# konrad-kaminski/ratelimit

Hardware: AMD Instinct MI355X
Metric: rate-limit decisions/sec (whole node) at 10M/1B keys; p99 batch latency (higher is better)
Workload: dtype u32

## Files before the change

### ratelimit_amd/csrc/rl_engine.h

```cpp
#pragma once

#include <hip/hip_runtime.h>

#include <string>

#include "../../include/ratelimit_hip.h"
#include "rl_device.h"
#include "rl_kernels.h"
#include "rl_match.h"

namespace rl {

#ifndef RL_NBUF
#define RL_NBUF 4
#endif
constexpr uint32_t NBUF = RL_NBUF;
constexpr uint32_t ERRB_RING = 2 * NBUF;
constexpr uint32_t ERRW_B0 = NBUF + 3, ERRW_WORDS = ERRW_B0 + ERRB_RING;
constexpr uint32_t PROF_RING = 8;
constexpr uint32_t PROGRESS_RING = 64;

struct HostSlot {
  uint8_t* stem = nullptr;
  uint32_t *off = nullptr, *req = nullptr, *limit = nullptr, *hits = nullptr, *rule = nullptr;
  int64_t* now = nullptr;
  uint8_t *unit = nullptr, *flags = nullptr;
  uint8_t *code = nullptr, *status = nullptr;
  uint32_t *rem = nullptr, *reset = nullptr;
  unsigned long long* stats = nullptr;
  uint8_t* cbuf = nullptr;
  uint64_t cbuf_cap = 0;
  hipEvent_t in_done = nullptr;
  hipEvent_t out_done = nullptr;
};

struct Engine {
  rl_config cfg;
  hipStream_t stream = nullptr;
  hipStream_t pipe[NBUF] = {};
  hipEvent_t b_done[NBUF] = {};
  hipEvent_t b_table[NBUF] = {};
  hipEvent_t consumed[NBUF] = {};
  hipEvent_t route_ready = nullptr;
  hipEvent_t caller_ready = nullptr;
  bool serial_debug = false;
  uint32_t next = 0, last = NBUF - 1;
  uint32_t errb_seq = NBUF;
  bool b_early = true;
  uint64_t hash_seed = 0;
  HashKey hk{};
  Slot* slots = nullptr;
  uint64_t nslots = 0;
  LogEnt* log = nullptr;
  uint32_t log_cap = 0;
  unsigned long long* log_ctr = nullptr;
  uint32_t horizon = 0;
  uint32_t* tear = nullptr;
  bool copy_time = false;
  bool host_time = false;
  double ht[8] = {};
  uint64_t ht_n = 0;
  hipEvent_t ct_ev[3][64] = {};
  uint32_t ct_n = 0;
  double ct_ms = 0, ct_wait_ms = 0, ct_gap_ms = 0;
  uint64_t ct_count = 0;
  uint8_t* arena = nullptr;
  uint8_t* arena2 = nullptr;
  uint64_t arena_cap16 = 0;
  Scratch s[NBUF]{};
  Scratch rs{};
  bool rs_ready = false;
  unsigned long long* h_base = nullptr;
  uint32_t* errw = nullptr;
  uint8_t* d_stem = nullptr;
  uint32_t *d_off = nullptr, *d_req = nullptr, *d_limit = nullptr, *d_hits = nullptr, *d_rule = nullptr;
  int64_t* d_now = nullptr;
  uint8_t *d_unit = nullptr, *d_flags = nullptr, *d_code = nullptr, *d_status = nullptr;
  uint32_t *d_rem = nullptr, *d_reset = nullptr;
  unsigned long long* d_stats = nullptr;
  uint32_t* h_err = nullptr;
  uint32_t* h_long = nullptr;
  uint32_t long_recent = 0;
  int long_mode = 1;
  uint32_t* h_big = nullptr;
  uint32_t big_recent = 0;
  int big_mode = 1;
  uint32_t* h_late = nullptr;
  uint32_t late_recent = 0;
  int late_mode = 1;
  unsigned long long* h_counters = nullptr;
  std::string last_error;
  uint64_t batches = 0, decisions = 0;
  bool prof = false;
  uint32_t prof_every = 1, prof_skip = 0;
  bool prof_pending[PROF_RING] = {};
  uint32_t prof_next = 0;
  hipEvent_t ev[PROF_RING][RL_NUM_STAGES + 1] = {};
  double stage_ms[RL_NUM_STAGES] = {};
  uint64_t prof_batches = 0;
  unsigned long long* d_kt_acc = nullptr;
  double wclk_khz = 0;
  uint8_t* cfg_blob = nullptr;
  CfgDev cfg_dev{};
  bool cfg_loaded = false;
  uint8_t* mbuf = nullptr;
  size_t mbuf_cap = 0;
  uint32_t* h_match = nullptr;
  HostSlot hs[NBUF]{};
  hipStream_t h2d = nullptr, d2h = nullptr;
  uint32_t hnext = 0;
  bool hs_ready = false;
  uint64_t seq_sub = 0, seq_done = 0;
  hipEvent_t done_ring[PROGRESS_RING] = {};
};

enum StreamRole : uint32_t { SR_ROUTER = 1, SR_HOSTCOPY = 2, SR_PIPE = 4 };
hipError_t rl_stream_create(hipStream_t* st, uint32_t role);
Engine* eng_create(const rl_config* cfg, char* err, size_t errlen);
void eng_destroy(Engine* c);
const char* eng_last_error(const Engine* c);
int eng_do_limit(Engine* c, const rl_batch* in, rl_result* out);
int eng_do_limit_async(Engine* c, const rl_batch* in, rl_result* out, void* stream);
int eng_do_limit_host_async(Engine* c, const rl_batch* in, rl_result* out);
int eng_do_limit_compact_async(Engine* c, const rl_batch_compact* in, rl_result* out);
int eng_compact_check(Engine* c, const rl_batch_compact* in, const rl_result* out);
int eng_do_limit_prefixed_async(Engine* c, const rl_batch_prefixed* in, rl_result* out);
int eng_prefixed_check(Engine* c, const rl_batch_prefixed* in, const rl_result* out, uint32_t* tiles);
int eng_synchronize(Engine* c);
int eng_batch_progress(Engine* c, uint64_t* submitted, uint64_t* completed);
int eng_sweep(Engine* c, int64_t now, uint64_t* n_evicted);
int eng_restore(Engine* c, const rl_restore_batch* in);
int eng_table_info_get(Engine* c, rl_table_info* info);
int eng_debug_keys(Engine* c, const rl_batch* in, uint8_t* out_bytes, uint32_t* out_off, uint32_t out_cap);
int eng_debug_log_tear(Engine* c, const rl_log_tear* arm, rl_log_tear* out);
int eng_debug_decide(Engine* c, uint32_t n, const uint32_t* before, const uint32_t* after, const uint8_t* lc_hit,
                     const uint32_t* hits, const uint32_t* limit, const uint8_t* unit, const uint8_t* flags,
                     const int64_t* now, uint8_t* code, uint32_t* remaining, uint32_t* reset_s, uint64_t* stat_deltas,
                     uint8_t* lc_set);
struct RouteBufs {
  uint8_t* dest;
  uint32_t* hist;
  uint32_t* start;
};
int eng_route_pack(Engine* c, const rl_batch* in, uint32_t n_shards, uint32_t src_rank, void* send_rec,
                   uint8_t* send_stem, uint32_t* perm, uint64_t* counts, void* stream, uint32_t cstride = 2,
                   uint64_t meta0 = 0, uint64_t meta1 = 0, uint32_t own_rank = ROUTE_OWN_NONE,
                   unsigned long long* hash_out = nullptr, unsigned long long* counts_host = nullptr,
                   const RouteBufs* bufs = nullptr);
int eng_route_do_limit(Engine* c, uint32_t n, const void* recv_rec, const uint8_t* recv_stem, uint64_t recv_stem_bytes,
                       const uint64_t* src_stem_base, uint32_t n_shards, uint32_t n_rules, uint32_t rule_stride,
                       uint64_t* ret, uint64_t* stats, int isolate, void* stream);
int eng_route_scatter(Engine* c, uint32_t n, const uint32_t* perm, const uint64_t* ret, rl_result* out, void* stream);
int eng_profile(Engine* c, int enable);
int eng_profile_read(Engine* c, double* ms, uint32_t n, uint64_t* batches);
int eng_config_load(Engine* c, const rl_config_tree* tree);
using RequestsDoLimit = int (*)(void* user, const rl_batch* dev_in, rl_result* dev_out, hipStream_t st);
int eng_do_limit_requests(Engine* c, const rl_request_batch* in, rl_request_result* out, RequestsDoLimit run = nullptr,
                          void* user = nullptr);
int eng_local_cache_info_get(Engine* c, int64_t now, rl_local_cache_info* info);
int eng_snapshot_size(Engine* c, uint64_t* bytes);
int eng_snapshot_save(Engine* c, void* host, uint64_t bytes);
int eng_snapshot_load(Engine* c, const void* host, uint64_t bytes);

int eng_route_owner(Engine* c, uint32_t n, const Wire* recv_rec, const uint8_t* recv_stem, uint64_t recv_stem_bytes,
                    const uint64_t* src_stem_base, uint32_t n_src, uint32_t n_rules, uint32_t rule_stride,
                    unsigned long long* stats, int isolate, hipEvent_t ready, uint32_t* slot,
                    const OwnChunk* own = nullptr, const uint32_t* woff = nullptr,
                    const unsigned long long* wbad = nullptr);

int eng_fail(Engine* c, int code, const std::string& msg);

bool scratch_alloc(Scratch& s, uint32_t n);
void scratch_free(Scratch& s);

}
```

### ratelimit_amd/csrc/rl_engine.hip

```cpp
#include <hip/hip_runtime.h>
#include <hip/hip_ext.h>

#include <algorithm>
#include <chrono>
#include <cstdio>
#include <cstdlib>
#include <random>
#include <cstring>
#include <string>
#include <vector>

#include "../../include/ratelimit_hip.h"
#include "rl_device.h"
#include "rl_kernels.h"
#include "rl_match.h"
#include "rl_engine.h"

using namespace rl;



namespace {

thread_local std::string g_err;

int set_err(Engine* c, int code, const std::string& msg);

void prof_fold(Engine* c, uint32_t k) {
  if (!c->prof_pending[k]) return;
  c->prof_pending[k] = false;
  if (hipEventSynchronize(c->ev[k][RL_NUM_STAGES]) != hipSuccess) return;
  for (int i = 0; i < RL_NUM_STAGES; i++) {
    float ms = 0;
    if (hipEventElapsedTime(&ms, c->ev[k][i], c->ev[k][i + 1]) == hipSuccess) c->stage_ms[i] += ms;
  }
  c->prof_batches++;
}

void prof_fold_all(Engine* c) {
  for (uint32_t k = 0; k < PROF_RING; k++) prof_fold(c, (c->prof_next + k) % PROF_RING);
}

hipEvent_t* prof_events(Engine* c) {
  if (!c->prof) return nullptr;
  if (c->prof_skip) {
    c->prof_skip--;
    return nullptr;
  }
  c->prof_skip = c->prof_every - 1;
  const uint32_t k = c->prof_next;
  c->prof_next = (k + 1) % PROF_RING;
  prof_fold(c, k);
  c->prof_pending[k] = true;
  return c->ev[k];
}

int set_err(Engine* c, int code, const std::string& msg) {
  if (c) c->last_error = msg;
  else g_err = msg;
  return code;
}

#define HIPCHK(c, expr)                                                                        \
  do {                                                                                         \
    hipError_t _e = (expr);                                                                    \
    if (_e != hipSuccess)                                                                      \
      return set_err((c), RL_E_HIP, std::string("gpu: ") + #expr + ": " + hipGetErrorString(_e)); \
  } while (0)

template <typename T>
hipError_t dalloc(T** p, size_t count) {
  return hipMalloc((void**)p, std::max<size_t>(count, 1) * sizeof(T));
}

inline double wall_s() {
  return std::chrono::duration<double>(std::chrono::steady_clock::now().time_since_epoch()).count();
}

int map_err(Engine* c, uint32_t e) {
  if (!e) return RL_OK;
  if (e & ERR_TIME) return set_err(c, RL_E_TIME, "gpu: now outside [0, 2^32-172800] or before the last sweep");
  if (e & ERR_HISTORY)
    return set_err(c, RL_E_TIME,
                   "gpu: a request's window is older than its key's history holds (more than 8 windows and "
                   "div + expiration_jitter_max_seconds behind the key's newest, or the history log overwrote it: "
                   "raise history_entries)");
  if (e & ERR_INVALID) return set_err(c, RL_E_INVALID, "gpu: malformed batch (unit, rule id, request index or stem offsets)");
  if (e & ERR_TABLE_FULL) return set_err(c, RL_E_TABLE_FULL, "gpu: counter table full (raise table_slots or sweep)");
  if (e & ERR_ARENA_FULL) return set_err(c, RL_E_ARENA_FULL, "gpu: long-stem arena full (raise arena_bytes)");
  return set_err(c, RL_E_INTERNAL, "gpu: unknown device error");
}

hipError_t after_batches(Engine* c, hipStream_t st) {
  for (uint32_t k = 0; k < NBUF; k++) {
    const hipError_t e = hipStreamWaitEvent(st, c->b_done[k], 0);
    if (e != hipSuccess) return e;
  }
  return hipSuccess;
}

int collect(Engine* c, hipStream_t st = nullptr) {
  if (!st) st = c->stream;
  HIPCHK(c, hipMemcpyAsync(c->h_err, c->errw, ERRW_WORDS * sizeof(uint32_t), hipMemcpyDeviceToHost, st));
  HIPCHK(c, hipStreamSynchronize(st));
  uint32_t e = c->h_err[NBUF + 2];
  for (uint32_t j = 0; j < NBUF; j++) e |= c->h_err[j];
  for (uint32_t j = 0; j < ERRB_RING; j++) e |= c->h_err[ERRW_B0 + j];
  if (e || c->h_err[NBUF + 1]) {
    HIPCHK(c, hipMemsetAsync(c->errw, 0, ERRW_WORDS * sizeof(uint32_t), st));
    HIPCHK(c, hipStreamSynchronize(st));
  }
  return map_err(c, e);
}

TableDev table_view(Engine* c);
Params params(Engine* c, int isolate = 0);

uint32_t enqueue(Engine* c, const BatchDev& b_in, const OutDev& o, int restore, hipStream_t st, bool pipelined) {
  const uint32_t k = c->next;
  const BatchDev& b = b_in;
  c->next = (k + 1) % NBUF;
  TableDev t = table_view(c);
  t.log_epoch = c->s[k].log_epoch;
  const int isolate = (!restore && o.status) ? 1 : 0;
  const Params P = params(c, isolate);
  const uint32_t* errb_prev = c->s[c->last].errb;
  c->s[k].errb = c->errw + ERRW_B0 + (c->errb_seq++ % ERRB_RING);
  const bool early = c->b_early;
  bool lng = c->long_mode == 2;
  if (c->long_mode == 1) {
    for (uint32_t j = 0; j < NBUF; j++)
      if (__atomic_load_n(&c->h_long[j], __ATOMIC_RELAXED)) {
        __atomic_store_n(&c->h_long[j], 0u, __ATOMIC_RELAXED);
        c->long_recent = 4 * NBUF;
      }
    lng = c->long_recent > 0;
    if (c->long_recent) c->long_recent--;
  }
  uint32_t* hint = c->long_mode ? c->h_long + k : nullptr;
  bool big_full = c->big_mode == 0;
  if (c->big_mode == 1) {
    for (uint32_t j = 0; j < NBUF; j++)
      if (__atomic_load_n(&c->h_big[j], __ATOMIC_RELAXED)) {
        __atomic_store_n(&c->h_big[j], 0u, __ATOMIC_RELAXED);
        c->big_recent = 4 * NBUF;
      }
    big_full = c->big_recent > 0;
    if (c->big_recent) c->big_recent--;
  }
  uint32_t* bhint = c->big_mode == 1 ? c->h_big + k : nullptr;
  bool late_full = c->late_mode == 0;
  if (c->late_mode == 1) {
    for (uint32_t j = 0; j < NBUF; j++)
      if (__atomic_load_n(&c->h_late[j], __ATOMIC_RELAXED)) {
        __atomic_store_n(&c->h_late[j], 0u, __ATOMIC_RELAXED);
        c->late_recent = 4 * NBUF;
      }
    late_full = c->late_recent > 0;
    if (c->late_recent) c->late_recent--;
  }
  uint32_t* lhint = c->late_mode == 1 ? c->h_late + k : nullptr;
  if (pipelined) {
    hipStream_t a = c->pipe[k];
    hipEvent_t* ev = prof_events(c);
    (void)hipStreamWaitEvent(a, c->b_done[k], 0);
    (void)hipStreamWaitEvent(a, c->consumed[k], 0);
    launch_stage_a(b, c->s[k], isolate, P.per_second, a, ev, hint, lng, bhint, big_full);
    if (early) launch_b_begin_early(b, o, c->s[k], restore, a, c->log_ctr);
    (void)hipStreamWaitEvent(a, c->b_table[c->last], 0);
    launch_stage_b(b, o, t, P, c->s[k], restore, a, ev, errb_prev, c->b_table[k], ev ? c->d_kt_acc : nullptr,
                   early, lhint, late_full);
    (void)hipEventRecord(c->b_done[k], a);
  } else {
    if (!st) st = c->stream;
    (void)after_batches(c, st);
    hipEvent_t* ev = prof_events(c);
    launch_stage_a(b, c->s[k], isolate, P.per_second, st, ev, hint, lng, bhint, big_full);
    if (early) launch_b_begin_early(b, o, c->s[k], restore, st, c->log_ctr);
    launch_stage_b(b, o, t, P, c->s[k], restore, st, ev, errb_prev, c->b_table[k], ev ? c->d_kt_acc : nullptr,
                   early, lhint, late_full);
    (void)hipEventRecord(c->b_done[k], st);
  }
  c->last = k;
  return k;
}

hipError_t track(Engine* c, hipStream_t st) {
  if (c->seq_sub - c->seq_done >= PROGRESS_RING) {
    const hipError_t e = hipEventSynchronize(c->done_ring[c->seq_done % PROGRESS_RING]);
    if (e != hipSuccess) return e;
    c->seq_done++;
  }
  const hipError_t e = hipEventRecord(c->done_ring[c->seq_sub % PROGRESS_RING], st);
  c->seq_sub++;
  return e;
}

int check_sizes(Engine* c, const rl_batch* in, uint64_t stem_bytes) {
  if (!in) return set_err(c, RL_E_INVALID, "gpu: null batch");
  if (in->n > c->cfg.max_batch || in->n_requests > c->cfg.max_requests || in->n_rules > c->cfg.max_rules ||
      stem_bytes > c->cfg.max_stem_bytes)
    return set_err(c, RL_E_CAPACITY, "gpu: batch exceeds configured max_batch/max_requests/max_rules/max_stem_bytes");
  if (in->n && in->n_requests == 0) return set_err(c, RL_E_INVALID, "gpu: descriptors without requests");
  return RL_OK;
}

BatchDev dev_view(const Engine* c, const rl_batch* in, uint32_t stem_cap) {
  BatchDev b{};
  b.hk = c->hk;
  b.n = in->n;
  b.n_req = in->n_requests;
  b.n_rules = in->n_rules;
  b.stem_cap = stem_cap;
  b.stem_total = stem_cap;
  b.now_desc = 0;
  b.stem = in->stem_bytes;
  b.off = in->stem_off;
  b.now = in->now;
  b.req = in->req_idx;
  b.unit = in->unit;
  b.flags = in->flags;
  b.limit = in->limit;
  b.hits = in->hits;
  b.rule = in->rule_id;
  return b;
}

hipError_t log_ctr_get(Engine* c, std::vector<unsigned long long>& ctr, unsigned long long* lost,
                       unsigned long long* refused = nullptr) {
  std::vector<unsigned long long> h((size_t)(LOG_PARTS + 1) * LOG_CTR_STRIDE);
  hipError_t e = hipMemcpyAsync(h.data(), c->log_ctr, h.size() * 8, hipMemcpyDeviceToHost, c->stream);
  if (e == hipSuccess) e = hipStreamSynchronize(c->stream);
  if (e != hipSuccess) return e;
  ctr.resize(LOG_PARTS);
  for (uint32_t k = 0; k < LOG_PARTS; k++) ctr[k] = h[(size_t)k * LOG_CTR_STRIDE];
  if (lost) *lost = h[(size_t)LOG_PARTS * LOG_CTR_STRIDE];
  if (refused) *refused = h[(size_t)LOG_PARTS * LOG_CTR_STRIDE + 1];
  return hipSuccess;
}

TableDev table_view(Engine* c) {
  TableDev t;
  t.slots = c->slots;
  t.log = c->log;
  t.log_ctr = c->log_ctr;
  t.log_cap = c->log_cap;
  t.horizon = c->horizon;
  t.hist_lost = c->log_ctr + (size_t)LOG_PARTS * LOG_CTR_STRIDE;
  t.tear = c->tear;
  t.log_epoch = nullptr;
  t.mask = c->nslots - 1;
  t.arena = c->arena;
  t.arena_used16 = c->s[0].counters + 4;
  t.arena_cap16 = c->arena_cap16;
  t.max_probe = (uint32_t)std::min<uint64_t>(c->nslots, 1u << 16);
  t.shift = 64u - (uint32_t)__builtin_ctzll(c->nslots);
  return t;
}

Params params(Engine* c, int isolate) {
  Params P;
  P.ratio = c->cfg.near_limit_ratio;
  P.lc_en = c->cfg.local_cache_enabled != 0;
  P.per_second = c->cfg.per_second_split != 0;
  P.isolate = isolate;
  return P;
}

bool alloc_buffer(Scratch& s, uint32_t n) {
  const size_t items = (size_t)n / (64 * 4 * 8) + 1 + PART_DIGITS;
  bool ok = dalloc(&s.big_meta, PART_DIGITS) == hipSuccess && dalloc(&s.big_n, 1) == hipSuccess &&
            dalloc(&s.big_work, items) == hipSuccess && dalloc(&s.work_n, 1) == hipSuccess &&
            dalloc(&s.sorted_n, 1) == hipSuccess &&
            dalloc(&s.big_cnt, items * (1 + 2 * BIG_HEAVY)) == hipSuccess;
  ok = ok && dalloc(&s.rec, n) == hipSuccess && dalloc(&s.res, n) == hipSuccess;
  for (int i = 0; i < 2; i++) ok = ok && dalloc(&s.keys[i], n) == hipSuccess && dalloc(&s.vals[i], n) == hipSuccess;
  ok = ok && dalloc(&s.grp, n) == hipSuccess && dalloc(&s.lead, n) == hipSuccess && dalloc(&s.gmask, n) == hipSuccess &&
       dalloc(&s.defer, n) == hipSuccess &&
       dalloc(&s.defer_n, 1) == hipSuccess && dalloc(&s.defer2, n) == hipSuccess &&
       dalloc(&s.defer1, n) == hipSuccess && dalloc(&s.defer1_n, 1) == hipSuccess &&
       dalloc(&s.defer2_n, 1) == hipSuccess && dalloc(&s.fast_blk, (size_t)n / (256 * 32) + 1) == hipSuccess &&
       dalloc(&s.log_epoch, LOG_PARTS) == hipSuccess &&
       dalloc(&s.uniq, n) == hipSuccess && dalloc(&s.uniq_n, 1) == hipSuccess &&
       dalloc(&s.long_runs, (size_t)n / 1024 + 2) == hipSuccess &&
       dalloc(&s.kt_blk, 2 * ((size_t)n / 2 + BIG_HEAVY * PART_DIGITS + 2 * (size_t)n + 512) / 256) == hipSuccess;
  ok = ok && dalloc(&s.hits_s, n) == hipSuccess && dalloc(&s.segsum, n) == hipSuccess &&
       dalloc(&s.rid, n) == hipSuccess && dalloc(&s.run_start, (size_t)n + 1) == hipSuccess &&
       dalloc(&s.run_flags, n) == hipSuccess && dalloc(&s.run_state, n) == hipSuccess && dalloc(&s.run_alias, n) == hipSuccess &&
       dalloc(&s.run_f, n) == hipSuccess &&
       dalloc(&s.runs64, 1) == hipSuccess && dalloc(&s.split, 2) == hipSuccess && dalloc(&s.drun, (size_t)n / 2 + BIG_HEAVY * PART_DIGITS) == hipSuccess;
  ok = ok && dalloc(&s.hit_a, n) == hipSuccess && dalloc(&s.tile, n) == hipSuccess &&
       dalloc(&s.hit_t, n) == hipSuccess;
  ok = ok && dalloc(&s.run_end, n) == hipSuccess &&
       dalloc(&s.part_info, (size_t)PART_DIGITS * std::max((n + PART_TILE - 1) / PART_TILE, 1u)) == hipSuccess;
  ok = ok && dalloc(&s.r_base, RL_MAX_SHARDS) == hipSuccess && dalloc(&s.woff, (size_t)n + 1) == hipSuccess &&
       dalloc(&s.wtsum, WIRE_SCAN_WORDS(n)) == hipSuccess;
  return ok;
}

void free_buffer(Scratch& s) {
  void* bufs[] = {s.rec, s.res, s.big_meta, s.big_n, s.big_work, s.work_n, s.sorted_n, s.big_cnt, s.keys[0], s.keys[1],
                  s.vals[0], s.vals[1], s.grp, s.lead, s.gmask, s.defer, s.defer_n, s.defer2, s.defer2_n, s.defer1,
                  s.defer1_n, s.fast_blk, s.hits_s, s.segsum, s.rid, s.run_start, s.run_flags, s.run_state, s.run_alias,
                  s.run_f, s.runs64, s.split, s.drun, s.run_end, s.part_info, s.hit_a, s.tile, s.hit_t, s.r_base,
                  s.uniq, s.uniq_n, s.long_runs, s.kt_blk, s.log_epoch, s.woff, s.wtsum};
  for (void* p : bufs)
    if (p) (void)hipFree(p);
}

int stage(Engine* c, const rl_batch* in, BatchDev* out) {
  const uint32_t n = in->n, nq = in->n_requests;
  const uint64_t nb = n ? in->stem_off[n] : 0;
  int rc = check_sizes(c, in, nb);
  if (rc) return rc;
  hipStream_t st = c->stream;
  HIPCHK(c, after_batches(c, st));
  if (nb) HIPCHK(c, hipMemcpyAsync(c->d_stem, in->stem_bytes, nb, hipMemcpyHostToDevice, st));
  HIPCHK(c, hipMemcpyAsync(c->d_off, in->stem_off, (n + 1) * sizeof(uint32_t), hipMemcpyHostToDevice, st));
  if (nq) HIPCHK(c, hipMemcpyAsync(c->d_now, in->now, nq * sizeof(int64_t), hipMemcpyHostToDevice, st));
  if (n) {
    HIPCHK(c, hipMemcpyAsync(c->d_req, in->req_idx, n * 4, hipMemcpyHostToDevice, st));
    HIPCHK(c, hipMemcpyAsync(c->d_unit, in->unit, n, hipMemcpyHostToDevice, st));
    HIPCHK(c, hipMemcpyAsync(c->d_flags, in->flags, n, hipMemcpyHostToDevice, st));
    HIPCHK(c, hipMemcpyAsync(c->d_limit, in->limit, n * 4, hipMemcpyHostToDevice, st));
    HIPCHK(c, hipMemcpyAsync(c->d_hits, in->hits, n * 4, hipMemcpyHostToDevice, st));
    HIPCHK(c, hipMemcpyAsync(c->d_rule, in->rule_id, n * 4, hipMemcpyHostToDevice, st));
  }
  rl_batch d = *in;
  d.stem_bytes = c->d_stem;
  d.stem_off = c->d_off;
  d.now = c->d_now;
  d.req_idx = c->d_req;
  d.unit = c->d_unit;
  d.flags = c->d_flags;
  d.limit = c->d_limit;
  d.hits = c->d_hits;
  d.rule_id = c->d_rule;
  *out = dev_view(c, &d, c->cfg.max_stem_bytes);
  return RL_OK;
}

}

namespace rl {

const char* eng_last_error(const Engine* c) { return c ? c->last_error.c_str() : g_err.c_str(); }

hipError_t rl_stream_create(hipStream_t* st, uint32_t role) {
  static const uint32_t dedicated =
      getenv("RL_DEDICATED_QUEUES") ? (uint32_t)strtoul(getenv("RL_DEDICATED_QUEUES"), nullptr, 0) : 0u;
  if (!(dedicated & role)) return hipStreamCreateWithFlags(st, hipStreamNonBlocking);
  int dev = 0, cus = 0;
  hipError_t e = hipGetDevice(&dev);
  if (e == hipSuccess) e = hipDeviceGetAttribute(&cus, hipDeviceAttributeMultiprocessorCount, dev);
  if (e != hipSuccess) return e;
  std::vector<uint32_t> mask(((uint32_t)cus + 31) / 32, 0xFFFFFFFFu);
  return hipExtStreamCreateWithCUMask(st, (uint32_t)mask.size(), mask.data());
}

Engine* eng_create(const rl_config* cfg_in, char* err, size_t errlen) {
  auto fail = [&](const std::string& m, Engine* c) -> Engine* {
    if (err && errlen) snprintf(err, errlen, "%s", m.c_str());
    g_err = m;
    if (c) eng_destroy(c);
    return nullptr;
  };
  if (!cfg_in) return fail("gpu: null config", nullptr);
  rl_config cfg = *cfg_in;
  if (!cfg.table_slots) cfg.table_slots = 1ull << 24;
  if (cfg.table_slots & (cfg.table_slots - 1)) return fail("gpu: table_slots must be a power of two", nullptr);
  if (!cfg.arena_bytes) cfg.arena_bytes = 64ull << 20;
  if (!cfg.history_entries) cfg.history_entries = cfg.table_slots;
  if (cfg.history_entries > (uint64_t)LOG_PARTS * LOG_PART_MAX)
    return fail("gpu: history_entries must be at most 2^31", nullptr);
  if (cfg.expiration_jitter_max_seconds < 0) return fail("gpu: expiration_jitter_max_seconds must be >= 0", nullptr);
  if (!cfg.max_batch) cfg.max_batch = 1u << 20;
  if (cfg.max_batch > MAX_PART_TILES * PART_TILE)
    return fail("gpu: max_batch must be at most 8388608 descriptors", nullptr);
  if (!cfg.max_requests) cfg.max_requests = cfg.max_batch;
  if (!cfg.max_rules) cfg.max_rules = 65536;
  if (!cfg.max_stem_bytes) cfg.max_stem_bytes = 128u * cfg.max_batch;
  if (hipSetDevice(cfg.device) != hipSuccess) return fail("gpu: hipSetDevice failed", nullptr);

  Engine* c = new Engine();
  c->cfg = cfg;
  c->hash_seed = cfg.hash_seed;
  while (!c->hash_seed) {
    std::random_device rd;
    c->hash_seed = ((uint64_t)rd() << 32) ^ rd();
  }
  c->cfg.hash_seed = c->hash_seed;
  c->hk = hash_key_of(c->hash_seed, cfg.debug_hash_bits);
  c->nslots = cfg.table_slots;
  {
    const uint64_t want = std::max<uint64_t>(cfg.history_entries / LOG_PARTS, std::max<uint64_t>(cfg.max_batch / 16, 1024));
    uint64_t cap = 1;
    while (cap * 2 <= want && cap * 2 <= LOG_PART_MAX) cap *= 2;
    if (cap < want && cap < LOG_PART_MAX) cap *= 2;
    c->log_cap = (uint32_t)cap;
    c->cfg.history_entries = (uint64_t)LOG_PARTS * cap;
    c->horizon = (uint32_t)std::min<int64_t>(cfg.expiration_jitter_max_seconds, 1ll << 30);
  }
  c->arena_cap16 = cfg.arena_bytes / 16;
  const uint32_t n = cfg.max_batch;
  bool ok = true;
  for (uint32_t k = 0; k < NBUF; k++) ok = ok && rl_stream_create(&c->pipe[k], SR_PIPE) == hipSuccess;
  if (const char* be = getenv("RL_B_BEGIN_EARLY")) c->b_early = atoi(be) != 0;
  c->stream = c->pipe[0];
  for (uint32_t k = 0; k < NBUF; k++)
    ok = ok && hipEventCreateWithFlags(&c->b_done[k], hipEventDisableTiming) == hipSuccess &&
         hipEventCreateWithFlags(&c->b_table[k], hipEventDisableTiming) == hipSuccess;
  for (uint32_t k = 0; k < PROGRESS_RING; k++)
    ok = ok && hipEventCreateWithFlags(&c->done_ring[k], hipEventDisableTiming) == hipSuccess;
  ok = ok && dalloc(&c->slots, c->nslots) == hipSuccess &&
       dalloc(&c->log, (size_t)LOG_PARTS * c->log_cap) == hipSuccess &&
       dalloc(&c->log_ctr, (size_t)(LOG_PARTS + 1) * LOG_CTR_STRIDE) == hipSuccess;
  ok = ok && dalloc(&c->arena, cfg.arena_bytes) == hipSuccess && dalloc(&c->arena2, cfg.arena_bytes) == hipSuccess;
  for (uint32_t k = 0; k < NBUF; k++) ok = ok && alloc_buffer(c->s[k], n);
  Scratch& s0 = c->s[0];
  ok = ok && dalloc(&c->errw, ERRW_WORDS) == hipSuccess;
  for (uint32_t k = 0; k < NBUF; k++)
    ok = ok && hipEventCreateWithFlags(&c->consumed[k], hipEventDisableTiming) == hipSuccess;
  ok = ok && hipEventCreateWithFlags(&c->route_ready, hipEventDisableTiming) == hipSuccess &&
       hipEventCreateWithFlags(&c->caller_ready, hipEventDisableTiming) == hipSuccess;
  c->serial_debug = getenv("RL_DEBUG_SERIAL") != nullptr;
  c->copy_time = getenv("RL_DEBUG_COPYTIME") != nullptr;
  c->host_time = getenv("RL_DEBUG_HOSTTIME") != nullptr;
  for (uint32_t k = 0; c->copy_time && k < 64; k++)
    ok = ok && hipEventCreate(&c->ct_ev[0][k]) == hipSuccess && hipEventCreate(&c->ct_ev[1][k]) == hipSuccess &&
         hipEventCreate(&c->ct_ev[2][k]) == hipSuccess;
  ok = ok && hipHostMalloc((void**)&c->h_base, (size_t)NBUF * RL_MAX_SHARDS * 8) == hipSuccess;
  for (uint32_t k = 0; k < NBUF; k++)
    ok = ok && dalloc(&c->s[k].stripes, (size_t)STAT_STRIPES * STAT_LDS_RULES * RL_NUM_STATS) == hipSuccess;
  ok = ok && dalloc(&s0.time_floor, 1) == hipSuccess;
  ok = ok && dalloc(&s0.counters, 8) == hipSuccess;
  for (uint32_t k = 0; k < NBUF; k++) {
    Scratch& sk = c->s[k];
    sk.err = c->errw ? c->errw + k : nullptr;
    sk.errb = c->errw ? c->errw + ERRW_B0 + k : nullptr;
    sk.errs = c->errw ? c->errw + NBUF + 1 : nullptr;
    sk.time_floor = s0.time_floor;
    sk.counters = s0.counters;
  }
  ok = ok && dalloc(&c->d_stem, (size_t)cfg.max_stem_bytes + 64) == hipSuccess;
  ok = ok && dalloc(&c->d_off, (size_t)n + 1) == hipSuccess;
  ok = ok && dalloc(&c->d_now, cfg.max_requests) == hipSuccess;
  ok = ok && dalloc(&c->d_req, n) == hipSuccess && dalloc(&c->d_unit, n) == hipSuccess &&
       dalloc(&c->d_flags, n) == hipSuccess && dalloc(&c->d_limit, n) == hipSuccess &&
       dalloc(&c->d_hits, n) == hipSuccess && dalloc(&c->d_rule, n) == hipSuccess;
  ok = ok && dalloc(&c->d_code, n) == hipSuccess && dalloc(&c->d_status, n) == hipSuccess &&
       dalloc(&c->d_rem, n) == hipSuccess &&
       dalloc(&c->d_reset, n) == hipSuccess;
  ok = ok && dalloc(&c->d_stats, (size_t)cfg.max_rules * RL_NUM_STATS) == hipSuccess;
  ok = ok && hipHostMalloc((void**)&c->h_err, ERRW_WORDS * sizeof(uint32_t)) == hipSuccess;
  ok = ok && hipHostMalloc((void**)&c->h_counters, 8 * sizeof(unsigned long long)) == hipSuccess;
  ok = ok && hipHostMalloc((void**)&c->h_long, NBUF * sizeof(uint32_t)) == hipSuccess;
  if (ok) memset(c->h_long, 0, NBUF * sizeof(uint32_t));
  if (const char* sl = getenv("RL_SPLIT_LONG")) c->long_mode = atoi(sl);
  ok = ok && hipHostMalloc((void**)&c->h_big, NBUF * sizeof(uint32_t)) == hipSuccess;
  if (ok) memset(c->h_big, 0, NBUF * sizeof(uint32_t));
  if (const char* bc = getenv("RL_BIG_CUE")) c->big_mode = atoi(bc);
  ok = ok && hipHostMalloc((void**)&c->h_late, NBUF * sizeof(uint32_t)) == hipSuccess;
  if (ok) memset(c->h_late, 0, NBUF * sizeof(uint32_t));
  if (const char* lc = getenv("RL_LATE_CUE")) c->late_mode = atoi(lc);
  if (!ok) return fail("gpu: device allocation failed (table_slots/arena/max_batch too large?)", c);
  ok = hipMemsetAsync(c->slots, 0, c->nslots * sizeof(Slot), c->stream) == hipSuccess &&
       hipMemsetAsync(c->log_ctr, 0, (size_t)(LOG_PARTS + 1) * LOG_CTR_STRIDE * 8, c->stream) == hipSuccess &&
       hipMemsetAsync(c->errw, 0, ERRW_WORDS * 4, c->stream) == hipSuccess &&
       hipMemsetAsync(s0.time_floor, 0, 8, c->stream) == hipSuccess &&
       hipMemsetAsync(s0.counters, 0, 64, c->stream) == hipSuccess &&
       hipMemsetAsync(c->s[0].stripes, 0, (size_t)STAT_STRIPES * STAT_LDS_RULES * RL_NUM_STATS * 8, c->stream) ==
           hipSuccess &&
       hipMemsetAsync(c->d_stem, 0, (size_t)cfg.max_stem_bytes + 64, c->stream) == hipSuccess &&
       hipStreamSynchronize(c->stream) == hipSuccess;
  for (uint32_t k = 0; k < NBUF; k++)
    ok = ok && hipEventRecord(c->b_done[k], c->stream) == hipSuccess &&
         hipEventRecord(c->b_table[k], c->stream) == hipSuccess &&
         (k == 0 || hipMemsetAsync(c->s[k].stripes, 0, (size_t)STAT_STRIPES * STAT_LDS_RULES * RL_NUM_STATS * 8,
                                   c->stream) == hipSuccess) &&
         hipEventRecord(c->consumed[k], c->stream) == hipSuccess;
  if (!ok) return fail("gpu: device initialisation failed", c);
  return c;
}

void free_host_slots(Engine* c) {
  for (HostSlot& h : c->hs) {
    void* bufs[] = {h.stem, h.off, h.req, h.limit, h.hits, h.rule, h.now, h.unit, h.flags, h.code, h.status, h.rem,
                    h.reset, h.stats, h.cbuf};
    for (void* p : bufs)
      if (p) (void)hipFree(p);
    if (h.in_done) (void)hipEventDestroy(h.in_done);
    if (h.out_done) (void)hipEventDestroy(h.out_done);
    h = HostSlot{};
  }
  for (hipStream_t st : {c->h2d, c->d2h})
    if (st) (void)hipStreamDestroy(st);
  c->h2d = c->d2h = nullptr;
  c->hs_ready = false;
}

void copy_time_fold(Engine* c, bool all);

void eng_destroy(Engine* c) {
  if (!c) return;
  (void)hipSetDevice(c->cfg.device);
  if (c->host_time && c->ht_n)
    fprintf(stderr, "RL_DEBUG_HOSTTIME: %llu batches, ms each: check %.4f copy %.4f unpack %.4f enqueue %.4f to_host %.4f "
            "track %.4f\n", (unsigned long long)c->ht_n, c->ht[0] / c->ht_n * 1e3, c->ht[1] / c->ht_n * 1e3,
            c->ht[2] / c->ht_n * 1e3, c->ht[3] / c->ht_n * 1e3, c->ht[4] / c->ht_n * 1e3, c->ht[5] / c->ht_n * 1e3);
  if (c->copy_time) {
    (void)hipDeviceSynchronize();
    copy_time_fold(c, true);
    if (c->ct_count)
      fprintf(stderr, "RL_DEBUG_COPYTIME: %llu input copies, %.4f ms each, slot wait %.4f ms, gap after the previous "
              "copy %.4f ms\n", (unsigned long long)c->ct_count, c->ct_ms / c->ct_count, c->ct_wait_ms / c->ct_count,
              c->ct_gap_ms / c->ct_count);
    for (uint32_t k = 0; k < 64; k++)
      for (int j = 0; j < 3; j++)
        if (c->ct_ev[j][k]) (void)hipEventDestroy(c->ct_ev[j][k]);
  }
  if (c->hs_ready) {
    (void)hipDeviceSynchronize();
    free_host_slots(c);
  }
  for (uint32_t k = 0; k < NBUF; k++)
    if (c->pipe[k]) (void)hipStreamSynchronize(c->pipe[k]);
  for (uint32_t k = 0; k < PROF_RING; k++)
    for (int i = 0; i <= RL_NUM_STAGES; i++)
      if (c->ev[k][i]) (void)hipEventDestroy(c->ev[k][i]);
  if (c->d_kt_acc) (void)hipFree(c->d_kt_acc);
  for (uint32_t k = 0; k < NBUF; k++) {
    free_buffer(c->s[k]);
    if (c->b_done[k]) (void)hipEventDestroy(c->b_done[k]);
    if (c->b_table[k]) (void)hipEventDestroy(c->b_table[k]);
    if (c->consumed[k]) (void)hipEventDestroy(c->consumed[k]);
  }
  for (uint32_t k = 0; k < PROGRESS_RING; k++)
    if (c->done_ring[k]) (void)hipEventDestroy(c->done_ring[k]);
  if (c->rs_ready) {
    c->rs.err = nullptr;
    scratch_free(c->rs);
  }
  if (c->route_ready) (void)hipEventDestroy(c->route_ready);
  if (c->caller_ready) (void)hipEventDestroy(c->caller_ready);
  if (c->h_base) (void)hipHostFree(c->h_base);
  const Scratch& s0 = c->s[0];
  void* bufs[] = {c->slots, c->log, c->log_ctr, c->tear, c->arena, c->arena2, c->errw, s0.stripes, s0.time_floor, s0.counters, c->d_stem, c->d_off,
                  c->d_now, c->d_req, c->d_unit, c->d_flags, c->d_limit, c->d_hits, c->d_rule, c->d_code, c->d_status,
                  c->d_rem,
                  c->d_reset, c->d_stats};
  for (void* p : bufs)
    if (p) (void)hipFree(p);
  for (uint32_t k = 1; k < NBUF; k++)
    if (c->s[k].stripes) (void)hipFree(c->s[k].stripes);
  if (c->h_err) (void)hipHostFree(c->h_err);
  if (c->h_counters) (void)hipHostFree(c->h_counters);
  if (c->h_long) (void)hipHostFree(c->h_long);
  if (c->h_big) (void)hipHostFree(c->h_big);
  if (c->h_late) (void)hipHostFree(c->h_late);
  for (void* p : {(void*)c->cfg_blob, (void*)c->mbuf})
    if (p) (void)hipFree(p);
  if (c->h_match) (void)hipHostFree(c->h_match);
  for (uint32_t k = 0; k < NBUF; k++)
    if (c->pipe[k]) (void)hipStreamDestroy(c->pipe[k]);
  delete c;
}

int eng_do_limit_async(Engine* c, const rl_batch* in, rl_result* out, void* stream) {
  if (!c || !in || !out) return set_err(c, RL_E_INVALID, "gpu: null argument");
  int rc = check_sizes(c, in, 0);
  if (rc) return rc;
  if ((uintptr_t)in->stem_bytes & 3u) return set_err(c, RL_E_INVALID, "gpu: stem_bytes must be 4-byte aligned");
  HIPCHK(c, hipSetDevice(c->cfg.device));
  BatchDev b = dev_view(c, in, c->cfg.max_stem_bytes);
  OutDev o{out->code, out->limit_remaining, out->reset_s, (unsigned long long*)out->stats, out->status};
  hipStream_t st = (hipStream_t)stream;
  if (st && c->serial_debug) {
    enqueue(c, b, o, 0, st, false);
    HIPCHK(c, track(c, st));
  } else {
    if (st && hipStreamQuery(st) == hipErrorNotReady) {
      HIPCHK(c, hipEventRecord(c->caller_ready, st));
      HIPCHK(c, hipStreamWaitEvent(c->pipe[c->next], c->caller_ready, 0));
    }
    const uint32_t k = enqueue(c, b, o, 0, nullptr, true);
    HIPCHK(c, track(c, c->pipe[k]));
  }
  HIPCHK(c, hipGetLastError());
  c->batches++;
  c->decisions += in->n;
  return RL_OK;
}

bool scratch_alloc(Scratch& s, uint32_t n) {
  s = Scratch{};
  bool ok = alloc_buffer(s, n);
  ok = ok && dalloc(&s.err, 1) == hipSuccess && dalloc(&s.route_start, 2 * RL_MAX_SHARDS + 1) == hipSuccess &&
       dalloc(&s.route_dest, n) == hipSuccess && dalloc(&s.route_hash, n) == hipSuccess &&
       dalloc(&s.route_hist, 2ull * RL_MAX_SHARDS * ((n + ROUTE_TILE - 1) / ROUTE_TILE)) == hipSuccess;
  ok = ok && hipMemset(s.err, 0, 4) == hipSuccess;
  return ok;
}

void scratch_free(Scratch& s) {
  free_buffer(s);
  for (void* p : {(void*)s.err, (void*)s.route_start, (void*)s.route_dest, (void*)s.route_hash, (void*)s.route_hist})
    if (p) (void)hipFree(p);
  s = Scratch{};
}

int eng_route_pack(Engine* c, const rl_batch* in, uint32_t n_shards, uint32_t src_rank, void* send_rec,
                   uint8_t* send_stem, uint32_t* perm, uint64_t* counts, void* stream, uint32_t cstride,
                   uint64_t meta0, uint64_t meta1, uint32_t own_rank, unsigned long long* hash_out,
                   unsigned long long* counts_host, const RouteBufs* bufs) {
  if (!c || !in || !counts || (in->n && (!send_rec || !send_stem || !perm)))
    return set_err(c, RL_E_INVALID, "gpu: null argument");
  if (n_shards < 1 || n_shards > RL_MAX_SHARDS || src_rank >= n_shards)
    return set_err(c, RL_E_INVALID, "gpu: n_shards must be 1..256 and src_rank < n_shards");
  int rc = check_sizes(c, in, 0);
  if (rc) return rc;
  if ((uintptr_t)in->stem_bytes & 3u) return set_err(c, RL_E_INVALID, "gpu: stem_bytes must be 4-byte aligned");
  HIPCHK(c, hipSetDevice(c->cfg.device));
  if (!c->rs_ready) {
    HIPCHK(c, after_batches(c, c->stream));
    HIPCHK(c, hipStreamSynchronize(c->stream));
    if (!scratch_alloc(c->rs, c->cfg.max_batch)) {
      scratch_free(c->rs);
      return set_err(c, RL_E_HIP, "gpu: routing scratch allocation failed");
    }
    (void)hipFree(c->rs.err);
    c->rs.err = c->errw + NBUF + 2;
    c->rs_ready = true;
  }
  hipStream_t st = stream ? (hipStream_t)stream : c->stream;
  BatchDev b = dev_view(c, in, c->cfg.max_stem_bytes);
  Scratch rs = c->rs;
  if (bufs) {
    rs.route_dest = bufs->dest;
    rs.route_hist = bufs->hist;
    rs.route_start = bufs->start;
  }
  launch_route_pack(b, n_shards, src_rank, (Wire*)send_rec, send_stem, perm, (unsigned long long*)counts, rs, st,
                    cstride, meta0, meta1, own_rank, hash_out, counts_host);
  HIPCHK(c, hipGetLastError());
  return RL_OK;
}

int eng_route_owner(Engine* c, uint32_t n, const Wire* recv_rec, const uint8_t* recv_stem, uint64_t recv_stem_bytes,
                    const uint64_t* src_stem_base, uint32_t n_src, uint32_t n_rules, uint32_t rule_stride,
                    unsigned long long* stats, int isolate, hipEvent_t ready, uint32_t* slot,
                    const OwnChunk* own, const uint32_t* woff, const unsigned long long* wbad) {
  const uint32_t rules_eff = rule_stride ? n_src * rule_stride : n_rules;
  const bool has_own = own && own->n;
  if (!c || !src_stem_base || (n && (!recv_rec || (!recv_stem && recv_stem_bytes))) || (rules_eff && !stats))
    return set_err(c, RL_E_INVALID, "gpu: null argument");
  if (n && !recv_stem && !(has_own && own->n == n)) return set_err(c, RL_E_INVALID, "gpu: null argument");
  if (has_own && ((uint64_t)own->lo + own->n > n || own->rank >= n_src || !own->idx || !own->hash || !own->stem ||
                  ((uintptr_t)own->stem & 3u)))
    return set_err(c, RL_E_INVALID, "gpu: bad own chunk");
  if (n_src < 1 || n_src > RL_MAX_SHARDS) return set_err(c, RL_E_INVALID, "gpu: n_shards must be 1..256");
  if (rule_stride && n_rules > rule_stride) return set_err(c, RL_E_INVALID, "gpu: n_rules exceeds the rule stride");
  if (n > c->cfg.max_batch || rules_eff > c->cfg.max_rules || recv_stem_bytes >= (1ull << 32))
    return set_err(c, RL_E_CAPACITY, "gpu: routed batch exceeds max_batch/max_rules or 4 GiB of stems");
  if ((uintptr_t)recv_stem & 3u) return set_err(c, RL_E_INVALID, "gpu: recv_stem must be 4-byte aligned");
  HIPCHK(c, hipSetDevice(c->cfg.device));
  const uint32_t k = c->next;
  Scratch& sk = c->s[k];
  hipStream_t a = c->pipe[k];
  HIPCHK(c, hipStreamWaitEvent(a, c->b_done[k], 0));
  HIPCHK(c, hipStreamWaitEvent(a, c->consumed[k], 0));
  if (ready) HIPCHK(c, hipStreamWaitEvent(a, ready, 0));
  if (!(has_own && own->n == n)) {
    unsigned long long* hb = c->h_base + (size_t)k * RL_MAX_SHARDS;
    HIPCHK(c, hipEventSynchronize(c->b_done[k]));
    for (uint32_t j = 0; j < n_src; j++) hb[j] = src_stem_base[j];
    HIPCHK(c, hipMemcpyAsync(sk.r_base, hb, (size_t)n_src * 8, hipMemcpyHostToDevice, a));
    if (!woff) {
      launch_wire_offsets(recv_rec, n, has_own ? own->lo : 0u, has_own ? own->lo + own->n : 0u, sk.r_base, n_src,
                          recv_stem_bytes, sk.woff, sk.wtsum, a);
      woff = sk.woff;
      wbad = sk.wtsum + WIRE_SCAN_TILES(n);
    }
  }
  BatchDev b{};
  b.hk = c->hk;
  b.n = n;
  b.n_req = n;
  b.n_rules = rules_eff;
  b.stem_cap = (uint32_t)recv_stem_bytes;
  b.stem_total = (uint32_t)recv_stem_bytes;
  b.now_desc = 1;
  b.stem = recv_stem;
  b.wire = recv_rec;
  b.woff = woff;
  b.wbad = wbad;
  b.wbase = sk.r_base;
  b.n_src = n_src;
  b.rule_stride = rule_stride;
  if (has_own) b.own = *own;
  OutDev o{nullptr, nullptr, nullptr, stats, isolate ? c->d_status : nullptr};
  const uint32_t kk = enqueue(c, b, o, 0, nullptr, true);
  HIPCHK(c, hipGetLastError());
  c->batches++;
  c->decisions += n;
  *slot = kk;
  return RL_OK;
}

int eng_route_do_limit(Engine* c, uint32_t n, const void* recv_rec, const uint8_t* recv_stem, uint64_t recv_stem_bytes,
                       const uint64_t* src_stem_base, uint32_t n_shards, uint32_t n_rules, uint32_t rule_stride,
                       uint64_t* ret, uint64_t* stats, int isolate, void* stream) {
  if (!c || (n && !ret)) return set_err(c, RL_E_INVALID, "gpu: null argument");
// ... 987 lines not shown
```

### ratelimit_amd/csrc/rl_kernels.h

```cpp
#pragma once

#include <hip/hip_runtime.h>
#include <stdint.h>

#include "rl_device.h"

namespace rl {

#ifndef RL_PART_ITEMS
#define RL_PART_ITEMS 16
#endif
constexpr uint32_t PART_ITEMS = RL_PART_ITEMS, PART_TILE = 256 * PART_ITEMS;
constexpr uint32_t PART_BITS = 10, PART_DIGITS = 1u << PART_BITS;
#ifndef RL_BIG_BLOCKS
#define RL_BIG_BLOCKS 64
#endif
constexpr uint32_t BIG_BLOCKS = RL_BIG_BLOCKS;
constexpr uint32_t BIG_ITEM_BLOCKS = 256;
constexpr uint32_t BIG_HEAVY = 4;

struct BigMeta {
  uint32_t d, S, base, nchunks, item0, r, rb_heavy, db_heavy;
  uint32_t heavy[BIG_HEAVY];
};
constexpr uint32_t MAX_PART_TILES = 2048 * 16 / PART_ITEMS;
constexpr uint32_t LONG_RUN = 32;
constexpr uint32_t RUN_SLOW = 1, RUN_FAST = 2, RUN_MULTI = 4;
constexpr uint32_t RUN_NOWVAR = 8;
constexpr uint32_t RUN_ALIAS = 16;
constexpr uint32_t RUN_AHEAD = 32;
constexpr uint32_t RUN_MERGE = 64;
constexpr uint32_t RUN_G_SHIFT = 8, RUN_UMASK_SHIFT = 16;
constexpr uint32_t RUN_UNITS = 128, RUN_STEMS = 1u << 24;
#ifndef RL_KEY_HEAD
#define RL_KEY_HEAD 64
#endif
constexpr uint32_t KEY_HEAD = RL_KEY_HEAD;
constexpr uint32_t KEY_HV = KEY_HEAD / 16;
static_assert(KEY_HEAD % 16 == 0 && KEY_HEAD >= 48 && KEY_HEAD <= 64, "key head: 48 or 64 bytes (>= KEY_IN)");
constexpr uint32_t STAT_STRIPES = 64;
constexpr uint32_t STAT_LDS_RULES = 512;
constexpr uint32_t RUNS_GENERAL_LATE_BLOCKS = 8;

struct Wire;
struct OwnChunk {
  uint32_t lo, n, rank, stem_total;
  uint32_t src_n;
  uint32_t n_rules;
  const uint32_t* idx;
  const unsigned long long* hash;
  const uint8_t* stem;
  const uint32_t* off;
  const int64_t* now;
  const uint32_t* req;
  const uint8_t* unit;
  const uint8_t* flags;
  const uint32_t* limit;
  const uint32_t* hits;
  const uint32_t* rule;
  uint8_t* code;
  uint32_t* rem;
  uint32_t* reset;
  uint8_t* status;
  uint32_t* src_err;
};
struct BatchDev {
  uint32_t n, n_req, n_rules, stem_cap;
  uint32_t stem_total;
  uint32_t now_desc;
  HashKey hk;
  const uint8_t* stem;
  const uint32_t* off;
  const int64_t* now;
  const uint32_t* req;
  const uint8_t* unit;
  const uint8_t* flags;
  const uint32_t* limit;
  const uint32_t* hits;
  const uint32_t* rule;
  const Wire* wire;
  const uint32_t* woff;
  const unsigned long long* wbad;
  const unsigned long long* wbase;
  uint32_t n_src, rule_stride;
  OwnChunk own;
};

struct __attribute__((aligned(16))) Rec {
  uint32_t hlo;
  uint32_t off;
  uint32_t lu;
  uint32_t rule;
  uint32_t req;
  uint32_t now;
  uint32_t hits;
  uint32_t limit;
};
static_assert(sizeof(Rec) == 32, "Rec is two dwordx4");

struct SRec {
  const Rec* rec;
  const uint32_t* sv;
  __device__ inline Rec operator[](uint32_t q) const { return rec[sv[q]]; }
};

__host__ __device__ inline uint32_t rec_len(const Rec& r) { return r.lu & 0xFFFFu; }
__host__ __device__ inline uint32_t rec_unit(const Rec& r) { return (r.lu >> 16) & 0xFFu; }
__host__ __device__ inline uint32_t rec_flags(const Rec& r) { return r.lu >> 24; }

constexpr uint32_t ROUTE_REQ_BITS = 24;
constexpr uint32_t ROUTE_MAX_REQ = 1u << ROUTE_REQ_BITS;
constexpr uint32_t ROUTE_TILE = 512;
struct __attribute__((aligned(8))) Wire {
  uint32_t label;
  uint32_t lu;
  uint32_t limit;
  uint32_t hits;
  uint32_t rule;
  uint32_t now;
  unsigned long long hash;
};
constexpr uint32_t WIRE_NOW_BAD = 0xFFFFFFFFu;
static_assert(sizeof(Wire) == RL_WIRE_BYTES, "wire record size is part of the ABI");

struct OutDev {
  uint8_t* code;
  uint32_t* rem;
  uint32_t* reset;
  unsigned long long* stats;
  uint8_t* status;
};

struct TableDev {
  Slot* slots;
  LogEnt* log;
  unsigned long long* log_ctr;
  uint32_t log_cap;
  uint32_t horizon;
  unsigned long long* hist_lost;
  const unsigned long long* log_epoch;
  uint32_t* tear;
  uint64_t mask;
  uint8_t* arena;
  unsigned long long* arena_used16;
  uint64_t arena_cap16;
  uint32_t max_probe;
  uint32_t shift;
};

struct Params {
  float ratio;
  int lc_en;
  int per_second;
  int isolate;
};

struct Scratch {
  Rec* rec;
  unsigned long long* res;
  uint32_t* keys[2];
  uint32_t* vals[2];
  BigMeta* big_meta;
  uint32_t* big_n;
  uint32_t* big_work;
  uint32_t* work_n;
  uint32_t* sorted_n;
  uint32_t* big_cnt;
  uint32_t* grp;
  uint32_t* lead;
  uint8_t* gmask;
  uint32_t* defer;
  uint32_t* defer_n;
  uint32_t* defer2;
  uint32_t* defer2_n;
  uint32_t* defer1;
  uint32_t* defer1_n;
  uint32_t* fast_blk;
  unsigned long long* log_epoch;
  uint2* uniq;
  uint32_t* uniq_n;
  uint32_t* long_runs;
  unsigned long long* kt_blk;
  unsigned long long* stripes;
  uint32_t* hits_s;
  uint32_t* hit_a;
  uint4* tile;
  uint32_t* hit_t;
  uint32_t* segsum;
  uint32_t* rid;
  uint32_t* run_start;
  uint32_t* run_end;
  uint32_t* part_info;
  uint32_t* run_flags;
  uint4* run_state;
  uint4* run_alias;
  uint32_t* run_f;
  unsigned long long* runs64;
  unsigned long long* split;
  uint32_t* drun;
  uint32_t* err;
  uint32_t* errb;
  uint32_t* errs;
  int64_t* time_floor;
  unsigned long long* counters;
  uint32_t* route_start;
  uint8_t* route_dest;
  unsigned long long* route_hash;
  uint32_t* route_hist;
  unsigned long long* r_base;
  uint32_t* woff;
  unsigned long long* wtsum;
};

void launch_stage_a(const BatchDev& b, const Scratch& s, int isolate, int per_second, hipStream_t st,
                    hipEvent_t* ev = nullptr, uint32_t* long_hint = nullptr, bool long_kernel = false,
                    uint32_t* big_hint = nullptr, bool big_full = true);
void launch_stage_b(const BatchDev& b, const OutDev& o, const TableDev& t, const Params& P, const Scratch& s,
                    int restore, hipStream_t st, hipEvent_t* ev, const uint32_t* errb_prev, hipEvent_t table_done,
                    unsigned long long* kt_acc = nullptr, bool early = false, uint32_t* late_hint = nullptr,
                    bool late_full = true);
void launch_b_begin_early(const BatchDev& b, const OutDev& o, const Scratch& s, int restore, hipStream_t st,
                          const unsigned long long* log_ctr);
void launch_unpack(const rl_batch_compact& cb, const uint8_t* buf, uint32_t* req, uint8_t* unit, uint8_t* flags,
                   uint32_t* limit, uint32_t* hits, uint32_t* rule, int64_t* now, uint32_t* err, hipStream_t st);
void launch_unpack_range(const rl_batch_compact& cb, const uint8_t* buf, uint32_t d0, uint32_t d1, uint32_t q0,
                         uint32_t q1, uint32_t* req, uint8_t* unit, uint8_t* flags, uint32_t* limit, uint32_t* hits,
                         uint32_t* rule, int64_t* now, uint32_t* err, hipStream_t st);
constexpr uint32_t TO_HOST_MAX = 6;
struct ToHost {
  const uint8_t* src[TO_HOST_MAX];
  uint8_t* dst[TO_HOST_MAX];
  uint64_t bytes[TO_HOST_MAX];
  uint32_t n;
};
void launch_to_host(const ToHost& c, hipStream_t st);
hipError_t copy_to_host(ToHost c, hipStream_t st);

void launch_unpack_prefixed(const rl_batch_prefixed& pb, const uint8_t* buf, uint32_t t0, uint32_t t1, uint8_t* stem,
                            uint32_t* off, uint32_t* req, uint8_t* unit, uint8_t* flags, uint32_t* limit,
                            uint32_t* hits, uint32_t* rule, int64_t* now, uint32_t* err, hipStream_t st);
constexpr uint32_t ROUTE_OWN_NONE = 0xFFFFFFFFu;
constexpr uint32_t WIRE_SCAN_TILE = 2048;
inline uint32_t WIRE_SCAN_TILES(uint64_t n) { return (uint32_t)((n + WIRE_SCAN_TILE) / WIRE_SCAN_TILE); }
inline uint32_t WIRE_SCAN_WORDS(uint64_t n) { return WIRE_SCAN_TILES(n) + 1; }
void launch_wire_offsets(const Wire* w, uint32_t n, uint32_t olo, uint32_t ohi, const unsigned long long* wbase,
                         uint32_t n_src, unsigned long long stem_total, uint32_t* woff, unsigned long long* tsum,
                         hipStream_t st);
void launch_route_pack(const BatchDev& b, uint32_t n_shards, uint32_t src_rank, Wire* out, uint8_t* out_stem,
                       uint32_t* perm, unsigned long long* counts, const Scratch& s, hipStream_t st,
                       uint32_t cstride = 2, unsigned long long meta0 = 0, unsigned long long meta1 = 0,
                       uint32_t own_rank = ROUTE_OWN_NONE, unsigned long long* hash_out = nullptr,
                       unsigned long long* counts_host = nullptr);
void launch_cnt_fill(unsigned long long* cnt, uint32_t n_peers, uint32_t cstride, unsigned long long meta0,
                     unsigned long long meta1, hipStream_t st, unsigned long long* cnt_host = nullptr);
void launch_route_fail(unsigned long long* ret, uint32_t n, uint32_t status, hipStream_t st);
void launch_route_scatter(const uint32_t* perm, const unsigned long long* ret, uint32_t n, const OutDev& o,
                          hipStream_t st, uint32_t* src_err = nullptr, const uint32_t* errb = nullptr,
                          uint32_t own_lo = 0, uint32_t own_hi = 0);
void launch_route_ret(const unsigned long long* res, uint32_t n, const uint32_t* errb, unsigned long long* ret,
                      hipStream_t st);
void launch_stats_sum(const unsigned long long* stage, uint32_t n_blocks, uint32_t m, unsigned long long* out,
                      hipStream_t st, uint32_t stride = 0);
void launch_sweep(const TableDev& t, uint64_t nslots, uint32_t now, unsigned long long* evicted, hipStream_t st);
void launch_arena_compact(Slot* slots, uint64_t nslots, const uint8_t* from, uint8_t* to, unsigned long long* used16,
                          hipStream_t st);
void launch_lc_count(const TableDev& t, uint64_t nslots, uint32_t now, unsigned long long* out, hipStream_t st);
void launch_table_info(const Slot* slots, uint64_t nslots, unsigned long long* out, hipStream_t st);
bool log_tear_hook();
void launch_debug_keys(const BatchDev& b, uint8_t* out, uint32_t* klen, hipStream_t st);
void launch_debug_decide(uint32_t n, const uint32_t* before, const uint32_t* after, const uint8_t* lc_hit,
                         const uint32_t* hits, const uint32_t* limit, const uint8_t* unit, const uint8_t* flags,
                         const int64_t* now, float ratio, int lc_en, uint8_t* code, uint32_t* rem, uint32_t* reset,
                         unsigned long long* deltas, uint8_t* lc_set, hipStream_t st);

}
```

### ratelimit_amd/csrc/rl_kernels.hip

```cpp
#include <hip/hip_runtime.h>
#include <stdint.h>
#include <cstdlib>

#include "rl_device.h"
#include "rl_kernels.h"

#ifndef RL_ABL
#define RL_ABL 0
#endif

namespace rl {

constexpr uint32_t HASH_LDS_BYTES = 16384;

__global__ __launch_bounds__(256) void k_prepare(BatchDev b, Rec* __restrict__ rec, uint32_t* __restrict__ keys,
                                                 uint32_t* err, uint32_t* errs, int isolate,
                                                 const int64_t* time_floor, uint32_t* defer_n,
                                                 uint32_t* big_n, uint32_t* work_n, uint32_t* __restrict__ run_flags,
                                                 unsigned long long* num_runs, uint32_t* __restrict__ hit_a,
                                                 unsigned long long* __restrict__ res, uint32_t* sorted_n,
                                                 uint32_t* uniq_n) {
  __shared__ uint32_t lds[HASH_LDS_BYTES / 4 + 4];
  const uint32_t tid = threadIdx.x;
  const uint32_t i = blockIdx.x * 256 + tid;
// ... 1195 lines not shown
        c = Win{x.w, 0, 0, lcw};
      } else if (G.old[ui].ws != x.w) {
        gen_set_old(t, G, ui, Win{x.w, 0, 0, lcw}, true);
      }
    }
    for (uint32_t k = 0; k < 4; k++) {
      if (!(G.present >> k & 1) || ps_class(P, k) != ps_e) continue;
      Win* R = gen_rec(t, G, k, x.w, x.now, nullptr);
      if (R) {
        R->count = nv;
        R->expire = ex;
        gen_touch(G, k, R);
      }
    }
    after = nv;
  }
  if (restore) {
    if (x.flags) {
      for (uint32_t k = 0; k < 4; k++) {
        if (!(G.present >> k & 1)) continue;
        Win* R = gen_rec(t, G, k, x.w, x.now, nullptr);
        if (R) {
          R->lc = x.now + x.d;
          gen_touch(G, k, R);
        }
      }
    }
    return;
  }
  const Decision r = decide(after - x.h, after, lc_hit && !x.shadow, x.h, x.thr, P.ratio, x.shadow, P.lc_en);
  if (r.set_lc) {
    uint32_t j = 0;
    while (j < G.npend && G.pend_w[j] != x.w) j++;
    if (j == G.npend) G.npend++;
    G.pend_w[j] = x.w;
    G.pend_e[j] = x.now + x.d;
  }
  emit(res, L, acc, x, r, lc_hit);
}

__device__ __attribute__((always_inline)) inline void replay_simple(SRec rec_s, const uint32_t* svals,
                                                                    unsigned long long* res, const TableDev& t,
                                                                    const Params& P, const uint32_t* grp,
                                                                    uint32_t p, uint32_t end, uint32_t k, int64_t s0,
                                                                    Win cur0, uint32_t ring0, uint32_t tag0,
                                                                    const Rec& x0, uint32_t e0, LaneStats& L,
                                                                    StatAcc& acc, uint32_t* err, bool restore) {
  Slot* s = &t.slots[s0];
  SimpleState S;
  S.cur = cur0;
  S.old = Win{WS_INVALID, 0, 0, 0};
  S.si = (uint32_t)s0;
  S.tag = tag0;
  S.chain = ring0;
  S.cur_dirty = S.old_dirty = S.chain_dirty = false;
  S.cur_req = 0xFFFFFFFFu;
  S.pend = false;
  simple_step(t, P, res, L, acc, S, load_elem(x0, e0, restore), restore, err);
  for (uint32_t q = p + 1; q < end; q++) {
    if (grp && grp[q] != k) continue;
    simple_step(t, P, res, L, acc, S, load_elem(rec_s[q], svals[q], restore), restore, err);
  }
  S.apply_pending();
  if (S.old_dirty) simple_put(t, S);
  if (S.cur_dirty) s->cur = S.cur;
  if (S.chain_dirty) s->ring = S.chain;
}

__device__ __attribute__((always_inline)) inline uint32_t wave_incl_add(uint32_t x);
struct SegPair {
  uint32_t f, s;
};
__device__ inline SegPair seg_op(SegPair a, SegPair b) { return SegPair{a.f | b.f, b.f ? b.s : a.s + b.s}; }

struct SegChunk {
  uint64_t heads;
  uint32_t h;
};

__device__ inline SegPair seg_chunk_scan(const SegChunk& c, uint32_t lane) {
  const uint32_t P = wave_incl_add(c.h);
  const uint64_t le = c.heads & (lane == 63 ? ~0ull : ((2ull << lane) - 1));
  const uint32_t lh = le ? 63u - (uint32_t)__clzll((long long)le) : 0u;
  const uint32_t Plh = __shfl(P, lh, 64), hlh = __shfl(c.h, lh, 64);
  return le ? SegPair{1u, P - (Plh - hlh)} : SegPair{0u, P};
}

constexpr uint32_t BK_HEAVY = BIG_HEAVY;
constexpr uint32_t BK_HEAVY_MIN = 3;

template <uint32_t W, uint32_t IT>
struct BkShape {
  static constexpr uint32_t WAVES = W, ITEMS = IT, THREADS = 64 * W, CAP = 64 * W * IT, STRIP = 64 * IT;
};
using BkSmall = BkShape<4, 8>;
using BkBig = BkShape<8, 8>;

#ifdef RL_BK_PROF
__device__ unsigned long long g_bk_prof[PART_DIGITS * 16];
__device__ uint32_t g_bk_peel[PART_DIGITS * 16];
#define BK_STAMP(d, k) \
  if (threadIdx.x == 0) g_bk_prof[(d) * 16 + (k)] = wall_clock64()
#else
#define BK_STAMP(d, k)
#endif

template <uint32_t IT, uint32_t BITS>
__device__ inline void wave_multisplit(const uint32_t (&kk)[IT], uint32_t nvalid_base, uint32_t limit, uint32_t shift,
                                       uint32_t* row, uint32_t (&pos)[IT]) {
  const uint32_t lane = threadIdx.x & 63;
  const uint64_t lt_mask = (1ull << lane) - 1;
  uint32_t leader[IT];
#pragma unroll
  for (uint32_t i = 0; i < IT; i++) {
    leader[i] = lane;
    pos[i] = 0;
    if (nvalid_base + i * 64 >= limit) continue;
    const bool valid = nvalid_base + i * 64 + lane < limit;
    const uint32_t d = (kk[i] >> shift) & ((1u << BITS) - 1u);
    uint64_t peers = __ballot(valid);
#pragma unroll
    for (uint32_t bit = 0; bit < BITS; bit++) {
      const bool sb = (d >> bit) & 1u;
      const uint64_t bal = __ballot(sb);
      peers &= sb ? bal : ~bal;
    }
    const uint32_t rank = __popcll(peers & lt_mask);
    leader[i] = valid ? (uint32_t)(__ffsll((unsigned long long)peers) - 1) : lane;
    pos[i] = (valid && rank == 0) ? atomicAdd(&row[d], (uint32_t)__popcll(peers)) : 0u;
    pos[i] |= rank << 16;
  }
#pragma unroll
  for (uint32_t i = 0; i < IT; i++) pos[i] = __shfl(pos[i] & 0xFFFFu, leader[i]) + (pos[i] >> 16);
}

__device__ inline uint32_t scan256(uint32_t v, uint32_t* wsum4, uint32_t* total) {
  const uint32_t lane = threadIdx.x & 63, wave = threadIdx.x >> 6;
  uint32_t inc = v;
#pragma unroll
  for (uint32_t off = 1; off < 64; off <<= 1) {
    const uint32_t y = __shfl_up(inc, off, 64);
    if (lane >= off) inc += y;
  }
  if (wave < 4 && lane == 63) wsum4[wave] = inc;
  __syncthreads();
  uint32_t pre = 0;
#pragma unroll
  for (uint32_t w = 0; w < 4; w++) pre += w < wave ? wsum4[w] : 0u;
  if (total) *total = wsum4[0] + wsum4[1] + wsum4[2] + wsum4[3];
  __syncthreads();
  return pre + inc - v;
}

__global__ __launch_bounds__(256) void k_part(const uint32_t* __restrict__ kin, const uint32_t* __restrict__ hin,
                                              uint4* __restrict__ out, uint32_t n, uint32_t ntiles,
                                              uint32_t* __restrict__ info, const uint32_t* err) {
  constexpr uint32_t DPT = PART_DIGITS / 256;
  __shared__ uint32_t wcnt[4][PART_DIGITS];
  __shared__ uint32_t wsum[4];
  __shared__ uint32_t sk[PART_TILE], sv[PART_TILE], sh[PART_TILE];
  if (*err) return;
  const uint32_t tid = threadIdx.x, lane = tid & 63, wave = tid >> 6, tile = blockIdx.x;
  for (uint32_t j = tid; j < 4 * PART_DIGITS; j += 256) (&wcnt[0][0])[j] = 0;
  __syncthreads();
  const uint32_t wbase = tile * PART_TILE + wave * 64 * PART_ITEMS;
  uint32_t kk[PART_ITEMS], vv[PART_ITEMS], hh[PART_ITEMS], pos[PART_ITEMS];
#pragma unroll
  for (uint32_t i = 0; i < PART_ITEMS; i++) {
    const uint32_t j = min(wbase + i * 64 + lane, n - 1);
    kk[i] = kin[j];
    vv[i] = j;
    hh[i] = hin[j];
  }
  wave_multisplit<PART_ITEMS, PART_BITS>(kk, wbase, n, 32 - PART_BITS, wcnt[wave], pos);
  __syncthreads();
  uint32_t c[DPT], tsum = 0;
#pragma unroll
  for (uint32_t j = 0; j < DPT; j++) {
    const uint32_t d = tid * DPT + j;
    uint32_t acc = 0;
#pragma unroll
    for (uint32_t w = 0; w < 4; w++) {
      const uint32_t t = wcnt[w][d];
      wcnt[w][d] = acc;
      acc += t;
    }
    c[j] = acc;
    tsum += acc;
  }
  uint32_t excl = scan256(tsum, wsum, nullptr);
#pragma unroll
  for (uint32_t j = 0; j < DPT; j++) {
    const uint32_t d = tid * DPT + j;
    info[(size_t)d * ntiles + tile] = (excl << 16) | c[j];
#pragma unroll
    for (uint32_t w = 0; w < 4; w++) wcnt[w][d] += excl;
    excl += c[j];
  }
  __syncthreads();
#pragma unroll
  for (uint32_t i = 0; i < PART_ITEMS; i++) {
    if (wbase + i * 64 + lane < n) {
      const uint32_t d = kk[i] >> (32 - PART_BITS);
      const uint32_t q = wcnt[wave][d] + pos[i];
      sk[q] = kk[i];
      sv[q] = vv[i];
      sh[q] = hh[i];
    }
  }
  __syncthreads();
  const uint32_t cnt = min(PART_TILE, n - tile * PART_TILE);
  uint4* o = out + (size_t)tile * PART_TILE;
#pragma unroll
  for (uint32_t i = 0; i < PART_ITEMS; i++) {
    const uint32_t q = i * 256 + tid;
    if (q < cnt) o[q] = make_uint4(sk[q], sv[q], sh[q], 0u);
  }
}

template <typename B>
struct BucketLds {
  uint32_t k[B::CAP], v[B::CAP], h[B::CAP];
  uint32_t wcnt[B::WAVES][256];
  uint32_t gsum[B::WAVES / 4][256];
  uint32_t base[256];
  uint32_t roff[3][256];
  uint32_t dtot[256];
  uint32_t wsum[B::WAVES];
  SegPair sp[B::WAVES];
  uint32_t sh[B::WAVES];
  SegPair carry;
  uint32_t hcarry, rb, nruns, S, base_pos, db, dcnt;
  uint32_t heavy[BK_HEAVY];
  uint32_t hcnt[BK_HEAVY];
  uint32_t hstart[BK_HEAVY];
  uint32_t hrun[BK_HEAVY];
  uint32_t hw[B::WAVES][BK_HEAVY];
  uint32_t hsw[B::WAVES][BK_HEAVY];
  uint32_t acc[1 + 2 * BK_HEAVY];
  uint32_t lw[B::WAVES];
  uint32_t nheavy, nlight;
  uint32_t ub;
};

extern __shared__ uint32_t bk_seg[];

template <uint32_t IT>
__device__ inline void bucket_src(uint32_t ntiles, const uint32_t (&p)[IT], uint32_t (&j)[IT]) {
  const uint32_t* seg = bk_seg;
  const uint32_t* src = bk_seg + ntiles + 1;
  uint32_t lo[IT];
#pragma unroll
  for (uint32_t i = 0; i < IT; i++) lo[i] = 0;
#pragma unroll
  for (uint32_t step = MAX_PART_TILES / 2; step; step >>= 1) {
    if (step >= ntiles) continue;
#pragma unroll
    for (uint32_t i = 0; i < IT; i++) {
      const uint32_t m = lo[i] + step;
      if (m < ntiles && seg[m] <= p[i]) lo[i] = m;
    }
  }
#pragma unroll
  for (uint32_t i = 0; i < IT; i++) j[i] = src[lo[i]] + p[i];
}

template <typename B>
__device__ inline uint32_t block_sum(BucketLds<B>& L, uint32_t v) {
  const uint32_t lane = threadIdx.x & 63, wave = threadIdx.x >> 6;
#pragma unroll
  for (uint32_t off = 32; off; off >>= 1) v += __shfl_xor(v, off, 64);
  if (lane == 0) L.wsum[wave] = v;
  __syncthreads();
  uint32_t s = 0;
#pragma unroll
  for (uint32_t w = 0; w < B::WAVES; w++) s += L.wsum[w];
  __syncthreads();
  return s;
}

template <typename B>
__device__ inline void bucket_setup(BucketLds<B>& L, const uint32_t* __restrict__ info, uint32_t ntiles, uint32_t d) {
  const uint32_t tid = threadIdx.x, lane = tid & 63, wave = tid >> 6;
  uint32_t* seg = bk_seg;
  uint32_t* src = bk_seg + ntiles + 1;
  uint32_t carry = 0, offs = 0;
  for (uint32_t t0 = 0; t0 < ntiles; t0 += B::THREADS) {
    const uint32_t t = t0 + tid;
    const uint32_t e = t < ntiles ? info[(size_t)d * ntiles + t] : 0u;
    const uint32_t cnt = e & 0xFFFFu;
    offs += e >> 16;
    uint32_t inc = cnt;
#pragma unroll
    for (uint32_t off = 1; off < 64; off <<= 1) {
      const uint32_t y = __shfl_up(inc, off, 64);
      if (lane >= off) inc += y;
    }
    if (lane == 63) L.wsum[wave] = inc;
    __syncthreads();
    uint32_t pre = carry, all = carry;
    for (uint32_t w = 0; w < B::WAVES; w++) {
      pre += w < wave ? L.wsum[w] : 0u;
      all += L.wsum[w];
    }
    if (t < ntiles) {
      const uint32_t st = pre + inc - cnt;
      seg[t] = st;
      src[t] = t * PART_TILE + (e >> 16) - st;
    }
    carry = all;
    __syncthreads();
  }
  const uint32_t bp = block_sum(L, offs);
  if (tid == 0) {
    seg[ntiles] = carry;
    L.S = carry;
    L.base_pos = bp;
  }
  __syncthreads();
}

template <typename B, uint32_t BITS>
__device__ inline void bucket_rank(BucketLds<B>& L, const uint32_t (&kk)[B::ITEMS], uint32_t strip0, uint32_t limit,
                                   uint32_t shift, bool chunk_scan, uint32_t (&pos)[B::ITEMS]) {
  const uint32_t tid = threadIdx.x, wave = tid >> 6;
  for (uint32_t j = tid; j < B::WAVES * 256; j += B::THREADS) (&L.wcnt[0][0])[j] = 0;
  __syncthreads();
  uint32_t local[B::ITEMS];
  wave_multisplit<B::ITEMS, BITS>(kk, strip0, limit, shift, L.wcnt[wave], local);
  __syncthreads();
  constexpr uint32_t NG = B::WAVES / 4;
  const uint32_t dg = tid & 255u, g = tid >> 8;
  uint32_t r[4], c = 0;
#pragma unroll
  for (uint32_t w = 0; w < 4; w++) r[w] = L.wcnt[g * 4 + w][dg];
#pragma unroll
  for (uint32_t w = 0; w < 4; w++) {
    const uint32_t t = r[w];
    r[w] = c;
    c += t;
  }
  L.gsum[g][dg] = c;
  __syncthreads();
  uint32_t pre = 0, all = 0;
#pragma unroll
  for (uint32_t q = 0; q < NG; q++) {
    const uint32_t t = L.gsum[q][dg];
    pre += q < g ? t : 0u;
    all += t;
  }
#pragma unroll
  for (uint32_t w = 0; w < 4; w++) L.wcnt[g * 4 + w][dg] = r[w] + pre;
  if (tid < 256) L.dtot[tid] = all;
  const uint32_t excl = scan256(tid < 256 ? all : 0u, L.wsum, nullptr);
  if (chunk_scan && tid < 256) L.base[tid] = excl;
  __syncthreads();
#pragma unroll
  for (uint32_t i = 0; i < B::ITEMS; i++) {
    const uint32_t d = (kk[i] >> shift) & ((1u << BITS) - 1u);
    pos[i] = L.base[d] + L.wcnt[wave][d] + local[i];
  }
  __syncthreads();
}

template <typename B>
__device__ inline void lds_sort3(BucketLds<B>& L, uint32_t (&kk)[B::ITEMS], uint32_t (&vv)[B::ITEMS],
                                 uint32_t (&hh)[B::ITEMS], uint32_t n) {
  static_assert(32 - PART_BITS == 22, "passes of 8 + 8 + 6 bits");
  const uint32_t lane = threadIdx.x & 63, strip0 = (threadIdx.x >> 6) * B::STRIP;
  uint32_t pos[B::ITEMS];
#pragma unroll 1
  for (uint32_t pass = 0; pass < 3; pass++) {
    if (pass < 2) bucket_rank<B, 8>(L, kk, strip0, n, 8 * pass, true, pos);
    else bucket_rank<B, 6>(L, kk, strip0, n, 16, true, pos);
#pragma unroll
    for (uint32_t i = 0; i < B::ITEMS; i++) {
      if (strip0 + i * 64 + lane < n) {
        L.k[pos[i]] = kk[i];
        L.v[pos[i]] = vv[i];
        L.h[pos[i]] = hh[i];
      }
    }
    __syncthreads();
#pragma unroll
    for (uint32_t i = 0; i < B::ITEMS; i++) {
      const uint32_t p = strip0 + i * 64 + lane;
      if (p < n) {
        kk[i] = L.k[p];
        vv[i] = L.v[p];
        hh[i] = L.h[p];
      }
    }
  }
}

template <typename B, bool FROM_LDS>
__device__ inline void bucket_segment(BucketLds<B>& L, uint32_t d, uint32_t S, uint32_t base,
                                      const uint32_t* __restrict__ sk, const uint32_t* __restrict__ sh,
                                      uint32_t* __restrict__ segsum, uint32_t* __restrict__ rid,
                                      uint32_t* __restrict__ run_start, uint32_t* __restrict__ run_end,
                                      unsigned long long* num_runs, uint32_t* __restrict__ drun) {
  constexpr uint32_t IT = B::ITEMS;
  const uint32_t tid = threadIdx.x, lane = tid & 63, wave = tid >> 6;
  auto key = [&](uint32_t p) -> uint32_t { return FROM_LDS ? L.k[p] : sk[base + p]; };
  auto hit = [&](uint32_t p) -> uint32_t { return FROM_LDS ? L.h[p] : sh[base + p]; };
  uint32_t nh = 0, nd = 0;
  for (uint32_t c0 = 0; c0 < S; c0 += B::CAP) {
    uint32_t a[IT], b[IT], c[IT];
#pragma unroll
    for (uint32_t i = 0; i < IT; i++) {
      const uint32_t p = min(c0 + i * B::THREADS + tid, S - 1);
      a[i] = key(p ? p - 1 : 0);
      b[i] = key(p);
      c[i] = key(p > 1 ? p - 2 : 0);
    }
#pragma unroll
    for (uint32_t i = 0; i < IT; i++) {
      const uint32_t p = c0 + i * B::THREADS + tid;
      nh += (p < S && (p == 0 || a[i] != b[i])) ? 1u : 0u;
      nd += (p < S && p >= 1 && a[i] == b[i] && (p == 1 || c[i] != a[i])) ? 1u : 0u;
    }
  }
  nh = block_sum(L, nh);
  nd = block_sum(L, nd);
  BK_STAMP(d, 4);
  if (tid == 0) {
    const unsigned long long old = atomicAdd(num_runs, ((unsigned long long)nd << 32) | nh);
    L.rb = (uint32_t)old;
    L.db = (uint32_t)(old >> 32);
    L.dcnt = 0;
    L.nruns = nh;
    L.carry = SegPair{0, 0};
    L.hcarry = 0;
  }
  __syncthreads();
  const uint32_t rb = L.rb;
  for (uint32_t c0 = 0; c0 < S; c0 += B::CAP) {
    const uint32_t s0 = c0 + wave * B::STRIP;
    const uint32_t ni = s0 >= S ? 0u : min(IT, (S - s0 + 63) / 64);
    SegChunk ch[IT];
    SegPair agg{0, 0};
    uint32_t hc = 0;
    uint32_t kp[IT], kq[IT], hq[IT], kpp[IT];
#pragma unroll
    for (uint32_t j = 0; j < IT; j++) {
      const uint32_t q = min(s0 + 64 * j + lane, S - 1);
      kp[j] = key(q ? q - 1 : 0);
      kq[j] = key(q);
      hq[j] = hit(q);
      kpp[j] = key(q > 1 ? q - 2 : 0);
    }
    uint32_t hd = 0, sd = 0;
#pragma unroll
    for (uint32_t j = 0; j < IT; j++) {
      const uint32_t q = s0 + 64 * j + lane;
      hd |= (q < S && (q == 0 || kp[j] != kq[j])) ? 1u << j : 0u;
      sd |= (q < S && q >= 1 && kp[j] == kq[j] && (q == 1 || kpp[j] != kp[j])) ? 1u << j : 0u;
    }
#pragma unroll
    for (uint32_t j = 0; j < IT; j++) {
      ch[j] = SegChunk{0, 0};
      if (j >= ni) continue;
      const uint32_t hv = s0 + 64 * j + lane < S ? (hq[j] > 1 ? hq[j] : 1u) : 0u;
      ch[j] = SegChunk{(uint64_t)__ballot((hd >> j) & 1u), hv};
      uint32_t t = hv;
      const uint32_t lh = ch[j].heads ? 63u - (uint32_t)__clzll((long long)ch[j].heads) : 0u;
      if (ch[j].heads && lane < lh) t = 0;
#pragma unroll
      for (uint32_t off = 32; off; off >>= 1) t += __shfl_xor(t, off, 64);
      agg = seg_op(agg, SegPair{ch[j].heads ? 1u : 0u, t});
      hc += (uint32_t)__popcll(ch[j].heads);
    }
    if (lane == 0) {
      L.sp[wave] = agg;
      L.sh[wave] = hc;
    }
    __syncthreads();
    SegPair run = L.carry;
    uint32_t hrun = L.hcarry;
    SegPair tot = run;
    uint32_t htot = hrun;
    for (uint32_t w = 0; w < B::WAVES; w++) {
      if (w == wave) {
        run = tot;
        hrun = htot;
      }
      tot = seg_op(tot, L.sp[w]);
      htot += L.sh[w];
    }
    __syncthreads();
    if (tid == 0) {
      L.carry = tot;
      L.hcarry = htot;
    }
#pragma unroll
    for (uint32_t j = 0; j < IT; j++) {
      if (j >= ni) continue;
      const uint32_t q = s0 + 64 * j + lane;
      const SegPair v = seg_chunk_scan(ch[j], lane);
      const SegPair in = seg_op(run, v);
      const uint64_t heads = ch[j].heads;
      const uint32_t r = hrun + (uint32_t)__popcll(heads & (lane == 63 ? ~0ull : ((2ull << lane) - 1))) - 1;
      if (q < S) {
        segsum[base + q] = in.s;
        rid[base + q] = rb + r;
        if ((heads >> lane) & 1) {
          run_start[rb + r] = base + q;
          if (r) run_end[rb + r - 1] = base + q;
        }
        if ((sd >> j) & 1) drun[L.db + atomicAdd(&L.dcnt, 1u)] = rb + r;
      }
      run = seg_op(run, SegPair{__shfl(v.f, 63, 64), __shfl(v.s, 63, 64)});
      hrun += (uint32_t)__popcll(heads);
    }
    __syncthreads();
  }
  if (tid == 0 && S) run_end[rb + L.nruns - 1] = base + S;
}

constexpr uint32_t BIG_CHUNK = BkSmall::CAP;
constexpr uint32_t BIG_LIGHT_CAP = BkBig::CAP;
constexpr uint32_t BIG_CNT = 1 + 2 * BK_HEAVY;

constexpr uint32_t BK_SAMPLES_PER_LANE = 4;
template <typename B>
__device__ inline void sample_heavy(BucketLds<B>& L, uint32_t S, uint32_t ntiles, const uint4* __restrict__ pt) {
  constexpr uint32_t R = BK_SAMPLES_PER_LANE, NS = 64 * R;
  const uint32_t lane = threadIdx.x & 63;
  if ((threadIdx.x >> 6) == 0) {
    uint32_t p[R], j[R], ks[R], cnt[R];
    bool first[R];
#pragma unroll
    for (uint32_t i = 0; i < R; i++) p[i] = (uint32_t)(((uint64_t)(2 * (lane * R + i) + 1) * S) / (2 * NS));
    bucket_src(ntiles, p, j);
#pragma unroll
    for (uint32_t i = 0; i < R; i++) {
      ks[i] = pt[j[i]].x;
      cnt[i] = 0;
      first[i] = true;
    }
    for (uint32_t q = 0; q < 64; q++) {
#pragma unroll
      for (uint32_t r = 0; r < R; r++) {
        const uint32_t kq = __shfl(ks[r], q, 64), g = q * R + r;
#pragma unroll
        for (uint32_t i = 0; i < R; i++) {
          cnt[i] += kq == ks[i] ? 1u : 0u;
          if (g < lane * R + i && kq == ks[i]) first[i] = false;
        }
      }
    }
    uint32_t nc = 0;
#pragma unroll
    for (uint32_t i = 0; i < R; i++) nc += (first[i] && cnt[i] >= BK_HEAVY_MIN) ? 1u : 0u;
    uint32_t incl = nc;
#pragma unroll
    for (uint32_t o = 1; o < 64; o <<= 1) {
      const uint32_t y = __shfl_up(incl, o, 64);
      if (lane >= o) incl += y;
    }
    uint32_t rank = incl - nc;
#pragma unroll
    for (uint32_t i = 0; i < R; i++)
      if (first[i] && cnt[i] >= BK_HEAVY_MIN) {
        if (rank < BK_HEAVY) L.heavy[rank] = ks[i];
        rank++;
      }
    if (lane == 63) L.nheavy = min(incl, BK_HEAVY);
  }
  __syncthreads();
}

__global__ __launch_bounds__(BkSmall::THREADS, 4) void k_bucket(
    const uint4* __restrict__ pt,
    const uint32_t* __restrict__ info, uint32_t ntiles, uint32_t* __restrict__ sk, uint32_t* __restrict__ sv,
    uint32_t* __restrict__ sh, uint32_t* __restrict__ segsum, uint32_t* __restrict__ rid,
    uint32_t* __restrict__ run_start, uint32_t* __restrict__ run_end, unsigned long long* num_runs,
    uint32_t* __restrict__ drun, BigMeta* __restrict__ meta, uint32_t* big_n, uint32_t* __restrict__ work,
    uint32_t* work_n, uint32_t* sorted_n, uint2* __restrict__ uniq, uint32_t* uniq_n, const uint32_t* err,
    uint32_t* big_hint) {
  using B = BkSmall;
  __shared__ BucketLds<B> L;
  if (*err) return;
  const uint32_t tid = threadIdx.x, lane = tid & 63, wave = tid >> 6, d = blockIdx.x;
  BK_STAMP(d, 0);
  bucket_setup(L, info, ntiles, d);
  const uint32_t S = L.S;
  if (!S) return;
  if (S > B::CAP) {
    sample_heavy(L, S, ntiles, pt);
    if (tid == 0) {
      BigMeta M;
      M.d = d;
      M.S = S;
      M.base = atomicAdd(sorted_n, S);
      M.r = L.nheavy;
      M.nchunks = M.r ? (S + BIG_CHUNK - 1) / BIG_CHUNK : 0u;
      M.item0 = M.nchunks ? atomicAdd(work_n, M.nchunks) : 0u;
      const unsigned long long old =
          M.r ? atomicAdd(num_runs, ((unsigned long long)M.r << 32) | M.r) : 0ull;
      M.rb_heavy = (uint32_t)old;
      M.db_heavy = (uint32_t)(old >> 32);
      for (uint32_t c = 0; c < BK_HEAVY; c++) M.heavy[c] = c < M.r ? L.heavy[c] : 0u;
      const uint32_t b = atomicAdd(big_n, 1u);
      meta[b] = M;
      if (big_hint) *big_hint = 1u;
      L.rb = b;
      L.nruns = M.item0;
      L.hcarry = M.nchunks;
    }
    __syncthreads();
    for (uint32_t t = tid; t < L.hcarry; t += B::THREADS) work[L.nruns + t] = (L.rb << 16) | t;
    return;
  }
  BK_STAMP(d, 1);
  uint32_t kk[B::ITEMS], vv[B::ITEMS], hh[B::ITEMS];
  const uint32_t strip0 = wave * B::STRIP;
  uint32_t pp[B::ITEMS], jj[B::ITEMS];
#pragma unroll
  for (uint32_t i = 0; i < B::ITEMS; i++) pp[i] = min(strip0 + i * 64 + lane, S - 1);
  bucket_src(ntiles, pp, jj);
#pragma unroll
  for (uint32_t i = 0; i < B::ITEMS; i++) {
    const uint4 e = pt[jj[i]];
    kk[i] = e.x;
    vv[i] = e.y;
    hh[i] = e.z;
  }
  BK_STAMP(d, 2);
  uint32_t* ht = L.v;
  uint8_t* df = reinterpret_cast<uint8_t*>(&L.wcnt[0][0]);
  static_assert(sizeof(L.wcnt) >= B::CAP, "dup flags fit the multisplit rows");
  constexpr uint32_t HT = 2 * B::CAP, HT_SHIFT = 32 - 12;
  static_assert(HT == 1u << 12, "hash index bits");
#pragma unroll
  for (uint32_t i = 0; i < B::ITEMS; i++) {
    const uint32_t p = strip0 + i * 64 + lane;
    if (p < S) L.k[p] = kk[i];
  }
  for (uint32_t j = tid; j < HT; j += B::THREADS) ht[j] = 0xFFFFFFFFu;
  for (uint32_t j = tid; j < B::CAP / 4; j += B::THREADS) reinterpret_cast<uint32_t*>(df)[j] = 0u;
  __syncthreads();
#pragma unroll
  for (uint32_t i = 0; i < B::ITEMS; i++) {
    const uint32_t p = strip0 + i * 64 + lane;
    if (p >= S) continue;
    uint32_t h = (kk[i] * 0x9E3779B1u) >> HT_SHIFT;
    for (;;) {
      const uint32_t o = atomicCAS(&ht[h], 0xFFFFFFFFu, p);
      if (o == 0xFFFFFFFFu) break;
      if (L.k[o] == kk[i]) {
        df[p] = 1;
        df[o] = 1;
        break;
      }
      h = (h + 1) & (HT - 1);
    }
  }
  __syncthreads();
  const uint64_t lt = (1ull << lane) - 1;
  uint32_t cidx[B::ITEMS], sidx[B::ITEMS], wc = 0, ws = 0, dmask = 0, smask = 0;
#pragma unroll
  for (uint32_t i = 0; i < B::ITEMS; i++) {
    const uint32_t p = strip0 + i * 64 + lane;
    const bool dup = p < S && df[p], one = p < S && !df[p];
    const uint64_t bl = __ballot(dup), bs = __ballot(one);
    cidx[i] = wc + (uint32_t)__popcll(bl & lt);
    sidx[i] = ws + (uint32_t)__popcll(bs & lt);
    wc += (uint32_t)__popcll(bl);
    ws += (uint32_t)__popcll(bs);
    dmask |= dup ? 1u << i : 0u;
    smask |= one ? 1u << i : 0u;
  }
  if (lane == 0) {
    L.wsum[wave] = wc;
    L.lw[wave] = ws;
  }
  __syncthreads();
  uint32_t wpre = 0, M = 0, spre = 0;
#pragma unroll
  for (uint32_t w = 0; w < B::WAVES; w++) {
    wpre += w < wave ? L.wsum[w] : 0u;
    spre += w < wave ? L.lw[w] : 0u;
    M += L.wsum[w];
  }
#pragma unroll
  for (uint32_t i = 0; i < B::ITEMS; i++) {
    if (!((dmask >> i) & 1u)) continue;
    const uint32_t c = wpre + cidx[i];
    L.k[c] = kk[i];
    L.v[c] = vv[i];
    L.h[c] = hh[i];
  }
  if (tid == 0) {
    if (M) L.base_pos = atomicAdd(sorted_n, M);
    L.ub = M < S ? atomicAdd(uniq_n, S - M) : 0u;
  }
  __syncthreads();
  const uint32_t ub = L.ub + spre;
#pragma unroll
  for (uint32_t i = 0; i < B::ITEMS; i++)
    if ((smask >> i) & 1u) uniq[ub + sidx[i]] = make_uint2(vv[i], kk[i]);
  if (!M) return;
  const uint32_t base = L.base_pos;
  if (M <= 64) {
    if (wave == 0) {
      const bool v = lane < M;
      const uint32_t k = v ? L.k[lane] : 0xFFFFFFFFu, x = v ? L.v[lane] : 0u, y = v ? L.h[lane] : 0u;
      uint32_t r = 0;
      for (uint32_t j = 0; j < M; j++) {
        const uint32_t kj = __shfl(k, j, 64);
        r += (kj < k || (kj == k && j < lane)) ? 1u : 0u;
      }
      if (v) {
        L.k[r] = k;
        L.v[r] = x;
        L.h[r] = y;
      }
    }
    __syncthreads();
  } else {
#pragma unroll
    for (uint32_t i = 0; i < B::ITEMS; i++) {
      const uint32_t p = strip0 + i * 64 + lane;
      kk[i] = p < M ? L.k[p] : 0xFFFFFFFFu;
      vv[i] = p < M ? L.v[p] : 0u;
      hh[i] = p < M ? L.h[p] : 0u;
    }
    __syncthreads();
    lds_sort3(L, kk, vv, hh, M);
  }
  for (uint32_t p = tid; p < M; p += B::THREADS) {
    sk[base + p] = L.k[p];
    sv[base + p] = L.v[p];
  }
  BK_STAMP(d, 3);
  bucket_segment<B, true>(L, d, M, base, sk, sh, segsum, rid, run_start, run_end, num_runs, drun);
  BK_STAMP(d, 5);
}

template <typename B>
__device__ inline bool bucket_peel(BucketLds<B>& L, uint32_t d, uint32_t S, uint32_t base, uint32_t ntiles,
                                   const uint4* __restrict__ pt,
                                   uint32_t* __restrict__ sk,
                                   uint32_t* __restrict__ sv, uint32_t* __restrict__ sh) {
  constexpr uint32_t IT = B::ITEMS;
  const uint32_t tid = threadIdx.x, lane = tid & 63, wave = tid >> 6;
  const uint64_t lt_mask = (1ull << lane) - 1;
  if (wave == 0) {
    uint32_t p[1] = {(uint32_t)(((uint64_t)(2 * lane + 1) * S) >> 7)}, j[1];
    bucket_src(ntiles, p, j);
    const uint32_t ks = pt[j[0]].x;
    uint32_t cnt = 0;
    bool first = true;
    for (uint32_t q = 0; q < 64; q++) {
      const uint32_t kq = __shfl(ks, q, 64);
      cnt += kq == ks ? 1u : 0u;
      if (q < lane && kq == ks) first = false;
    }
    const bool cand = first && cnt >= BK_HEAVY_MIN;
    const uint64_t b = __ballot(cand);
    const uint32_t rank = __popcll(b & lt_mask);
    if (cand && rank < BK_HEAVY) L.heavy[rank] = ks;
    if (lane < BK_HEAVY) {
      L.hcnt[lane] = 0;
      L.hrun[lane] = 0;
    }
    if (lane == 0) {
      L.nheavy = min((uint32_t)__popcll(b), BK_HEAVY);
      L.nlight = 0;
    }
  }
  __syncthreads();
  const uint32_t r = L.nheavy;
  if (!r) return false;
  uint32_t hk[BK_HEAVY];
#pragma unroll
  for (uint32_t c = 0; c < BK_HEAVY; c++) hk[c] = __builtin_amdgcn_readfirstlane(c < r ? L.heavy[c] : 0u);
  uint32_t kk[IT], vv[IT], hh[IT], cls[IT];
  for (uint32_t c0 = 0; c0 < S; c0 += B::CAP) {
    const uint32_t strip0 = c0 + wave * B::STRIP;
    uint32_t pp[IT], jj[IT];
#pragma unroll
    for (uint32_t i = 0; i < IT; i++) pp[i] = min(strip0 + i * 64 + lane, S - 1);
    bucket_src(ntiles, pp, jj);
#pragma unroll
    for (uint32_t i = 0; i < IT; i++) {
      const uint4 e = pt[jj[i]];
      kk[i] = e.x;
      vv[i] = e.y;
      hh[i] = e.z;
    }
    uint32_t wl = 0, lr[IT];
    uint32_t wc[BK_HEAVY];
#pragma unroll
    for (uint32_t c = 0; c < BK_HEAVY; c++) wc[c] = 0;
#pragma unroll
    for (uint32_t i = 0; i < IT; i++) {
      const bool in = strip0 + i * 64 + lane < S;
      cls[i] = in ? r : 0xFFu;
#pragma unroll
      for (uint32_t c = 0; c < BK_HEAVY; c++)
        if (in && c < r && kk[i] == hk[c]) cls[i] = c;
      const uint64_t bl = __ballot(cls[i] == r);
      lr[i] = wl + __popcll(bl & lt_mask);
      wl += __popcll(bl);
#pragma unroll
      for (uint32_t c = 0; c < BK_HEAVY; c++) wc[c] += c < r ? __popcll(__ballot(cls[i] == c)) : 0u;
    }
    if (lane == 0) {
      L.lw[wave] = wl;
#pragma unroll
      for (uint32_t c = 0; c < BK_HEAVY; c++) L.hw[wave][c] = wc[c];
    }
    __syncthreads();
    uint32_t pre = L.nlight, tl = 0;
    for (uint32_t w = 0; w < B::WAVES; w++) {
      pre += w < wave ? L.lw[w] : 0u;
      tl += L.lw[w];
    }
#pragma unroll
    for (uint32_t i = 0; i < IT; i++) {
      const uint32_t at = pre + lr[i];
      if (cls[i] == r && at < B::CAP) {
        L.k[at] = kk[i];
        L.v[at] = vv[i];
        L.h[at] = hh[i];
      }
    }
    __syncthreads();
    if (tid < BK_HEAVY) {
      uint32_t t = 0;
      for (uint32_t w = 0; w < B::WAVES; w++) t += L.hw[w][tid];
      L.hcnt[tid] += t;
    }
    if (tid == 0) L.nlight += tl;
    __syncthreads();
  }
  const uint32_t nl = L.nlight;
  if (nl > B::CAP) return false;
  BK_STAMP(d, 13);
  const uint32_t strip0 = wave * B::STRIP;
#pragma unroll
  for (uint32_t i = 0; i < IT; i++) {
    const uint32_t p = strip0 + i * 64 + lane;
    kk[i] = p < nl ? L.k[p] : 0xFFFFFFFFu;
    vv[i] = p < nl ? L.v[p] : 0u;
    hh[i] = p < nl ? L.h[p] : 0u;
  }
  if (nl) lds_sort3(L, kk, vv, hh, nl);
  if (tid < r) {
    const uint32_t K = hk[tid];
    uint32_t lo = 0, hi = nl;
    while (lo < hi) {
      const uint32_t mid = (lo + hi) >> 1;
      if (L.k[mid] < K) lo = mid + 1;
      else hi = mid;
    }
    uint32_t st = lo;
    for (uint32_t c = 0; c < r; c++) st += hk[c] < K ? L.hcnt[c] : 0u;
    L.hstart[tid] = st;
  }
#ifdef RL_BK_PROF
  __syncthreads();
  if (tid == 0) {
    uint32_t* g = g_bk_peel + d * 16;
    g[0] = r;
    g[1] = nl;
    for (uint32_t c = 0; c < BK_HEAVY; c++) {
      g[2 + c] = hk[c];
      g[6 + c] = L.hcnt[c];
      g[10 + c] = L.hstart[c];
    }
    g[14] = S;
  }
#endif
#pragma unroll
  for (uint32_t i = 0; i < IT; i++) {
    const uint32_t p = strip0 + i * 64 + lane;
    if (p < nl) {
      uint32_t at = p;
#pragma unroll
      for (uint32_t c = 0; c < BK_HEAVY; c++) at += (c < r && hk[c] < kk[i]) ? L.hcnt[c] : 0u;
      sk[base + at] = kk[i];
      sv[base + at] = vv[i];
      sh[base + at] = hh[i];
    }
  }
  __syncthreads();
  BK_STAMP(d, 14);
  for (uint32_t c0 = 0; c0 < S; c0 += B::CAP) {
    const uint32_t s0 = c0 + wave * B::STRIP;
    uint32_t pp[IT], jj[IT];
#pragma unroll
    for (uint32_t i = 0; i < IT; i++) pp[i] = min(s0 + i * 64 + lane, S - 1);
    bucket_src(ntiles, pp, jj);
#pragma unroll
    for (uint32_t i = 0; i < IT; i++) {
      const uint4 e = pt[jj[i]];
      kk[i] = e.x;
      vv[i] = e.y;
      hh[i] = e.z;
    }
    uint32_t hr[IT], wc[BK_HEAVY];
#pragma unroll
    for (uint32_t c = 0; c < BK_HEAVY; c++) wc[c] = 0;
#pragma unroll
    for (uint32_t i = 0; i < IT; i++) {
      const bool in = s0 + i * 64 + lane < S;
      cls[i] = BK_HEAVY;
#pragma unroll
      for (uint32_t c = 0; c < BK_HEAVY; c++)
        if (in && c < r && kk[i] == hk[c]) cls[i] = c;
      hr[i] = 0;
#pragma unroll
      for (uint32_t c = 0; c < BK_HEAVY; c++) {
        if (c >= r) continue;
        const uint64_t b = __ballot(cls[i] == c);
        if (cls[i] == c) hr[i] = wc[c] + __popcll(b & lt_mask);
        wc[c] += __popcll(b);
      }
    }
    if (lane == 0) {
#pragma unroll
      for (uint32_t c = 0; c < BK_HEAVY; c++) L.hw[wave][c] = wc[c];
    }
    __syncthreads();
#pragma unroll
    for (uint32_t i = 0; i < IT; i++) {
      const uint32_t c = cls[i];
      if (c < BK_HEAVY) {
        uint32_t at = L.hstart[c] + L.hrun[c] + hr[i];
        for (uint32_t w = 0; w < wave; w++) at += L.hw[w][c];
        sk[base + at] = kk[i];
        sv[base + at] = vv[i];
        sh[base + at] = hh[i];
      }
    }
    __syncthreads();
    if (tid < r) {
      uint32_t t = 0;
      for (uint32_t w = 0; w < B::WAVES; w++) t += L.hw[w][tid];
      L.hrun[tid] += t;
    }
    __syncthreads();
  }
  __threadfence_block();
  __syncthreads();
  BK_STAMP(d, 15);
  return true;
}

template <typename B>
__device__ inline void bucket_lsd(BucketLds<B>& L, uint32_t S, uint32_t base, uint32_t ntiles,
                                  const uint4* __restrict__ pt,
                                  uint32_t* __restrict__ sk,
                                  uint32_t* __restrict__ sv, uint32_t* __restrict__ sh, uint32_t* __restrict__ ht,
                                  uint32_t* __restrict__ segsum, uint32_t* __restrict__ rid) {
  constexpr uint32_t IT = B::ITEMS;
  const uint32_t tid = threadIdx.x, lane = tid & 63, wave = tid >> 6;
  uint32_t kk[IT], vv[IT], hh[IT], pos[IT];
  for (uint32_t j = tid; j < 3 * 256; j += B::THREADS) (&L.roff[0][0])[j] = 0;
  __syncthreads();
  for (uint32_t c0 = 0; c0 < S; c0 += B::CAP) {
    uint32_t pp[IT], jj[IT];
#pragma unroll
    for (uint32_t i = 0; i < IT; i++) pp[i] = min(c0 + i * B::THREADS + tid, S - 1);
    bucket_src(ntiles, pp, jj);
#pragma unroll
    for (uint32_t i = 0; i < IT; i++) kk[i] = pt[jj[i]].x;
#pragma unroll
    for (uint32_t i = 0; i < IT; i++) {
      if (c0 + i * B::THREADS + tid < S) {
        atomicAdd(&L.roff[0][kk[i] & 255u], 1u);
        atomicAdd(&L.roff[1][(kk[i] >> 8) & 255u], 1u);
        atomicAdd(&L.roff[2][(kk[i] >> 16) & 63u], 1u);
      }
    }
  }
  __syncthreads();
  for (uint32_t pass = 0; pass < 3; pass++) {
    const uint32_t v = tid < 256 ? L.roff[pass][tid] : 0u;
    const uint32_t excl = scan256(v, L.wsum, nullptr);
    if (tid < 256) L.roff[pass][tid] = excl;
  }
  __syncthreads();
  for (uint32_t pass = 0; pass < 3; pass++) {
    const uint32_t* ik = pass == 1 ? sk + base : rid + base;
    const uint32_t* iv = pass == 1 ? sv + base : segsum + base;
    const uint32_t* ih = pass == 1 ? sh + base : ht + base;
    uint32_t* ok = pass == 1 ? rid + base : sk + base;
    uint32_t* ov = pass == 1 ? segsum + base : sv + base;
    uint32_t* oh = pass == 1 ? ht + base : sh + base;
    for (uint32_t c0 = 0; c0 < S; c0 += B::CAP) {
      const uint32_t strip0 = c0 + wave * B::STRIP;
      uint32_t pp[IT], jj[IT];
#pragma unroll
      for (uint32_t i = 0; i < IT; i++) pp[i] = min(strip0 + i * 64 + lane, S - 1);
      if (pass == 0) {
        bucket_src(ntiles, pp, jj);
      } else {
#pragma unroll
        for (uint32_t i = 0; i < IT; i++) jj[i] = pp[i];
      }
      if (pass == 0) {
#pragma unroll
        for (uint32_t i = 0; i < IT; i++) {
          const uint4 e = pt[jj[i]];
          kk[i] = e.x;
          vv[i] = e.y;
          hh[i] = e.z;
        }
      } else {
#pragma unroll
        for (uint32_t i = 0; i < IT; i++) {
          kk[i] = ik[jj[i]];
          vv[i] = iv[jj[i]];
          hh[i] = ih[jj[i]];
        }
      }
#pragma unroll
      for (uint32_t i = 0; i < IT; i++)
        if (strip0 + i * 64 + lane >= S) kk[i] = 0xFFFFFFFFu;
      if (tid < 256) L.base[tid] = L.roff[pass][tid];
      if (pass < 2) bucket_rank<B, 8>(L, kk, strip0, S, 8 * pass, false, pos);
      else bucket_rank<B, 6>(L, kk, strip0, S, 16, false, pos);
      if (tid < 256) L.roff[pass][tid] += L.dtot[tid];
#pragma unroll
      for (uint32_t i = 0; i < IT; i++) {
        if (strip0 + i * 64 + lane < S) {
          ok[pos[i]] = kk[i];
          ov[pos[i]] = vv[i];
          oh[pos[i]] = hh[i];
        }
      }
    }
    __threadfence_block();
    __syncthreads();
  }
}

__device__ inline uint32_t wave_sum32(uint32_t x) {
#pragma unroll
  for (uint32_t m = 32; m >= 1; m >>= 1) x += __shfl_xor(x, m, 64);
  return x;
}

#ifndef RL_DPP_SCAN
#define RL_DPP_SCAN 1
#endif
__device__ __attribute__((always_inline)) inline uint32_t wave_incl_add(uint32_t x) {
#if RL_DPP_SCAN
  x += (uint32_t)__builtin_amdgcn_update_dpp(0, (int)x, 0x111, 0xf, 0xf, false);
  x += (uint32_t)__builtin_amdgcn_update_dpp(0, (int)x, 0x112, 0xf, 0xf, false);
  x += (uint32_t)__builtin_amdgcn_update_dpp(0, (int)x, 0x114, 0xf, 0xf, false);
  x += (uint32_t)__builtin_amdgcn_update_dpp(0, (int)x, 0x118, 0xf, 0xf, false);
  x += (uint32_t)__builtin_amdgcn_update_dpp(0, (int)x, 0x142, 0xa, 0xf, false);
  x += (uint32_t)__builtin_amdgcn_update_dpp(0, (int)x, 0x143, 0xc, 0xf, false);
#else
  const uint32_t lane = __lane_id();
#pragma unroll
  for (uint32_t off = 1; off < 64; off <<= 1) {
    const uint32_t y = __shfl_up(x, off, 64);
    if (lane >= off) x += y;
  }
#endif
  return x;
}

__device__ inline void big_chunk_load(const BigMeta& M, uint32_t j, uint32_t ntiles, const uint4* __restrict__ pt,
                                      uint32_t (&kk)[BkSmall::ITEMS], uint32_t (&vv)[BkSmall::ITEMS],
                                      uint32_t (&hh)[BkSmall::ITEMS], uint32_t (&cls)[BkSmall::ITEMS], bool values) {
  using B = BkSmall;
  const uint32_t lane = threadIdx.x & 63, s0 = j * BIG_CHUNK + (threadIdx.x >> 6) * B::STRIP;
  uint32_t pp[B::ITEMS], jj[B::ITEMS];
#pragma unroll
  for (uint32_t i = 0; i < B::ITEMS; i++) pp[i] = min(s0 + i * 64 + lane, M.S - 1);
  bucket_src(ntiles, pp, jj);
#pragma unroll
  for (uint32_t i = 0; i < B::ITEMS; i++) {
    const uint4 e = pt[jj[i]];
    kk[i] = e.x;
    hh[i] = e.z;
    vv[i] = values ? e.y : 0u;
  }
#pragma unroll
  for (uint32_t i = 0; i < B::ITEMS; i++) {
    cls[i] = s0 + i * 64 + lane < M.S ? M.r : 0xFFu;
#pragma unroll
    for (uint32_t c = 0; c < BK_HEAVY; c++)
      if (cls[i] != 0xFFu && c < M.r && kk[i] == M.heavy[c]) cls[i] = c;
  }
}

__global__ __launch_bounds__(BkSmall::THREADS) void k_big_count(const uint4* __restrict__ pt,
                                                                const uint32_t* __restrict__ info, uint32_t ntiles,
                                                                const BigMeta* __restrict__ meta,
                                                                const uint32_t* __restrict__ work,
                                                                const uint32_t* work_n, uint32_t* __restrict__ cnt,
                                                                const uint32_t* err) {
  using B = BkSmall;
  __shared__ BucketLds<B> L;
  if (*err) return;
  const uint32_t tid = threadIdx.x, lane = tid & 63, wave = tid >> 6, nw = *work_n;
  for (uint32_t it = blockIdx.x; it < nw; it += gridDim.x) {
    const uint32_t w = work[it];
    const BigMeta M = meta[w >> 16];
    bucket_setup(L, info, ntiles, M.d);
    uint32_t kk[B::ITEMS], vv[B::ITEMS], hh[B::ITEMS], cls[B::ITEMS];
    big_chunk_load(M, w & 0xFFFFu, ntiles, pt, kk, vv, hh, cls, false);
    uint32_t nl = 0, nc[BK_HEAVY], hs[BK_HEAVY];
#pragma unroll
    for (uint32_t c = 0; c < BK_HEAVY; c++) nc[c] = hs[c] = 0;
#pragma unroll
    for (uint32_t i = 0; i < B::ITEMS; i++) {
      const uint32_t hv = hh[i] > 1 ? hh[i] : 1u;
      nl += cls[i] == M.r ? 1u : 0u;
#pragma unroll
      for (uint32_t c = 0; c < BK_HEAVY; c++) {
        nc[c] += cls[i] == c ? 1u : 0u;
        hs[c] += cls[i] == c ? hv : 0u;
      }
    }
    nl = wave_sum32(nl);
#pragma unroll
    for (uint32_t c = 0; c < BK_HEAVY; c++) {
      nc[c] = wave_sum32(nc[c]);
      hs[c] = wave_sum32(hs[c]);
    }
    if (lane == 0) {
      L.lw[wave] = nl;
#pragma unroll
      for (uint32_t c = 0; c < BK_HEAVY; c++) {
        L.hw[wave][c] = nc[c];
        L.hsw[wave][c] = hs[c];
      }
    }
    __syncthreads();
    if (tid < BIG_CNT) {
      uint32_t t = 0;
      for (uint32_t v = 0; v < B::WAVES; v++)
        t += tid == 0 ? L.lw[v] : tid <= BK_HEAVY ? L.hw[v][tid - 1] : L.hsw[v][tid - 1 - BK_HEAVY];
      cnt[(size_t)it * BIG_CNT + tid] = t;
    }
    __syncthreads();
  }
}

__global__ __launch_bounds__(BkSmall::THREADS) void k_big_place(
    const uint4* __restrict__ pt,
    const uint32_t* __restrict__ info, uint32_t ntiles, const BigMeta* __restrict__ meta,
    const uint32_t* __restrict__ work, const uint32_t* work_n, const uint32_t* __restrict__ cnt,
    uint32_t* __restrict__ sk, uint32_t* __restrict__ sv, uint32_t* __restrict__ sh, uint32_t* __restrict__ segsum,
    uint32_t* __restrict__ rid, uint32_t* __restrict__ run_start, uint32_t* __restrict__ run_end,
    uint32_t* __restrict__ drun, const uint32_t* err) {
  using B = BkSmall;
  __shared__ BucketLds<B> L;
  if (*err) return;
  const uint32_t tid = threadIdx.x, lane = tid & 63, wave = tid >> 6, nw = *work_n;
  const uint64_t lt_mask = (1ull << lane) - 1;
  for (uint32_t it = blockIdx.x; it < nw; it += gridDim.x) {
    const uint32_t w = work[it], j = w & 0xFFFFu;
    const BigMeta M = meta[w >> 16];
    if (tid < BIG_CNT) L.acc[tid] = 0;
    uint32_t tot[BIG_CNT];
#pragma unroll
    for (uint32_t k = 0; k < BIG_CNT; k++) tot[k] = 0;
    __syncthreads();
    for (uint32_t t = tid; t < M.nchunks; t += B::THREADS) {
      const uint32_t* ct = cnt + (size_t)(M.item0 + t) * BIG_CNT;
#pragma unroll
      for (uint32_t k = 0; k < BIG_CNT; k++) {
        const uint32_t v = ct[k];
        tot[k] += v;
        if (t < j) atomicAdd(&L.acc[k], v);
      }
    }
#pragma unroll
    for (uint32_t k = 0; k < 1 + BK_HEAVY; k++) tot[k] = block_sum(L, tot[k]);
    bucket_setup(L, info, ntiles, M.d);
    const uint32_t NL = tot[0];
    if (NL > BIG_LIGHT_CAP) continue;
    uint32_t hstart[BK_HEAVY];
    uint32_t st = NL;
#pragma unroll
    for (uint32_t c = 0; c < BK_HEAVY; c++) {
      hstart[c] = st;
      st += c < M.r ? tot[1 + c] : 0u;
    }
    if (j == 0 && tid < M.r) {
      run_start[M.rb_heavy + tid] = M.base + hstart[tid];
      run_end[M.rb_heavy + tid] = M.base + hstart[tid] + tot[1 + tid];
      drun[M.db_heavy + tid] = M.rb_heavy + tid;
    }
    uint32_t kk[B::ITEMS], vv[B::ITEMS], hh[B::ITEMS], cls[B::ITEMS];
    big_chunk_load(M, j, ntiles, pt, kk, vv, hh, cls, true);
    uint32_t rk[B::ITEMS], hp[B::ITEMS], wl = 0, wc[BK_HEAVY], wh[BK_HEAVY];
#pragma unroll
    for (uint32_t c = 0; c < BK_HEAVY; c++) wc[c] = wh[c] = 0;
#pragma unroll
    for (uint32_t i = 0; i < B::ITEMS; i++) {
      const uint64_t bl = __ballot(cls[i] == M.r);
      rk[i] = wl + __popcll(bl & lt_mask);
      wl += __popcll(bl);
      hp[i] = 0;
      const uint32_t hv = hh[i] > 1 ? hh[i] : 1u;
#pragma unroll
      for (uint32_t c = 0; c < BK_HEAVY; c++) {
        if (c >= M.r) continue;
        const bool mine = cls[i] == c;
        const uint64_t b = __ballot(mine);
        const uint32_t x = wave_incl_add(mine ? hv : 0u);
        if (mine) {
          rk[i] = wc[c] + __popcll(b & lt_mask);
          hp[i] = wh[c] + x;
        }
        wc[c] += __popcll(b);
        wh[c] += (uint32_t)__builtin_amdgcn_readlane((int)x, 63);
      }
    }
    if (lane == 0) {
      L.lw[wave] = wl;
#pragma unroll
      for (uint32_t c = 0; c < BK_HEAVY; c++) {
        L.hw[wave][c] = wc[c];
        L.hsw[wave][c] = wh[c];
      }
    }
    __syncthreads();
    uint32_t lpre = L.acc[0], cpre[BK_HEAVY], hpre[BK_HEAVY];
#pragma unroll
    for (uint32_t c = 0; c < BK_HEAVY; c++) {
      cpre[c] = L.acc[1 + c];
      hpre[c] = L.acc[1 + BK_HEAVY + c];
    }
    for (uint32_t v = 0; v < wave; v++) {
      lpre += L.lw[v];
#pragma unroll
      for (uint32_t c = 0; c < BK_HEAVY; c++) {
        cpre[c] += L.hw[v][c];
        hpre[c] += L.hsw[v][c];
      }
    }
#pragma unroll
    for (uint32_t i = 0; i < B::ITEMS; i++) {
      const uint32_t c = cls[i];
      if (c == M.r) {
        const uint32_t at = M.base + lpre + rk[i];
        sk[at] = kk[i];
        sv[at] = vv[i];
        sh[at] = hh[i];
      } else if (c < BK_HEAVY) {
        uint32_t cp = 0, hq = 0, hs0 = 0;
#pragma unroll
        for (uint32_t q = 0; q < BK_HEAVY; q++)
          if (q == c) {
            cp = cpre[q];
            hq = hpre[q];
            hs0 = hstart[q];
          }
        const uint32_t at = M.base + hs0 + cp + rk[i];
        sk[at] = kk[i];
        sv[at] = vv[i];
        segsum[at] = hq + hp[i];
        rid[at] = M.rb_heavy + c;
      }
    }
    __syncthreads();
  }
}

__global__ __launch_bounds__(BkBig::THREADS) void k_bucket_big(
    const uint4* __restrict__ pt,
    const uint32_t* __restrict__ info, uint32_t ntiles, uint32_t* __restrict__ sk, uint32_t* __restrict__ sv,
    uint32_t* __restrict__ sh, uint32_t* __restrict__ ht, uint32_t* __restrict__ segsum, uint32_t* __restrict__ rid,
    uint32_t* __restrict__ run_start, uint32_t* __restrict__ run_end, unsigned long long* num_runs,
    uint32_t* __restrict__ drun, const BigMeta* __restrict__ meta, const uint32_t* big_n,
    const uint32_t* __restrict__ cnt, const uint32_t* err) {
  using B = BkBig;
  __shared__ BucketLds<B> L;
  if (*err) return;
  const uint32_t tid = threadIdx.x, lane = tid & 63, wave = tid >> 6, nb = *big_n;
  for (uint32_t bi = blockIdx.x; bi < nb; bi += gridDim.x) {
    const BigMeta M = meta[bi];
    const uint32_t d = M.d, S = M.S, base = M.base;
    BK_STAMP(d, 0);
    uint32_t nl = 0;
    for (uint32_t t = tid; t < M.nchunks; t += B::THREADS) nl += cnt[(size_t)(M.item0 + t) * BIG_CNT];
    nl = block_sum(L, nl);
    if (M.r && nl <= BIG_LIGHT_CAP) {
      uint32_t kk[B::ITEMS], vv[B::ITEMS], hh[B::ITEMS];
      const uint32_t strip0 = wave * B::STRIP;
#pragma unroll
      for (uint32_t i = 0; i < B::ITEMS; i++) {
        const uint32_t p = min(strip0 + i * 64 + lane, nl ? nl - 1 : 0u);
        kk[i] = sk[base + p];
        vv[i] = sv[base + p];
        hh[i] = sh[base + p];
      }
#pragma unroll
      for (uint32_t i = 0; i < B::ITEMS; i++)
        if (strip0 + i * 64 + lane >= nl) kk[i] = 0xFFFFFFFFu;
      if (nl) {
        lds_sort3(L, kk, vv, hh, nl);
#pragma unroll
        for (uint32_t i = 0; i < B::ITEMS; i++) {
          const uint32_t p = strip0 + i * 64 + lane;
          if (p < nl) {
            sk[base + p] = kk[i];
            sv[base + p] = vv[i];
          }
        }
        __syncthreads();
        bucket_segment<B, true>(L, d, nl, base, sk, sh, segsum, rid, run_start, run_end, num_runs, drun);
      }
    } else {
      if (tid < M.r) run_start[M.rb_heavy + tid] = run_end[M.rb_heavy + tid] = 0;
      bucket_setup(L, info, ntiles, d);
      BK_STAMP(d, 1);
      if (!bucket_peel(L, d, S, base, ntiles, pt, sk, sv, sh))
        bucket_lsd(L, S, base, ntiles, pt, sk, sv, sh, ht, segsum, rid);
      bucket_segment<B, false>(L, d, S, base, sk, sh, segsum, rid, run_start, run_end, num_runs, drun);
    }
    BK_STAMP(d, 7);
    __syncthreads();
  }
}

#ifndef RL_RC_CHUNK
#define RL_RC_CHUNK 256
#endif
constexpr uint32_t RC_CHUNK = RL_RC_CHUNK;

template <typename Pred>
__device__ __attribute__((always_inline)) inline uint32_t block_compact(uint32_t lo, uint32_t hi, uint32_t* list,
                                                                        uint32_t* count, Pred pred) {
  const uint32_t lane = threadIdx.x & 63;
  if (threadIdx.x == 0) *count = 0;
  __syncthreads();
  for (uint32_t i0 = lo; i0 < hi; i0 += blockDim.x) {
    const uint32_t i = i0 + threadIdx.x;
    const bool take = i < hi && pred(i);
    const uint64_t m = __ballot(take);
    uint32_t base = 0;
    if (lane == 0 && m) base = atomicAdd(count, (uint32_t)__popcll(m));
    base = __shfl(base, 0);
    if (take) list[base + __popcll(m & ((1ull << lane) - 1))] = i;
  }
  __syncthreads();
  return *count;
}

constexpr uint32_t SPLIT_POS_OTHER = 0xFFu, SPLIT_POS_SKIP = 0xFEu, SPLIT_POS_NOWVAR = 1u << 16;
constexpr uint32_t SPLIT_ULIST = 1024;

__global__ __launch_bounds__(256) void k_run_check(BatchDev b, SRec rec_s,
                                                   const uint32_t* __restrict__ skeys,
                                                   const uint32_t* __restrict__ rid,
                                                   const uint32_t* __restrict__ run_start,
                                                   uint32_t* __restrict__ run_end,
                                                   uint32_t* __restrict__ run_flags, uint32_t* __restrict__ defer,
                                                   uint32_t* defer_n, const uint32_t* err,
                                                   const unsigned long long* num_runs, unsigned long long* split,
                                                   const uint32_t* sorted_n, uint32_t* __restrict__ pos_unit,
                                                   uint32_t* __restrict__ pos_hits, uint2* __restrict__ uniq,
                                                   uint32_t* uniq_n, uint32_t* long_runs, uint32_t* __restrict__ keys0) {
  __shared__ uint32_t s_list[RC_CHUNK], s_cnt;
  if (blockIdx.x == 0 && threadIdx.x == 0) {
    split[0] = 0;
    split[1] = *num_runs;
    long_runs[0] = 0;
  }
  if (*err) return;
  const uint32_t sn = *sorted_n;
  for (uint32_t q0 = blockIdx.x * RC_CHUNK; q0 < min(blockIdx.x * RC_CHUNK + RC_CHUNK, sn); q0 += blockDim.x) {
    const uint32_t q = q0 + threadIdx.x;
    const uint32_t k = q < sn ? skeys[q] : 0u;
    const bool one = q < sn && (q == 0 || skeys[q - 1] != k) && (q + 1 >= sn || skeys[q + 1] != k);
    const uint64_t m = __ballot(one);
    if (!m) continue;
    const uint32_t lane = threadIdx.x & 63, leader = (uint32_t)__ffsll((unsigned long long)m) - 1;
    uint32_t at = 0;
    if (lane == leader) at = atomicAdd(uniq_n, (uint32_t)__popcll(m));
    at = __shfl(at, leader, 64) + (uint32_t)__popcll(m & ((1ull << lane) - 1));
    if (one) uniq[at] = make_uint2(rec_s.sv[q], k);
  }
  const uint32_t lo = max(blockIdx.x * RC_CHUNK, 1u), hi = min(blockIdx.x * RC_CHUNK + RC_CHUNK, sn);
  if (lo >= hi) return;
  const uint32_t cnt = block_compact(lo, hi, s_list, &s_cnt, [&](uint32_t q) { return skeys[q - 1] == skeys[q]; });
  refine_totals(b);
  Rec* rec = const_cast<Rec*>(rec_s.rec);
#pragma unroll 1
  for (uint32_t j = threadIdx.x; j < cnt; j += blockDim.x) {
    const uint32_t q = s_list[j];
    const uint32_t r = rid[q];
    const uint32_t p = run_start[r];
    const uint32_t eq = rec_s.sv[q], ep = rec_s.sv[p];
    const Rec x = rec[eq], y = rec[ep];
    const bool skip = (rec_flags(x) | rec_flags(y)) & FLAG_SKIP;
    const bool same_stem = !skip && x.hlo == y.hlo && (x.lu & 0xFFFFu) == (y.lu & 0xFFFFu) &&
                           key_equal(key_of(b, x), key_of(b, y));
    if (!same_stem && !skip && q == p + 1 && run_end[r] == q + 1) {
      run_end[r] = p;
      const uint32_t at = atomicAdd(uniq_n, 2u);
      uniq[at] = make_uint2(ep, skeys[q]);
      uniq[at + 1] = make_uint2(eq, skeys[q]);
      continue;
    }
    keys0[eq] = KEY_DUP;
    if (q == p + 1) keys0[ep] = KEY_DUP;
    const bool same = same_stem && rec_unit(x) == rec_unit(y);
    pos_unit[q] = (rec_unit(x) << 8) | (skip ? SPLIT_POS_SKIP : !same_stem ? SPLIT_POS_OTHER : 0u) |
                  (x.now != y.now ? SPLIT_POS_NOWVAR : 0u);
    pos_hits[q] = x.hits > 1 ? x.hits : 1u;
    uint32_t f = 0;
    if (!same)
      f = RUN_MULTI | (same_stem ? RUN_UNITS | ((1u << (rec_unit(x) - 1)) << RUN_UMASK_SHIFT) : RUN_STEMS);
    if (x.now != y.now) {
      const uint32_t d = div_of(rec_unit(x));
      f |= (same && x.now / d != y.now / d) ? RUN_SLOW | RUN_NOWVAR : RUN_NOWVAR;
    }
    uint64_t pend = __ballot(f != 0);
    while (pend) {
      const uint32_t leader = (uint32_t)(__ffsll((unsigned long long)pend) - 1);
      const uint32_t rr = __shfl(r, leader, 64);
      const bool mine = f != 0 && r == rr;
      const uint64_t mm = __ballot(mine);
      constexpr uint32_t kBits[] = {RUN_MULTI, RUN_UNITS, RUN_STEMS, RUN_SLOW, RUN_NOWVAR,
                                    1u << RUN_UMASK_SHIFT, 2u << RUN_UMASK_SHIFT, 4u << RUN_UMASK_SHIFT,
                                    8u << RUN_UMASK_SHIFT};
      uint32_t fo = 0;
#pragma unroll
      for (uint32_t bi = 0; bi < sizeof(kBits) / sizeof(kBits[0]); bi++)
        if (__ballot(mine && (f & kBits[bi]))) fo |= kBits[bi];
      if ((threadIdx.x & 63u) == leader &&
          (__hip_atomic_load(&run_flags[rr], __ATOMIC_RELAXED, __HIP_MEMORY_SCOPE_AGENT) & fo) != fo) {
        const uint32_t old = atomicOr(&run_flags[rr], fo);
        if ((fo & RUN_MULTI) && !(old & RUN_MULTI)) defer[atomicAdd(defer_n, 1u)] = rr;
      }
      pend &= ~mm;
    }
  }
}

#ifndef RL_SPLIT_BLOCKS
#define RL_SPLIT_BLOCKS 128
#endif
constexpr uint32_t SPLIT_CAP = 1024, SPLIT_MAXG = 8, SPLIT_BLOCKS = RL_SPLIT_BLOCKS;
constexpr uint32_t DEFER_DONE = 0xFFFFFFFFu;
constexpr uint32_t SPLIT_BAD = 0xFFu;

struct SplitPlan {
  uint8_t ug[SPLIT_MAXG][4];
  uint8_t head[SPLIT_MAXG];
  uint8_t ng[SPLIT_MAXG];
  uint8_t fam[SPLIT_MAXG];
  uint8_t alias[SPLIT_MAXG];
  uint8_t gmask[SPLIT_MAXG];
  uint32_t G, any_alias;
};

__device__ inline uint32_t split_plan(SplitPlan& S, uint32_t NF, const uint32_t* fmask, const uint32_t* fnow,
                                      const uint32_t* fnv, int per_second) {
  uint32_t G = 0;
  S.any_alias = 0;
  for (uint32_t f = 0; f < NF; f++) {
    const uint32_t m = fmask[f];
    S.head[f] = (uint8_t)G;
    if (__popc(m) == 1) {
      if (G >= SPLIT_MAXG) return SPLIT_BAD;
      for (uint32_t u = 0; u < 4; u++) S.ug[f][u] = (uint8_t)G;
      S.fam[G] = (uint8_t)f;
      S.alias[G] = 0;
      S.gmask[G] = (uint8_t)m;
      S.ng[f] = 1;
      G++;
      continue;
    }
    if (fnv[f]) return SPLIT_BAD;
    const uint32_t now = fnow[f], first = G;
    uint32_t w[4];
    for (uint32_t u = 0; u < 4; u++) {
      S.ug[f][u] = SPLIT_BAD;
      if (!((m >> u) & 1)) continue;
      w[u] = now - now % div_of(u + 1);
      const bool cls = per_second && u == 0;
      uint32_t g = SPLIT_BAD;
      for (uint32_t v = 0; v < u; v++) {
        if (!((m >> v) & 1) || w[v] != w[u]) continue;
        if ((per_second && v == 0) != cls) return SPLIT_BAD;
        g = S.ug[f][v];
      }
      if (g == SPLIT_BAD) {
        if (G >= SPLIT_MAXG) return SPLIT_BAD;
        g = G++;
        S.fam[g] = (uint8_t)f;
        S.alias[g] = 1;
        S.gmask[g] = 0;
      }
      S.ug[f][u] = (uint8_t)g;
      S.gmask[g] |= (uint8_t)(1u << u);
    }
    S.ng[f] = (uint8_t)(G - first);
    S.any_alias = 1;
  }
  S.G = G;
  return G;
}

__device__ inline uint32_t split_group_flags(const SplitPlan& S, uint32_t g, uint32_t fl) {
  if (!S.alias[g]) return fl;
  const uint32_t f = S.fam[g];
  uint32_t x = RUN_ALIAS | ((uint32_t)S.gmask[g] << RUN_UMASK_SHIFT);
  if (S.head[f] == g) x |= RUN_AHEAD | ((uint32_t)S.ng[f] << RUN_G_SHIFT);
  return x;
}

constexpr uint32_t SPLIT_UNROLL = 8;
#ifndef RL_SPLIT_ST
#define RL_SPLIT_ST 16
#endif
constexpr uint32_t SPLIT_ST = RL_SPLIT_ST;
#ifndef RL_SPLIT_LONG_THREADS
#define RL_SPLIT_LONG_THREADS 1024
#endif
#ifndef RL_SPLIT_LONG_ST
#define RL_SPLIT_LONG_ST 8
#endif
#ifndef RL_SPLIT_LONG_OCC
#define RL_SPLIT_LONG_OCC 4
#endif
#ifndef RL_SPLIT_LONG_BLOCKS
#define RL_SPLIT_LONG_BLOCKS 8
#endif
#ifndef RL_SPLIT_THREADS
#define RL_SPLIT_THREADS 256
#endif
constexpr uint32_t SPLIT_THREADS = RL_SPLIT_THREADS;

struct UniqList {
  uint2* list;
  uint32_t* n;
  const uint32_t* skeys;
  uint32_t* keys0;
  __device__ inline void single(uint32_t e, uint32_t p) const {
    const uint32_t k = skeys[p];
    keys0[e] = k;
    list[atomicAdd(n, 1u)] = make_uint2(e, k);
  }
};

template <uint32_t NT, uint32_t ST>
__device__ __attribute__((always_inline)) inline void split_long_body(uint32_t j, uint32_t r, uint32_t p, uint32_t L, BatchDev b,
                                                          SRec rec_s, uint32_t* svals, uint32_t* segsum,
                                                          uint32_t* __restrict__ rid, uint32_t* __restrict__ run_start,
                                                          uint32_t* __restrict__ run_end,
                                                          uint32_t* __restrict__ run_flags, uint32_t* __restrict__ defer,
                                                          unsigned long long* num_runs, unsigned long long* split,
                                                          uint32_t* __restrict__ drun, uint32_t drun_cap, uint32_t* grp,
                                                          uint32_t* rank, uint32_t* __restrict__ pos_hits,
                                                          uint32_t* __restrict__ hnew, int per_second, uint32_t rfl,
                                                          const UniqList& uq) {
  constexpr uint32_t NW = NT / 64;
  __shared__ uint32_t s_wc[NW][SPLIT_MAXG], s_wh[NW][SPLIT_MAXG], s_wp[NW][SPLIT_MAXG], s_ws[NW];
  __shared__ uint32_t s_cnt[SPLIT_MAXG], s_base[SPLIT_MAXG], s_id[SPLIT_MAXG], s_fl[SPLIT_MAXG], s_off[SPLIT_MAXG];
  __shared__ uint32_t s_lnow[SPLIT_MAXG], s_lunit[SPLIT_MAXG], s_fmask[SPLIT_MAXG], s_fnv[SPLIT_MAXG];
  __shared__ uint32_t s_bad, s_lead, s_nu, s_ul[SPLIT_ULIST];
  __shared__ SplitPlan s_plan;
  const uint32_t tid = threadIdx.x, lane = tid & 63, wv = tid >> 6;
  const uint64_t lt = lane ? (~0ull >> (64 - lane)) : 0ull;
  Rec* rec = const_cast<Rec*>(rec_s.rec);
  const uint32_t* sv = rec_s.sv;
  {
#ifdef RL_SPLIT_PROF
    uint64_t ts[8];
    ts[0] = wall_clock64();
#define SPLIT_STAMP(i) ts[i] = wall_clock64()
#else
#define SPLIT_STAMP(i)
#endif
    __syncthreads();
    if (tid == 0) {
      s_bad = 0;
      s_nu = 0;
    }
    if (tid < SPLIT_MAXG) {
      s_fmask[tid] = 0;
      s_fnv[tid] = 0;
    }
    __syncthreads();
    uint32_t NF = 0;
    if (tid == 0) {
      const Rec y = rec[sv[p]];
      pos_hits[p] = y.hits > 1 ? y.hits : 1u;
      if ((rfl & (RUN_UNITS | RUN_STEMS)) == RUN_UNITS) {
        grp[p] = rec_unit(y) << 8;
        s_lnow[0] = y.now;
        s_lunit[0] = rec_unit(y);
        s_fnv[0] = (rfl & RUN_NOWVAR) ? 1u : 0u;
        s_fmask[0] = ((rfl >> RUN_UMASK_SHIFT) & 0xFu) | (1u << (rec_unit(y) - 1));
      }
    }
    if ((rfl & (RUN_UNITS | RUN_STEMS)) == RUN_UNITS) {
      NF = 1;
    } else {
      uint32_t fm0 = 0, nv0 = 0;
      for (uint32_t k = tid + 1; k < L; k += NT) {
        const uint32_t v = grp[p + k], lo = v & 0xFFu;
        if (lo == SPLIT_POS_SKIP) {
          s_bad = 1;
        } else if (lo == 0) {
          fm0 |= 1u << (((v >> 8) & 0xFFu) - 1);
          nv0 |= (v & SPLIT_POS_NOWVAR) ? 1u : 0u;
        } else {
          const uint32_t j = atomicAdd(&s_nu, 1u);
          if (j < SPLIT_ULIST) s_ul[j] = k;
        }
      }
      if (tid == 0) {
        const Rec y = rec[sv[p]];
        if ((y.lu >> 24) & FLAG_SKIP) s_bad = 1;
        grp[p] = rec_unit(y) << 8;
        s_lnow[0] = y.now;
        s_lunit[0] = rec_unit(y);
        fm0 |= 1u << (rec_unit(y) - 1);
      }
      if (fm0) atomicOr(&s_fmask[0], fm0);
      if (nv0) s_fnv[0] = 1;
      NF = 1;
      __syncthreads();
      const uint32_t nu = s_nu;
      for (; nu <= SPLIT_ULIST;) {
        if (tid == 0) s_lead = 0xFFFFFFFFu;
        __syncthreads();
        for (uint32_t j = tid; j < nu; j += NT)
          if ((grp[p + s_ul[j]] & 0xFFu) == 0xFFu) atomicMin(&s_lead, s_ul[j]);
        __syncthreads();
        const uint32_t ld = s_lead;
        if (ld == 0xFFFFFFFFu || s_bad || NF == SPLIT_MAXG) break;
        const Rec y = rec[sv[p + ld]];
        const Key ky = key_of(b, y);
        if (tid == 0) {
          s_lnow[NF] = y.now;
          s_lunit[NF] = rec_unit(y);
        }
        uint32_t fm = 0, nv = 0;
        for (uint32_t j = tid; j < nu; j += NT) {
          const uint32_t k = s_ul[j];
          if ((grp[p + k] & 0xFFu) != 0xFFu) continue;
          const Rec x = rec[sv[p + k]];
          if (x.hlo != y.hlo || (x.lu & 0xFFFFu) != (y.lu & 0xFFFFu)) continue;
          if (!key_equal(key_of(b, x), ky)) {
            s_bad = 1;
          } else {
            grp[p + k] = NF | (rec_unit(x) << 8);
            fm |= 1u << (rec_unit(x) - 1);
            nv |= x.now != y.now;
          }
        }
        if (fm) atomicOr(&s_fmask[NF], fm);
        if (nv) s_fnv[NF] = 1;
        NF++;
        __syncthreads();
      }
      for (; nu > SPLIT_ULIST;) {
        if (tid == 0) s_lead = 0xFFFFFFFFu;
        __syncthreads();
        for (uint32_t k = tid; k < L; k += NT)
          if ((grp[p + k] & 0xFFu) == 0xFFu) {
            atomicMin(&s_lead, k);
            break;
          }
        __syncthreads();
        const uint32_t ld = s_lead;
        if (ld == 0xFFFFFFFFu || s_bad || NF == SPLIT_MAXG) break;
        const Rec y = rec[sv[p + ld]];
        const Key ky = key_of(b, y);
        if (tid == 0) {
          s_lnow[NF] = y.now;
          s_lunit[NF] = rec_unit(y);
        }
        uint32_t fm = 0, nv = 0;
        for (uint32_t k0 = tid; k0 < L; k0 += NT * SPLIT_UNROLL) {
          Rec x[SPLIT_UNROLL];
          bool act[SPLIT_UNROLL];
#pragma unroll
          for (uint32_t u = 0; u < SPLIT_UNROLL; u++) {
            const uint32_t k = k0 + u * NT;
            act[u] = k < L && (grp[p + k] & 0xFFu) == 0xFFu;
            if (act[u]) x[u] = rec[sv[p + k]];
          }
#pragma unroll
          for (uint32_t u = 0; u < SPLIT_UNROLL; u++) {
            if (!act[u] || x[u].hlo != y.hlo || (x[u].lu & 0xFFFFu) != (y.lu & 0xFFFFu)) continue;
            if (!key_equal(key_of(b, x[u]), ky)) {
              s_bad = 1;
            } else {
              grp[p + k0 + u * NT] = NF | (rec_unit(x[u]) << 8);
              fm |= 1u << (rec_unit(x[u]) - 1);
              nv |= x[u].now != y.now;
            }
// ... 310 lines not shown
      s_fnv[tid] = 0;
    }
    for (uint32_t k = tid; k < L; k += SPLIT_THREADS) {
      const uint32_t e = rec_s.sv[p + k];
      const Rec x = rec[e];
      s_e[k] = e;
      s_hlo[k] = x.hlo;
      s_lu[k] = x.lu;
      s_now[k] = x.now;
      s_h[k] = x.hits > 1 ? x.hits : 1u;
      s_g[k] = 0xFF;
    }
    __syncthreads();
    for (uint32_t k = tid; k < L; k += SPLIT_THREADS)
      if ((s_lu[k] >> 24) & FLAG_SKIP) s_bad = 1;
    uint32_t NF = 0;
    for (;;) {
      if (tid == 0) s_lead = 0xFFFFFFFFu;
      __syncthreads();
      for (uint32_t k = tid; k < L; k += SPLIT_THREADS)
        if (s_g[k] == 0xFF) atomicMin(&s_lead, k);
      __syncthreads();
      const uint32_t ld = s_lead;
      if (ld == 0xFFFFFFFFu || s_bad || NF == SPLIT_MAXG) break;
      const Rec y = rec[s_e[ld]];
      const Key ky = key_of(b, y);
      if (tid == 0) {
        s_lnow[NF] = y.now;
        s_lunit[NF] = rec_unit(y);
      }
      for (uint32_t k = tid; k < L; k += SPLIT_THREADS) {
        if (s_g[k] != 0xFF || s_hlo[k] != y.hlo || (s_lu[k] & 0xFFFFu) != (y.lu & 0xFFFFu)) continue;
        if (!key_equal(key_of(b, rec[s_e[k]]), ky)) {
          s_bad = 1;
        } else {
          atomicOr(&s_fmask[NF], 1u << (((s_lu[k] >> 16) & 0xFFu) - 1));
          if (s_now[k] != y.now) s_fnv[NF] = 1;
          s_g[k] = (uint8_t)NF;
        }
      }
      NF++;
      __syncthreads();
    }
    if (s_lead != 0xFFFFFFFFu) s_bad = 1;
    __syncthreads();
    if (s_bad) continue;
    if (tid == 0 && split_plan(s_plan, NF, s_fmask, s_lnow, s_fnv, per_second) == SPLIT_BAD) s_bad = 1;
    __syncthreads();
    const uint32_t G = s_plan.G;
    if (s_bad || (G < 2 && !s_plan.any_alias)) continue;
    for (uint32_t k = tid; k < L; k += SPLIT_THREADS) s_g[k] = s_plan.ug[s_g[k]][((s_lu[k] >> 16) & 0xFFu) - 1];
    __syncthreads();
    if (tid < 64) {
      uint32_t cnt[SPLIT_MAXG];
#pragma unroll
      for (uint32_t g = 0; g < SPLIT_MAXG; g++) cnt[g] = 0;
      const uint64_t lt = lane ? (~0ull >> (64 - lane)) : 0ull;
      for (uint32_t c0 = 0; c0 < L; c0 += 64) {
        const uint32_t k = c0 + lane;
        const uint32_t gk = k < L ? s_g[k] : 0xFFu;
#pragma unroll
        for (uint32_t g = 0; g < SPLIT_MAXG; g++) {
          const uint64_t m = __ballot(gk == g);
          if (gk == g) s_pos[k] = (uint16_t)(cnt[g] + __popcll(m & lt));
          cnt[g] += __popcll(m);
        }
      }
      if (lane == 0) {
        uint32_t acc = 0;
#pragma unroll
        for (uint32_t g = 0; g < SPLIT_MAXG; g++) {
          s_cnt[g] = cnt[g];
          s_base[g] = acc;
          s_fl[g] = 0;
          acc += cnt[g];
        }
        uint32_t nd2 = 0;
        for (uint32_t g = 1; g < G; g++) nd2 += (cnt[g] >= 2 || s_plan.alias[g]) ? 1u : 0u;
        const unsigned long long add = ((unsigned long long)nd2 << 32) | (unsigned long long)(G - 1);
        const unsigned long long rs = atomicAdd(&split[0], add), base = split[1];
        const bool room = (uint32_t)(base >> 32) + (uint32_t)(rs >> 32) + nd2 <= drun_cap &&
                          (uint32_t)base + (uint32_t)rs + (G - 1) <= b.n;
        unsigned long long old = 0;
        if (!room) s_bad = 1;
        else old = atomicAdd(num_runs, add);
        if (!s_bad) {
          s_id[0] = r;
          uint32_t di = (uint32_t)(old >> 32);
          for (uint32_t g = 1; g < G; g++) {
            s_id[g] = (uint32_t)old + g - 1;
            if (cnt[g] >= 2 || s_plan.alias[g]) drun[di++] = s_id[g];
          }
        }
      }
    }
    __syncthreads();
    if (s_bad) continue;
    for (uint32_t k = tid; k < L; k += SPLIT_THREADS) {
      const uint32_t g = s_g[k], np = s_base[g] + s_pos[k];
      svals[p + np] = s_e[k];
      rid[p + np] = s_id[g];
      s_nh[np] = s_h[k];
      s_ng[np] = (uint8_t)g;
      if (!s_plan.alias[g]) {
        const uint32_t f = s_plan.fam[g], d = div_of(s_lunit[f]);
        if (s_now[k] != s_lnow[f])
          atomicOr(&s_fl[g], s_now[k] / d != s_lnow[f] / d ? RUN_SLOW | RUN_NOWVAR : RUN_NOWVAR);
        if (s_cnt[g] == 1) {
          uq.single(s_e[k], p);
        }
      }
    }
    __syncthreads();
    if (tid < 64) {
      uint32_t carry = 0;
      for (uint32_t c0 = 0; c0 < L; c0 += 64) {
        const uint32_t k = c0 + lane;
        const bool in = k < L;
        uint32_t v = in ? s_nh[k] : 0u;
        bool f = in && (k == 0 || s_ng[k - 1] != s_ng[k]);
#pragma unroll
        for (uint32_t off = 1; off < 64; off <<= 1) {
          const uint32_t y = __shfl_up(v, off, 64);
          const bool yf = __shfl_up(f ? 1 : 0, off, 64) != 0;
          if (lane >= off) {
            if (!f) v += y;
            f = f || yf;
          }
        }
        if (!f) v += carry;
        if (in) segsum[p + k] = v;
        carry = __shfl(v, 63, 64);
      }
    }
    if (tid < G) {
      const uint32_t id = s_id[tid];
      run_start[id] = p + s_base[tid];
      run_end[id] = p + s_base[tid] + s_cnt[tid];
      run_flags[id] = split_group_flags(s_plan, tid, s_fl[tid]);
    }
    if (tid == 0) defer[j] = DEFER_DONE;
  }
}

#ifndef RL_UNIQ_DENSE
#define RL_UNIQ_DENSE 3
#endif
__device__ __attribute__((always_inline)) inline void unique_body(uint32_t blk, BatchDev b, TableDev t, Params P, const Rec* __restrict__ rec,
                                                const uint32_t* __restrict__ keys0,
                                                const uint2* __restrict__ uniq, const uint32_t* uniq_n,
                                                unsigned long long* __restrict__ res,
                                                uint32_t* __restrict__ defer1, uint32_t* defer1_n,
                                                unsigned long long* stats, unsigned long long* stripes, uint32_t* err,
                                                uint32_t* errs, int restore, const uint32_t* errb_prev) {
  __shared__ uint32_t s_err, s_nu, s_cnt, s_list[256];
  if (threadIdx.x == 0) {
    s_err = __hip_atomic_load(err, __ATOMIC_RELAXED, __HIP_MEMORY_SCOPE_AGENT) | (errb_prev ? *errb_prev : 0u);
    s_nu = *uniq_n;
  }
  __syncthreads();
  const uint32_t nu = s_nu;
  const bool by_list = (uint64_t)nu * 4 < (uint64_t)b.n * RL_UNIQ_DENSE;
  const uint32_t lo = blk * 256, hi = min(lo + 256, by_list ? nu : b.n);
  if (s_err || lo >= hi) return;
  refine_totals(b);
  uint32_t* ferr = P.isolate ? errs : err;
  const bool use_lds = !restore && b.n_rules <= LDS_RULES;
  stats_block_begin(use_lds, b.n_rules);
  StatAcc acc{use_lds, stats};
  LaneStats L;
  L.reset();
  auto single = [&](uint32_t i) { return keys0[i] != KEY_DUP && !((rec[i].lu >> 24) & FLAG_SKIP); };
  bool act;
  uint32_t i, key = 0;
  if (by_list) {
    const uint32_t pos = lo + threadIdx.x;
    const uint2 ent = pos < hi ? uniq[pos] : make_uint2(0u, 0u);
    i = ent.x;
    key = ent.y;
    act = pos < hi && single(i);
  } else {
    const uint32_t i0 = lo + threadIdx.x;
    const bool own = i0 < hi && single(i0);
    if (__syncthreads_count(own) >= 192) {
      act = own;
      i = i0;
    } else {
      const uint32_t cnt = block_compact(lo, hi, s_list, &s_cnt, single);
      act = threadIdx.x < cnt;
      i = act ? s_list[threadIdx.x] : 0u;
    }
    if (act) key = keys0[i];
  }
  if (act) {
    const Rec x = rec[i];
    {
      const uint64_t h0 = ((uint64_t)key << 32) | x.hlo;
      const uint32_t u0 = rec_unit(x);
      SlotImg im;
      load_img_lo(&t.slots[h0 >> t.shift], im);
      const Key k0 = key_of(b, x);
      bool ins = false, ok = true;
      const uint32_t tg0 = slot_tag(h0, u0);
      const int64_t s0 = find_slot_img(t, h0, tg0, k0, u0, &ins, im, ferr);
      if (s0 < 0) {
        ok = false;
      } else if (im.flags() & SLOT_EXACT) {
        ok = false;
      } else if (ins) {
        for (uint32_t u = 1; u <= 4; u++) {
          bool dummy;
          const int64_t so = u == u0 ? -1 : find_slot(t, h0, slot_tag(h0, u), k0, u, false, &dummy, ferr);
          if (so >= 0) {
            t.slots[so].flags |= SLOT_EXACT;
            ok = false;
          }
        }
        if (!ok) t.slots[s0].flags |= SLOT_EXACT;
      }
      if (ok) {
        replay_simple(SRec{rec, nullptr}, nullptr, res, t, P, nullptr, 0, 1, 0, s0, im.cur(), im.ring(), tg0, x, i,
                      L, acc, ferr,
                      restore);
      } else if (s0 == SLOT_TABLE_FULL || s0 == SLOT_ARENA_FULL) {
        if (P.isolate) res[i] = pack_fail(slot_fail_status(s0));
      } else {
        defer1[atomicAdd(defer1_n, 1u)] = i;
      }
    }
  }
  if (!restore) wave_flush(L, acc);
  stats_block_end(use_lds, b.n_rules, stripes);
}

__device__ inline void fail_range(unsigned long long* res, const uint32_t* svals, uint32_t p, uint32_t end,
                                  uint32_t st) {
  for (uint32_t q = p; q < end; q++) res[svals[q]] = pack_fail(st);
}

struct AliasGroup {
  uint32_t id, p, end, mask, w;
};

#ifndef RL_ALIAS_ONE_WALK
#define RL_ALIAS_ONE_WALK 1
#endif
constexpr uint32_t UNIT_WALK_ENDED = 0x10u;
__device__ inline uint32_t find_unit_slots(const TableDev& t, uint64_t hs, const Key& stem, int64_t sidx[4], Win c[4],
                                           uint32_t chain[4]) {
  uint64_t i = hs >> t.shift;
  uint32_t found = 0;
  SlotImg im;
  for (uint32_t p = 0; p < t.max_probe && found != 0xFu; p++, i = (i + 1) & t.mask) {
    load_img_lo(&t.slots[i], im);
    const uint32_t st = im.tag();
    if (st == TAG_EMPTY) return found | UNIT_WALK_ENDED;
    const uint32_t u = im.unit();
    if (u < 1 || u > 4 || ((found >> (u - 1)) & 1) || st != slot_tag(hs, u) || !img_key_equal(im, stem, t.arena))
      continue;
    sidx[u - 1] = (int64_t)i;
    c[u - 1] = im.cur();
    chain[u - 1] = im.ring();
    found |= 1u << (u - 1);
  }
  return found;
}

#ifndef RL_ALIAS_NOINLINE
#define RL_ALIAS_NOINLINE 0
#endif
#if RL_ALIAS_NOINLINE
#define RL_ALIAS_ATTR __attribute__((noinline))
#else
#define RL_ALIAS_ATTR inline
#endif
__device__ RL_ALIAS_ATTR bool alias_setup(const TableDev& t, const Params& P, SRec rec_s, const uint32_t* __restrict__ rid,
                                   const uint32_t* __restrict__ run_start, const uint32_t* __restrict__ run_end,
                                   uint32_t* __restrict__ run_flags, uint4* __restrict__ run_state,
                                   uint4* __restrict__ run_alias, uint32_t* __restrict__ run_f,
                                   uint32_t* __restrict__ fast_blk, unsigned long long* __restrict__ res,
                                   const uint32_t* __restrict__ svals, uint32_t* ferr, uint32_t r, uint32_t fl,
                                   uint32_t u0, uint64_t hs, const Key& stem, uint32_t now) {
#ifdef RL_NO_ALIAS
  return true;
#endif
#ifdef RL_ALIAS_PROF
  uint64_t ta[4];
  ta[0] = wall_clock64();
#define ALIAS_STAMP(i) ta[i] = wall_clock64()
#else
#define ALIAS_STAMP(i)
#endif
  AliasGroup A[4];
  uint32_t G = 1, M;
  A[0].id = r;
  A[0].p = run_start[r];
  A[0].end = run_end[r];
  if (fl & RUN_AHEAD) {
    G = (fl >> RUN_G_SHIFT) & 0xFFu;
    A[0].mask = (fl >> RUN_UMASK_SHIFT) & 0xFu;
    for (uint32_t g = 1; g < G && g < 4; g++) {
      const uint32_t id = rid[A[g - 1].end];
      A[g].id = id;
      A[g].p = run_start[id];
      A[g].end = run_end[id];
      A[g].mask = (run_flags[id] >> RUN_UMASK_SHIFT) & 0xFu;
    }
    if (G > 4) return true;
  } else {
    A[0].mask = 1u << (u0 - 1);
  }
  M = 0;
  for (uint32_t g = 0; g < G; g++) {
    const uint32_t d = div_of(__ffs(A[g].mask));
    A[g].w = now - now % d;
// ... 480 lines not shown
      ce[0] = end;
      for (uint32_t g = 1; g < G; g++) {
        const uint32_t id = rid[ce[g - 1]];
        cq[g] = run_start[id];
        ce[g] = run_end[id];
        um |= (run_flags[id] >> RUN_UMASK_SHIFT) & 0xFu;
      }
      const Rec y = rec_s[p];
      stem_exact(t, P, res, L, acc, ferr, restore, ((uint64_t)key << 32) | y.hlo, key_at(b, rec_s, p), um,
                 [&](auto&& f) {
                   for (;;) {
                     uint32_t bg = MG, be = 0xFFFFFFFFu;
                     for (uint32_t g = 0; g < G; g++)
                       if (cq[g] < ce[g] && svals[cq[g]] < be) {
                         be = svals[cq[g]];
                         bg = g;
                       }
                     if (bg == MG) break;
                     f(load_elem(rec_s[cq[bg]], be, restore));
                     cq[bg]++;
                   }
                 });
      continue;
    }
    uint32_t ng = 0;
    for (uint32_t q = p; q < end; q++) {
      const Rec x = rec_s[q];
      if (rec_flags(x) & FLAG_SKIP) {
        grp[q] = GRP_NONE;
        continue;
      }
      const Key kx = key_of(b, x);
      uint32_t g = 0;
      for (; g < ng; g++) {
        const Rec y = rec_s[lead[p + g]];
        if (y.hlo == x.hlo && rec_len(y) == rec_len(x) && key_equal(key_of(b, y), kx)) break;
      }
      if (g == ng) {
        lead[p + ng] = q;
        gmask[p + ng] = 0;
        ng++;
      }
      grp[q] = g;
      gmask[p + g] |= (uint8_t)(1u << (rec_unit(x) - 1));
    }
    for (uint32_t g = 0; g < ng; g++) {
      const uint32_t q0 = lead[p + g], um = gmask[p + g];
      const Rec y = rec_s[q0];
      const Key stem = key_at(b, rec_s, q0);
      const uint64_t hs = ((uint64_t)key << 32) | y.hlo;
      bool simple = false;
      int64_t s0 = -1;
      if (__popc(um) == 1) {
        const uint32_t u0 = __ffs(um);
        bool ins;
        s0 = find_slot(t, hs, slot_tag(hs, u0), stem, u0, true, &ins, ferr);
        if (s0 < 0) {
          if (P.isolate) fail_group(res, svals, grp, q0, end, g, slot_fail_status(s0));
          continue;
        }
        if (!(t.slots[s0].flags & SLOT_EXACT)) {
          simple = true;
          if (ins) {
            for (uint32_t u = 1; u <= 4 && simple; u++) {
              bool dummy;
              if (u != u0 && find_slot(t, hs, slot_tag(hs, u), stem, u, false, &dummy, ferr) >= 0) simple = false;
            }
          }
        }
      }
      if (simple) {
        replay_simple(rec_s, svals, res, t, P, grp, q0, end, g, s0, t.slots[s0].cur, t.slots[s0].ring, slot_tag(hs, __ffs(um)), y,
                      svals[q0], L, acc, ferr,
                      restore);
        continue;
      }
      stem_exact(t, P, res, L, acc, ferr, restore, hs, stem, um, [&](auto&& f) {
        for (uint32_t q = q0; q < end; q++)
          if (grp[q] == g) f(load_elem(rec_s[q], svals[q], restore));
      });
    }
  }
  for (uint32_t di = blk * 256 + threadIdx.x; di < s_n1; di += nblk * 256) {
    const uint32_t e = defer1[di];
    const Rec x = rec_s.rec[e];
    const uint64_t hs = ((uint64_t)keys0[e] << 32) | x.hlo;
    stem_exact(t, P, res, L, acc, ferr, restore, hs, key_of(b, x), 1u << (rec_unit(x) - 1),
               [&](auto&& f) { f(load_elem(x, e, restore)); });
  }
  if (!restore) wave_flush(L, acc);
  stats_block_end(use_lds, b.n_rules, stripes);
}

__device__ __attribute__((always_inline)) inline void late_scan(uint32_t k, uint32_t F, BatchDev b, TableDev t, Params P,
                                                   SRec rec_s, const uint32_t* __restrict__ svals,
                                                   unsigned long long* __restrict__ res,
                                                   const uint32_t* __restrict__ segsum, const uint32_t* __restrict__ rid,
                                                   const uint32_t* __restrict__ run_start,
                                                   const uint32_t* __restrict__ run_end,
                                                   const uint32_t* __restrict__ run_flags,
                                                   const uint4* __restrict__ run_state,
                                                   const uint4* __restrict__ run_alias, const uint32_t* __restrict__ run_f,
                                                   unsigned long long* stats, unsigned long long* stripes,
                                                   const uint32_t* err, const uint32_t* __restrict__ fast_blk,
                                                   const uint32_t* sorted_n, uint32_t* hint) {
  __shared__ uint32_t s_w[256], s_word[256], s_cnt;
  const uint32_t nw = (b.n + 256u * 32u - 1) / (256u * 32u);
  for (uint32_t w0 = k * 256; w0 < nw; w0 += F * 256) {
    __syncthreads();
    if (threadIdx.x == 0) s_cnt = 0;
    __syncthreads();
    const uint32_t w = w0 + threadIdx.x;
    const uint32_t word = w < nw ? fast_blk[w] : 0u;
    if (word) {
      const uint32_t at = atomicAdd(&s_cnt, 1u);
      s_w[at] = w;
      s_word[at] = word;
    }
    __syncthreads();
    const uint32_t cnt = s_cnt;
    for (uint32_t j = 0; j < cnt; j++) {
      uint32_t bits = s_word[j];
      while (bits) {
        const uint32_t blk = s_w[j] * 32 + (uint32_t)(__ffs(bits) - 1);
        bits &= bits - 1;
        fast_emit_body(blk, sorted_n, b.n_rules, t, P, rec_s, svals, res, segsum, rid, run_start, run_end, run_flags,
                       run_state, run_alias, run_f, stats, stripes, err, fast_blk, hint);
      }
    }
  }
}

#ifndef RL_KT_UNIQ_FIRST
#define RL_KT_UNIQ_FIRST 0
#endif
#ifndef RL_KTABLE_WAVES
#define RL_KTABLE_WAVES 5
#endif
__global__ __launch_bounds__(256, RL_KTABLE_WAVES) void k_table(uint32_t g_runs, BatchDev b, TableDev t, Params P, SRec rec_s,
                                               const uint32_t* __restrict__ skeys,
                                               const uint32_t* __restrict__ svals,
                                               unsigned long long* __restrict__ res,
                                               const uint32_t* __restrict__ run_start,
                                               const uint32_t* __restrict__ run_end, uint32_t* __restrict__ run_flags,
                                               uint4* __restrict__ run_state, uint4* __restrict__ run_alias,
                                               const uint32_t* __restrict__ rid, uint32_t* __restrict__ run_f,
                                               const unsigned long long* num_runs, const uint32_t* __restrict__ drun,
                                               uint32_t* __restrict__ defer2, uint32_t* defer2_n,
                                               const uint32_t* __restrict__ keys0, uint32_t* __restrict__ defer1,
                                               uint32_t* defer1_n, unsigned long long* stats,
                                               unsigned long long* stripes, uint32_t* err, uint32_t* errs, int restore,
                                               uint32_t* __restrict__ fast_blk, const uint2* __restrict__ uniq,
                                               const uint32_t* uniq_n, unsigned long long* __restrict__ kt,
                                               const uint32_t* errb_prev) {

  if (kt && threadIdx.x == 0) kt[2 * blockIdx.x] = wall_clock64();
  if (errb_prev && blockIdx.x == 0 && threadIdx.x == 0) {
    const uint32_t p = *errb_prev;
    if (p) atomicOr(err, p);
  }
#if RL_KT_UNIQ_FIRST
  const uint32_t g_uniq = gridDim.x - g_runs;
  if (blockIdx.x >= g_uniq)
    runs_body(blockIdx.x - g_uniq, b, t, P, rec_s, skeys, svals, res, run_start, run_end, run_flags, run_state,
              run_alias, rid, run_f, num_runs, drun, defer2, defer2_n, stats, stripes, err, errs, restore, fast_blk,
              errb_prev);
  else
    unique_body(blockIdx.x, b, t, P, rec_s.rec, keys0, uniq, uniq_n, res, defer1, defer1_n, stats, stripes, err, errs,
                restore, errb_prev);
#else
  if (blockIdx.x < g_runs)
    runs_body(blockIdx.x, b, t, P, rec_s, skeys, svals, res, run_start, run_end, run_flags, run_state, run_alias, rid,
              run_f, num_runs, drun, defer2, defer2_n, stats, stripes, err, errs, restore, fast_blk, errb_prev);
  else
    unique_body(blockIdx.x - g_runs, b, t, P, rec_s.rec, keys0, uniq, uniq_n, res, defer1, defer1_n, stats, stripes,
                err, errs, restore, errb_prev);
#endif
  if (kt && threadIdx.x == 0) kt[2 * blockIdx.x + 1] = wall_clock64();
}

#ifndef RL_LATE_OCC
#define RL_LATE_OCC 8
#endif
__global__ __launch_bounds__(256, RL_LATE_OCC) void k_late(BatchDev b, TableDev t, Params P, SRec rec_s,
                                                 const uint32_t* __restrict__ skeys, const uint32_t* __restrict__ svals,
                                                 unsigned long long* __restrict__ res,
                                                 const uint32_t* __restrict__ run_start,
                                                 const uint32_t* __restrict__ run_end,
                                                 const uint32_t* __restrict__ defer, const uint32_t* defer_n,
                                                 const uint32_t* __restrict__ defer2, const uint32_t* defer2_n,
                                                 uint32_t* __restrict__ grp, uint32_t* __restrict__ lead,
                                                 uint8_t* __restrict__ gmask, const uint32_t* __restrict__ keys0,
                                                 const uint32_t* __restrict__ defer1, const uint32_t* defer1_n,
                                                 const uint32_t* __restrict__ segsum, const uint32_t* __restrict__ rid,
                                                 const uint32_t* __restrict__ run_flags,
                                                 const uint4* __restrict__ run_state,
                                                 const uint4* __restrict__ run_alias, const uint32_t* __restrict__ run_f,
                                                 unsigned long long* stats, unsigned long long* stripes, uint32_t* err,
                                                 uint32_t* errs, int restore, const uint32_t* __restrict__ fast_blk,
                                                 const uint32_t* sorted_n, uint32_t* hint, int scan) {
  if (blockIdx.x < RUNS_GENERAL_LATE_BLOCKS) {
    general_body(blockIdx.x, RUNS_GENERAL_LATE_BLOCKS, b, t, P, rec_s, skeys, svals, res, run_start, run_end, defer,
                 defer_n, defer2, defer2_n, grp, lead, gmask, keys0, defer1, defer1_n, run_flags, rid, stats, stripes,
                 err, errs, restore);
  } else if (restore) {
  } else if (!scan) {
    for (uint32_t blk = blockIdx.x - RUNS_GENERAL_LATE_BLOCKS; blk * 256 < b.n;
         blk += gridDim.x - RUNS_GENERAL_LATE_BLOCKS)
      fast_emit_body(blk, sorted_n, b.n_rules, t, P, rec_s, svals, res, segsum, rid, run_start, run_end, run_flags,
                     run_state, run_alias, run_f, stats, stripes, err, fast_blk, hint);
  } else {
    late_scan(blockIdx.x - RUNS_GENERAL_LATE_BLOCKS, gridDim.x - RUNS_GENERAL_LATE_BLOCKS, b, t, P, rec_s, svals, res,
              segsum, rid, run_start, run_end, run_flags, run_state, run_alias, run_f, stats, stripes, err, fast_blk,
              sorted_n, hint);
  }
}

__global__ __launch_bounds__(256) void k_b_begin(const uint32_t* __restrict__ erra, uint32_t* errb,
                                                 const uint32_t* errb_prev,
                                                 uint32_t* __restrict__ defer_n, uint32_t* __restrict__ defer1_n,
                                                 unsigned long long* __restrict__ stats, uint32_t m,
                                                 uint32_t* __restrict__ fast_blk, uint32_t nw,
                                                 const unsigned long long* log_ctr,
                                                 unsigned long long* __restrict__ log_epoch) {
  const uint32_t i = blockIdx.x * 256 + threadIdx.x;
  if (log_ctr && i < LOG_PARTS)
    log_epoch[i] = __hip_atomic_load(log_ctr + (size_t)i * LOG_CTR_STRIDE, __ATOMIC_RELAXED, __HIP_MEMORY_SCOPE_AGENT);
  if (i == 0) {
    *errb = (errb_prev ? *errb_prev : 0u) | *erra;
    *defer_n = 0;
    *defer1_n = 0;
  }
  for (uint32_t j = i; j < m; j += gridDim.x * 256) stats[j] = 0;
  for (uint32_t j = i; j < nw; j += gridDim.x * 256) fast_blk[j] = 0;
}

__global__ __launch_bounds__(256) void k_finish(const unsigned long long* __restrict__ res, uint32_t n, OutDev o,
                                                unsigned long long* __restrict__ stripes, uint32_t n_fold,
                                                const uint32_t* err, unsigned long long* lc_ctr,
                                                const unsigned long long* __restrict__ kt, uint32_t kt_n,
                                                unsigned long long* kt_acc, const OwnChunk own) {
  const uint32_t i = blockIdx.x * 256 + threadIdx.x;
  if (kt && blockIdx.x == 0) {
    __shared__ unsigned long long s_lo[256], s_hi[256];
    unsigned long long lo = ~0ull, hi = 0;
    for (uint32_t j = threadIdx.x; j < kt_n; j += 256) {
      lo = min(lo, kt[2 * j]);
      hi = max(hi, kt[2 * j + 1]);
    }
    s_lo[threadIdx.x] = lo;
    s_hi[threadIdx.x] = hi;
    __syncthreads();
    for (uint32_t w = 128; w; w >>= 1) {
      if (threadIdx.x < w) {
        s_lo[threadIdx.x] = min(s_lo[threadIdx.x], s_lo[threadIdx.x + w]);
        s_hi[threadIdx.x] = max(s_hi[threadIdx.x], s_hi[threadIdx.x + w]);
      }
      __syncthreads();
    }
    if (threadIdx.x == 0 && s_hi[0] > s_lo[0]) {
      atomicAdd(&kt_acc[0], s_hi[0] - s_lo[0]);
      atomicAdd(&kt_acc[1], 1ull);
    }
  }
  const bool ok = *err == 0;
  const uint32_t m = n_fold * RL_NUM_STATS;
  if (i < m) {
    unsigned long long s = 0;
    for (uint32_t k = 0; k < STAT_STRIPES; k++) {
      s += stripes[(size_t)k * m + i];
      stripes[(size_t)k * m + i] = 0;
    }
    if (ok) o.stats[i] += s;
  }
  bool hit = false;
  if (ok && i < n) {
    const unsigned long long v = res[i];
    if (o.code) {
      o.code[i] = (uint8_t)res_code(v);
      o.rem[i] = res_rem(v);
      o.reset[i] = res_reset(v);
      if (o.status) o.status[i] = (uint8_t)res_status(v);
    }
    hit = res_lc_hit(v);
  }
  if (own.code && i < n && i - own.lo < own.n) {
    const unsigned long long v = ok ? res[i] : pack_fail(err_status(*err));
    const uint32_t e = own.idx[i - own.lo];
    own.code[e] = (uint8_t)res_code(v);
    own.rem[e] = res_rem(v);
    if (own.reset) own.reset[e] = res_reset(v);
    if (own.status) own.status[e] = (uint8_t)res_status(v);
    else if (own.src_err && res_status(v)) atomicOr(own.src_err, status_err(res_status(v)));
  }
  if (lc_ctr && ok) {
    const unsigned long long w = __ballot(hit);
    if ((threadIdx.x & 63u) == 0 && w) atomicAdd(&lc_ctr[1], (unsigned long long)__popcll(w));
    if (i == 0) atomicAdd(&lc_ctr[0], (unsigned long long)n);
  }
}

template <typename F>
__device__ inline void chain_walk(const TableDev& t, uint32_t si, const Slot& s, F f) {
  uint32_t ptr = s.ring, tprev = s.cur.ws, saved = LOG_NONE, power = 1, lam = 0;
  for (uint32_t hops = 0; ptr != LOG_NONE && hops < LOG_MAX_HOPS && ptr != saved; hops++) {
    const uint32_t pos = ptr & LOG_POS_MASK;
    if (pos >= t.log_cap) return;
    if (++lam == power) {
      saved = ptr;
      power <<= 1;
      lam = 0;
    }
    const LogEnt& e = t.log[(size_t)(ptr >> LOG_POS_BITS) * t.log_cap + pos];
    if (e.slot != si || e.tag != s.tag || e.t_app > tprev) return;
    if (!f(e.w, hops)) return;
    tprev = e.t_app;
    ptr = e.prev;
  }
}

__global__ __launch_bounds__(256) void k_lc_count(const TableDev t, uint64_t nslots, uint32_t now,
                                                  unsigned long long* out) {
  uint32_t live = 0;
  for (uint64_t i = blockIdx.x * 256ull + threadIdx.x; i < nslots; i += (uint64_t)gridDim.x * 256) {
    const Slot& s = t.slots[i];
    if (s.tag < 2) continue;
    live += s.cur.ws != WS_INVALID && now < s.cur.lc;
    chain_walk(t, (uint32_t)i, s, [&](const Win& w, uint32_t at) {
      if (w.ws == WS_INVALID || !(now < w.lc)) return true;
      bool newest = true;
      chain_walk(t, (uint32_t)i, s, [&](const Win& v, uint32_t at2) {
        if (at2 >= at) return false;
        if (v.ws == w.ws) newest = false;
        return newest;
      });
      live += newest;
      return true;
    });
  }
  if (live) atomicAdd(out, (unsigned long long)live);
}

__device__ inline bool win_alive(const Win& w, uint32_t now) {
  return w.ws != WS_INVALID && (now <= w.expire || now < w.lc);
}

__global__ __launch_bounds__(256) void k_sweep(TableDev t, uint64_t nslots, uint32_t now, unsigned long long* evicted) {
  uint32_t local = 0;
  for (uint64_t i = blockIdx.x * 256ull + threadIdx.x; i < nslots; i += (uint64_t)gridDim.x * 256) {
    Slot* s = &t.slots[i];
    if (s->tag < 2) continue;
    bool alive = win_alive(s->cur, now);
    if (!alive)
      chain_walk(t, (uint32_t)i, *s, [&](const Win& w, uint32_t) {
        alive = win_alive(w, now);
        return !alive;
      });
    if (alive) continue;
    s->tag = TAG_TOMB;
    s->ring = LOG_NONE;
    local++;
  }
  if (local) atomicAdd(evicted, (unsigned long long)local);
}

__global__ __launch_bounds__(256) void k_arena_compact(Slot* slots, uint64_t nslots, const uint8_t* __restrict__ from,
                                                       uint8_t* __restrict__ to, unsigned long long* used16) {
  for (uint64_t i = blockIdx.x * 256ull + threadIdx.x; i < nslots; i += (uint64_t)gridDim.x * 256) {
    Slot* s = &slots[i];
    if (s->tag < 2 || s->key_len <= KEY_IN) continue;
    uint32_t* sd = reinterpret_cast<uint32_t*>(s);
    const uint32_t n16 = (s->key_len - KEY_SPLIT + 15) / 16;
    const unsigned long long off = atomicAdd(used16, (unsigned long long)n16);
    const uint4* src = reinterpret_cast<const uint4*>(from + (size_t)sd[SLOT_EXT_DW] * 16);
    uint4* dst = reinterpret_cast<uint4*>(to + off * 16);
    for (uint32_t k = 0; k < n16; k++) dst[k] = src[k];
    sd[SLOT_EXT_DW] = (uint32_t)off;
  }
}

__global__ __launch_bounds__(256) void k_table_info(const Slot* slots, uint64_t nslots, unsigned long long* out) {
  uint32_t live = 0, tomb = 0, exact = 0, hist = 0;
  for (uint64_t i = blockIdx.x * 256ull + threadIdx.x; i < nslots; i += (uint64_t)gridDim.x * 256) {
    const uint32_t tg = slots[i].tag;
    if (tg == TAG_TOMB) tomb++;
    else if (tg >= 2) {
      live++;
      exact += (slots[i].flags & SLOT_EXACT) != 0;
      hist += slots[i].ring != LOG_NONE;
    }
  }
  if (live) atomicAdd(&out[0], (unsigned long long)live);
  if (tomb) atomicAdd(&out[1], (unsigned long long)tomb);
  if (exact) atomicAdd(&out[2], (unsigned long long)exact);
  if (hist) atomicAdd(&out[3], (unsigned long long)hist);
}

__global__ __launch_bounds__(256) void k_debug_keys(BatchDev b, uint8_t* out, uint32_t* klen) {
  const uint32_t i = blockIdx.x * 256 + threadIdx.x;
  if (i >= b.n) return;
  const uint32_t s0 = b.off[i], len = b.off[i + 1] - s0;
  uint8_t* dst = out + s0 + 24ull * i;
  for (uint32_t j = 0; j < len; j++) dst[j] = b.stem[s0 + j];
  const uint32_t now = (uint32_t)b.now[b.req[i]];
  const uint32_t d = div_of(b.unit[i]);
  uint32_t ws = now / d * d;
  uint8_t tmp[12];
  uint32_t nd = 0;
  do { tmp[nd++] = (uint8_t)('0' + ws % 10); ws /= 10; } while (ws);
  for (uint32_t j = 0; j < nd; j++) dst[len + j] = tmp[nd - 1 - j];
  klen[i] = len + nd;
}

__global__ __launch_bounds__(256) void k_debug_decide(uint32_t n, const uint32_t* before, const uint32_t* after,
                                                      const uint8_t* lc_hit, const uint32_t* hits,
                                                      const uint32_t* limit, const uint8_t* unit,
                                                      const uint8_t* flags, const int64_t* now, float ratio,
                                                      int lc_en, uint8_t* code, uint32_t* rem, uint32_t* reset,
                                                      unsigned long long* deltas, uint8_t* lc_set) {
  const uint32_t i = blockIdx.x * 256 + threadIdx.x;
  if (i >= n) return;
  const bool shadow = flags[i] & RL_FLAG_SHADOW;
  const Decision r = decide(before[i], after[i], lc_hit[i] != 0, hits[i], limit[i], ratio, shadow, lc_en != 0);
  code[i] = r.code;
  rem[i] = r.remaining;
  const uint32_t d = div_of(unit[i]);
  reset[i] = d - (uint32_t)(now[i] % d);
  unsigned long long* s = deltas + (size_t)i * RL_NUM_STATS;
  s[RL_STAT_TOTAL_HITS] = 0;
  s[RL_STAT_OVER_LIMIT] = r.d_over;
  s[RL_STAT_NEAR_LIMIT] = r.d_near;
  s[RL_STAT_OVER_LIMIT_WITH_LOCAL_CACHE] = r.d_lc;
  s[RL_STAT_WITHIN_LIMIT] = r.d_within;
  s[RL_STAT_SHADOW_MODE] = r.d_shadow;
  lc_set[i] = r.set_lc;
}

static inline uint32_t cdiv(uint64_t a, uint64_t b) { return (uint32_t)((a + b - 1) / b); }

void launch_stage_a(const BatchDev& b, const Scratch& s, int isolate, int per_second, hipStream_t st,
                    hipEvent_t* ev, uint32_t* long_hint, bool long_kernel, uint32_t* big_hint, bool big_full) {
  const uint32_t g0 = cdiv(b.n > b.n_req ? b.n : b.n_req, 256);
  if (ev) (void)hipEventRecord(ev[0], st);
  if (g0)
    k_prepare<<<g0, 256, 0, st>>>(b, s.rec, s.keys[0], s.err, s.errs, isolate, s.time_floor, s.defer_n, s.big_n,
                                  s.work_n, s.run_flags, s.runs64, s.hit_a, s.res, s.sorted_n, s.uniq_n);
  if (ev) (void)hipEventRecord(ev[1], st);
  const uint32_t ptiles = cdiv(b.n, PART_TILE);
  if (b.n)
    k_part<<<ptiles, 256, 0, st>>>(s.keys[0], b.wire ? s.hit_a : b.hits, s.tile, b.n, ptiles, s.part_info, s.err);
  if (ev) (void)hipEventRecord(ev[2], st);
  if (b.n) {
    const size_t seg_lds = (2ull * ptiles + 1) * 4;
    k_bucket<<<PART_DIGITS, BkSmall::THREADS, seg_lds, st>>>(s.tile, s.part_info, ptiles,
                                                             s.keys[1], s.vals[0], s.hits_s, s.segsum, s.rid,
                                                             s.run_start, s.run_end, s.runs64, s.drun, s.big_meta, s.big_n,
                                                             s.big_work, s.work_n, s.sorted_n, s.uniq, s.uniq_n,
                                                             s.err, big_hint);
#ifndef RL_EXP_NO_BIG
    const uint32_t gi = big_full ? BIG_ITEM_BLOCKS : 1u, gb = big_full ? BIG_BLOCKS : 1u;
    k_big_count<<<gi, BkSmall::THREADS, seg_lds, st>>>(s.tile, s.part_info, ptiles,
                                                                    s.big_meta, s.big_work, s.work_n, s.big_cnt,
                                                                    s.err);
    k_big_place<<<gi, BkSmall::THREADS, seg_lds, st>>>(
        s.tile, s.part_info, ptiles, s.big_meta, s.big_work, s.work_n, s.big_cnt, s.keys[1],
        s.vals[0], s.hits_s, s.segsum, s.rid, s.run_start, s.run_end, s.drun, s.err);
    k_bucket_big<<<gb, BkBig::THREADS, seg_lds, st>>>(s.tile, s.part_info, ptiles,
                                                              s.keys[1], s.vals[0], s.hits_s, s.hit_t, s.segsum,
                                                              s.rid, s.run_start, s.run_end, s.runs64, s.drun, s.big_meta,
                                                              s.big_n, s.big_cnt, s.err);
#endif
    k_run_check<<<cdiv(b.n, RC_CHUNK), 256, 0, st>>>(b, SRec{s.rec, s.vals[0]}, s.keys[1], s.rid, s.run_start,
                                                s.run_end, s.run_flags, s.defer, s.defer_n, s.err, s.runs64, s.split,
                                                s.sorted_n, s.grp, s.hit_t, s.uniq, s.uniq_n, s.long_runs, s.keys[0]);
#ifndef RL_EXP_NO_SPLIT
    k_split<<<SPLIT_BLOCKS, SPLIT_THREADS, 0, st>>>(b, SRec{s.rec, s.vals[0]}, s.vals[0], s.segsum, s.rid, s.run_start,
                                          s.run_end, s.run_flags, s.defer, s.defer_n, s.runs64, s.split, s.drun,
                                          b.n / 2 + BIG_HEAVY * PART_DIGITS, s.grp, s.lead, s.hit_t, s.vals[1], s.err,
                                          per_second, UniqList{s.uniq, s.uniq_n, s.keys[1], s.keys[0]}, s.long_runs, long_hint,
                                          long_kernel ? 1 : 0);
#endif
#if RL_SPLIT_LONG_THREADS
    if (long_kernel)
      k_split_long<<<RL_SPLIT_LONG_BLOCKS, RL_SPLIT_LONG_THREADS, 0, st>>>(
          b, SRec{s.rec, s.vals[0]}, s.vals[0], s.segsum, s.rid, s.run_start, s.run_end, s.run_flags, s.defer,
          s.runs64, s.split, s.drun, b.n / 2 + BIG_HEAVY * PART_DIGITS, s.grp, s.lead, s.hit_t, s.vals[1], s.err,
          per_second, UniqList{s.uniq, s.uniq_n, s.keys[1], s.keys[0]}, s.long_runs);
#endif
  }
}

#ifndef RL_LATE_FAST_BLOCKS
#define RL_LATE_FAST_BLOCKS 0
#endif
constexpr uint32_t LATE_SCAN_BLOCKS = 4;
void launch_b_begin_early(const BatchDev& b, const OutDev& o, const Scratch& s, int restore, hipStream_t st,
                          const unsigned long long* log_ctr) {
  const uint32_t m = restore ? 0u : b.n_rules * RL_NUM_STATS;
  const uint32_t gb = m ? (cdiv(m, 256) < 64 ? cdiv(m, 256) : 64) : 1;
  k_b_begin<<<gb, 256, 0, st>>>(s.err, s.errb, nullptr, s.defer2_n, s.defer1_n, o.stats, m, s.fast_blk,
                                cdiv(b.n, 256 * 32), log_ctr, s.log_epoch);
}

void launch_stage_b(const BatchDev& b, const OutDev& o, const TableDev& t, const Params& P, const Scratch& s,
                    int restore, hipStream_t st, hipEvent_t* ev, const uint32_t* errb_prev, hipEvent_t table_done,
                    unsigned long long* kt_acc, bool early, uint32_t* late_hint, bool late_full) {
  const uint32_t m = restore ? 0u : b.n_rules * RL_NUM_STATS;
  const uint32_t gb = m ? (cdiv(m, 256) < 64 ? cdiv(m, 256) : 64) : 1;
  if (!early)
    k_b_begin<<<gb, 256, 0, st>>>(s.err, s.errb, errb_prev, s.defer2_n, s.defer1_n, o.stats, m, s.fast_blk,
                                  cdiv(b.n, 256 * 32), t.log_ctr, s.log_epoch);
  else if (!b.n)
    k_b_begin<<<1, 256, 0, st>>>(s.errb, s.errb, errb_prev, s.defer2_n, s.defer1_n, o.stats, 0, s.fast_blk, 0,
                                 nullptr, nullptr);
  if (b.n) {
    const uint32_t g = cdiv(b.n, 256);
    const size_t lds = (!restore && b.n_rules <= LDS_RULES) ? (size_t)b.n_rules * RL_NUM_STATS * 8 : 0;
    const SRec rs{s.rec, s.vals[0]};
    if (ev) (void)hipEventRecord(ev[3], st);
    const uint32_t g_runs = cdiv(b.n / 2 + BIG_HEAVY * PART_DIGITS, 256);
    k_table<<<g_runs + g, 256, lds, st>>>(g_runs, b, t, P, rs, s.keys[1], s.vals[0], s.res, s.run_start, s.run_end,
                                         s.run_flags, s.run_state, s.run_alias, s.rid, s.run_f, s.runs64, s.drun,
                                         s.defer2, s.defer2_n,
                                         s.keys[0], s.defer1, s.defer1_n, o.stats, s.stripes, s.errb, s.errs, restore,
                                         s.fast_blk, s.uniq, s.uniq_n, kt_acc ? s.kt_blk : nullptr,
                                         early ? errb_prev : nullptr);
    if (ev) (void)hipEventRecord(ev[4], st);
    if (!restore && P.lc_en)
      k_fast_over<<<g, 256, 0, st>>>(s.sorted_n, rs, s.segsum, s.rid, s.run_flags, s.run_state, s.run_f, s.errb);
#ifndef RL_EXP_NO_LATE
    const uint32_t gl = restore ? 0u : !late_full ? LATE_SCAN_BLOCKS
                                     : (RL_LATE_FAST_BLOCKS && g > RL_LATE_FAST_BLOCKS ? RL_LATE_FAST_BLOCKS : g);
    k_late<<<RUNS_GENERAL_LATE_BLOCKS + gl, 256, lds, st>>>(
        b, t, P, rs, s.keys[1], s.vals[0], s.res, s.run_start, s.run_end, s.defer, s.defer_n, s.defer2, s.defer2_n,
        s.grp, s.lead, s.gmask,
        s.keys[0], s.defer1, s.defer1_n, s.segsum, s.rid, s.run_flags, s.run_state, s.run_alias, s.run_f, o.stats,
        s.stripes, s.errb,
        s.errs, restore, s.fast_blk, s.sorted_n, late_hint, late_full ? 0 : 1);
#endif
    if (table_done) (void)hipEventRecord(table_done, st);
    if (!restore) {
      const uint32_t nf = b.n_rules <= LDS_RULES ? b.n_rules : 0u;
      const uint32_t gf = cdiv(nf * RL_NUM_STATS > b.n ? nf * RL_NUM_STATS : b.n, 256);
      k_finish<<<gf, 256, 0, st>>>(s.res, b.n, o, s.stripes, nf, s.errb, P.lc_en ? s.counters + 5 : nullptr,
                                   kt_acc ? s.kt_blk : nullptr, g_runs + g, kt_acc, b.own);
    }
  } else {
    if (ev) {
      (void)hipEventRecord(ev[3], st);
      (void)hipEventRecord(ev[4], st);
    }
    if (table_done) (void)hipEventRecord(table_done, st);
  }
  if (ev) (void)hipEventRecord(ev[5], st);
}


void launch_sweep(const TableDev& t, uint64_t nslots, uint32_t now, unsigned long long* evicted, hipStream_t st) {
  k_sweep<<<2048, 256, 0, st>>>(t, nslots, now, evicted);
}

void launch_arena_compact(Slot* slots, uint64_t nslots, const uint8_t* from, uint8_t* to, unsigned long long* used16,
                          hipStream_t st) {
  k_arena_compact<<<2048, 256, 0, st>>>(slots, nslots, from, to, used16);
}

void launch_lc_count(const TableDev& t, uint64_t nslots, uint32_t now, unsigned long long* out, hipStream_t st) {
  k_lc_count<<<2048, 256, 0, st>>>(t, nslots, now, out);
}

void launch_table_info(const Slot* slots, uint64_t nslots, unsigned long long* out, hipStream_t st) {
  k_table_info<<<2048, 256, 0, st>>>(slots, nslots, out);
}

bool log_tear_hook() { return RL_LOG_TEAR != 0; }

void launch_debug_keys(const BatchDev& b, uint8_t* out, uint32_t* klen, hipStream_t st) {
  if (b.n) k_debug_keys<<<cdiv(b.n, 256), 256, 0, st>>>(b, out, klen);
}

void launch_debug_decide(uint32_t n, const uint32_t* before, const uint32_t* after, const uint8_t* lc_hit,
                         const uint32_t* hits, const uint32_t* limit, const uint8_t* unit, const uint8_t* flags,
                         const int64_t* now, float ratio, int lc_en, uint8_t* code, uint32_t* rem, uint32_t* reset,
                         unsigned long long* deltas, uint8_t* lc_set, hipStream_t st) {
  if (n)
    k_debug_decide<<<cdiv(n, 256), 256, 0, st>>>(n, before, after, lc_hit, hits, limit, unit, flags, now, ratio,
                                                 lc_en, code, rem, reset, deltas, lc_set);
}

}
```

Before: 5.929 billion.

## Pack partition tiles to 8-byte records, tile-major info, XCD bucket mapping, adaptive uniq list

Measured after the change: 5.980 billion (median of 6 runs). No clear change (+0.9%).

```diff
diff --git a/ratelimit_amd/csrc/rl_engine.h b/ratelimit_amd/csrc/rl_engine.h
--- a/ratelimit_amd/csrc/rl_engine.h
+++ b/ratelimit_amd/csrc/rl_engine.h
@@ -88,6 +88,9 @@
   uint32_t* h_late = nullptr;
   uint32_t late_recent = 0;
   int late_mode = 1;
+  uint32_t* h_uniq = nullptr;
+  uint32_t uniq_recent = 0;
+  int uniq_mode = 1;
   unsigned long long* h_counters = nullptr;
   std::string last_error;
   uint64_t batches = 0, decisions = 0;
diff --git a/ratelimit_amd/csrc/rl_engine.hip b/ratelimit_amd/csrc/rl_engine.hip
--- a/ratelimit_amd/csrc/rl_engine.hip
+++ b/ratelimit_amd/csrc/rl_engine.hip
@@ -160,25 +160,36 @@
     if (c->late_recent) c->late_recent--;
   }
   uint32_t* lhint = c->late_mode == 1 ? c->h_late + k : nullptr;
+  bool uniq_list = c->uniq_mode == 0;
+  if (c->uniq_mode == 1) {
+    for (uint32_t j = 0; j < NBUF; j++)
+      if (__atomic_load_n(&c->h_uniq[j], __ATOMIC_RELAXED)) {
+        __atomic_store_n(&c->h_uniq[j], 0u, __ATOMIC_RELAXED);
+        c->uniq_recent = 4 * NBUF;
+      }
+    uniq_list = c->uniq_recent > 0;
+    if (c->uniq_recent) c->uniq_recent--;
+  }
+  uint32_t* uhint = c->uniq_mode == 1 ? c->h_uniq + k : nullptr;
   if (pipelined) {
     hipStream_t a = c->pipe[k];
     hipEvent_t* ev = prof_events(c);
     (void)hipStreamWaitEvent(a, c->b_done[k], 0);
     (void)hipStreamWaitEvent(a, c->consumed[k], 0);
-    launch_stage_a(b, c->s[k], isolate, P.per_second, a, ev, hint, lng, bhint, big_full);
+    launch_stage_a(b, c->s[k], isolate, P.per_second, a, ev, hint, lng, bhint, big_full, uniq_list);
     if (early) launch_b_begin_early(b, o, c->s[k], restore, a, c->log_ctr);
     (void)hipStreamWaitEvent(a, c->b_table[c->last], 0);
     launch_stage_b(b, o, t, P, c->s[k], restore, a, ev, errb_prev, c->b_table[k], ev ? c->d_kt_acc : nullptr,
-                   early, lhint, late_full);
+                   early, lhint, late_full, uniq_list, uhint);
     (void)hipEventRecord(c->b_done[k], a);
   } else {
     if (!st) st = c->stream;
     (void)after_batches(c, st);
     hipEvent_t* ev = prof_events(c);
-    launch_stage_a(b, c->s[k], isolate, P.per_second, st, ev, hint, lng, bhint, big_full);
+    launch_stage_a(b, c->s[k], isolate, P.per_second, st, ev, hint, lng, bhint, big_full, uniq_list);
     if (early) launch_b_begin_early(b, o, c->s[k], restore, st, c->log_ctr);
     launch_stage_b(b, o, t, P, c->s[k], restore, st, ev, errb_prev, c->b_table[k], ev ? c->d_kt_acc : nullptr,
-                   early, lhint, late_full);
+                   early, lhint, late_full, uniq_list, uhint);
     (void)hipEventRecord(c->b_done[k], st);
   }
   c->last = k;
@@ -463,6 +474,9 @@
   ok = ok && hipHostMalloc((void**)&c->h_late, NBUF * sizeof(uint32_t)) == hipSuccess;
   if (ok) memset(c->h_late, 0, NBUF * sizeof(uint32_t));
   if (const char* lc = getenv("RL_LATE_CUE")) c->late_mode = atoi(lc);
+  ok = ok && hipHostMalloc((void**)&c->h_uniq, NBUF * sizeof(uint32_t)) == hipSuccess;
+  if (ok) memset(c->h_uniq, 0, NBUF * sizeof(uint32_t));
+  if (const char* uc = getenv("RL_UNIQ_CUE")) c->uniq_mode = atoi(uc);
   if (!ok) return fail("gpu: device allocation failed (table_slots/arena/max_batch too large?)", c);
   ok = hipMemsetAsync(c->slots, 0, c->nslots * sizeof(Slot), c->stream) == hipSuccess &&
        hipMemsetAsync(c->log_ctr, 0, (size_t)(LOG_PARTS + 1) * LOG_CTR_STRIDE * 8, c->stream) == hipSuccess &&
@@ -558,6 +572,7 @@
   if (c->h_long) (void)hipHostFree(c->h_long);
   if (c->h_big) (void)hipHostFree(c->h_big);
   if (c->h_late) (void)hipHostFree(c->h_late);
+  if (c->h_uniq) (void)hipHostFree(c->h_uniq);
   for (void* p : {(void*)c->cfg_blob, (void*)c->mbuf})
     if (p) (void)hipFree(p);
   if (c->h_match) (void)hipHostFree(c->h_match);
diff --git a/ratelimit_amd/csrc/rl_kernels.h b/ratelimit_amd/csrc/rl_kernels.h
--- a/ratelimit_amd/csrc/rl_kernels.h
+++ b/ratelimit_amd/csrc/rl_kernels.h
@@ -24,6 +24,14 @@
   uint32_t heavy[BIG_HEAVY];
 };
 constexpr uint32_t MAX_PART_TILES = 2048 * 16 / PART_ITEMS;
+constexpr uint32_t TILE_IDX_BITS = 23, TILE_HITS_ESC = (1u << (32 - TILE_IDX_BITS)) - 1;
+static_assert((uint64_t)MAX_PART_TILES * PART_TILE <= (1ull << TILE_IDX_BITS), "a descriptor index fits the record");
+#ifndef RL_INFO_TILE_MAJOR
+#define RL_INFO_TILE_MAJOR 1
+#endif
+#ifndef RL_XCD_BUCKETS
+#define RL_XCD_BUCKETS 1
+#endif
 constexpr uint32_t LONG_RUN = 32;
 constexpr uint32_t RUN_SLOW = 1, RUN_FAST = 2, RUN_MULTI = 4;
 constexpr uint32_t RUN_NOWVAR = 8;
@@ -184,7 +192,7 @@
   unsigned long long* stripes;
   uint32_t* hits_s;
   uint32_t* hit_a;
-  uint4* tile;
+  uint2* tile;
   uint32_t* hit_t;
   uint32_t* segsum;
   uint32_t* rid;
@@ -214,11 +222,11 @@
 
 void launch_stage_a(const BatchDev& b, const Scratch& s, int isolate, int per_second, hipStream_t st,
                     hipEvent_t* ev = nullptr, uint32_t* long_hint = nullptr, bool long_kernel = false,
-                    uint32_t* big_hint = nullptr, bool big_full = true);
+                    uint32_t* big_hint = nullptr, bool big_full = true, bool uniq_list = true);
 void launch_stage_b(const BatchDev& b, const OutDev& o, const TableDev& t, const Params& P, const Scratch& s,
                     int restore, hipStream_t st, hipEvent_t* ev, const uint32_t* errb_prev, hipEvent_t table_done,
                     unsigned long long* kt_acc = nullptr, bool early = false, uint32_t* late_hint = nullptr,
-                    bool late_full = true);
+                    bool late_full = true, bool uniq_list = true, uint32_t* uniq_hint = nullptr);
 void launch_b_begin_early(const BatchDev& b, const OutDev& o, const Scratch& s, int restore, hipStream_t st,
                           const unsigned long long* log_ctr);
 void launch_unpack(const rl_batch_compact& cb, const uint8_t* buf, uint32_t* req, uint8_t* unit, uint8_t* flags,
diff --git a/ratelimit_amd/csrc/rl_kernels.hip b/ratelimit_amd/csrc/rl_kernels.hip
--- a/ratelimit_amd/csrc/rl_kernels.hip
+++ b/ratelimit_amd/csrc/rl_kernels.hip
@@ -1371,25 +1371,32 @@
   return pre + inc - v;
 }
 
+__device__ inline void tile_rec(const uint2 e, const uint32_t* __restrict__ hin, uint32_t& k, uint32_t& v,
+                                uint32_t& h) {
+  k = e.x;
+  v = e.y & ((1u << TILE_IDX_BITS) - 1u);
+  h = e.y >> TILE_IDX_BITS;
+  if (h == TILE_HITS_ESC) h = hin[v];
+}
+
 __global__ __launch_bounds__(256) void k_part(const uint32_t* __restrict__ kin, const uint32_t* __restrict__ hin,
-                                              uint4* __restrict__ out, uint32_t n, uint32_t ntiles,
+                                              uint2* __restrict__ out, uint32_t n, uint32_t ntiles,
                                               uint32_t* __restrict__ info, const uint32_t* err) {
   constexpr uint32_t DPT = PART_DIGITS / 256;
   __shared__ uint32_t wcnt[4][PART_DIGITS];
   __shared__ uint32_t wsum[4];
-  __shared__ uint32_t sk[PART_TILE], sv[PART_TILE], sh[PART_TILE];
+  __shared__ uint32_t sk[PART_TILE], sv[PART_TILE];
   if (*err) return;
   const uint32_t tid = threadIdx.x, lane = tid & 63, wave = tid >> 6, tile = blockIdx.x;
   for (uint32_t j = tid; j < 4 * PART_DIGITS; j += 256) (&wcnt[0][0])[j] = 0;
   __syncthreads();
   const uint32_t wbase = tile * PART_TILE + wave * 64 * PART_ITEMS;
-  uint32_t kk[PART_ITEMS], vv[PART_ITEMS], hh[PART_ITEMS], pos[PART_ITEMS];
+  uint32_t kk[PART_ITEMS], vv[PART_ITEMS], pos[PART_ITEMS];
 #pragma unroll
   for (uint32_t i = 0; i < PART_ITEMS; i++) {
     const uint32_t j = min(wbase + i * 64 + lane, n - 1);
     kk[i] = kin[j];
-    vv[i] = j;
-    hh[i] = hin[j];
+    vv[i] = j | (min(hin[j], TILE_HITS_ESC) << TILE_IDX_BITS);
   }
   wave_multisplit<PART_ITEMS, PART_BITS>(kk, wbase, n, 32 - PART_BITS, wcnt[wave], pos);
   __syncthreads();
@@ -1408,10 +1415,24 @@
     tsum += acc;
   }
   uint32_t excl = scan256(tsum, wsum, nullptr);
+#if RL_INFO_TILE_MAJOR
+  static_assert(DPT == 4, "a thread's digits are one 16-B store");
+  {
+    uint32_t e[DPT], x = excl;
+#pragma unroll
+    for (uint32_t j = 0; j < DPT; j++) {
+      e[j] = (x << 16) | c[j];
+      x += c[j];
+    }
+    reinterpret_cast<uint4*>(info + (size_t)tile * PART_DIGITS)[tid] = make_uint4(e[0], e[1], e[2], e[3]);
+  }
+#endif
 #pragma unroll
   for (uint32_t j = 0; j < DPT; j++) {
     const uint32_t d = tid * DPT + j;
+#if !RL_INFO_TILE_MAJOR
     info[(size_t)d * ntiles + tile] = (excl << 16) | c[j];
+#endif
 #pragma unroll
     for (uint32_t w = 0; w < 4; w++) wcnt[w][d] += excl;
     excl += c[j];
@@ -1424,16 +1445,15 @@
       const uint32_t q = wcnt[wave][d] + pos[i];
       sk[q] = kk[i];
       sv[q] = vv[i];
-      sh[q] = hh[i];
     }
   }
   __syncthreads();
   const uint32_t cnt = min(PART_TILE, n - tile * PART_TILE);
-  uint4* o = out + (size_t)tile * PART_TILE;
+  uint2* o = out + (size_t)tile * PART_TILE;
 #pragma unroll
   for (uint32_t i = 0; i < PART_ITEMS; i++) {
     const uint32_t q = i * 256 + tid;
-    if (q < cnt) o[q] = make_uint4(sk[q], sv[q], sh[q], 0u);
+    if (q < cnt) o[q] = make_uint2(sk[q], sv[q]);
   }
 }
 
@@ -1506,7 +1526,11 @@
   uint32_t carry = 0, offs = 0;
   for (uint32_t t0 = 0; t0 < ntiles; t0 += B::THREADS) {
     const uint32_t t = t0 + tid;
+#if RL_INFO_TILE_MAJOR
+    const uint32_t e = t < ntiles ? info[(size_t)t * PART_DIGITS + d] : 0u;
+#else
     const uint32_t e = t < ntiles ? info[(size_t)d * ntiles + t] : 0u;
+#endif
     const uint32_t cnt = e & 0xFFFFu;
     offs += e >> 16;
     uint32_t inc = cnt;
@@ -1743,7 +1767,7 @@
 
 constexpr uint32_t BK_SAMPLES_PER_LANE = 4;
 template <typename B>
-__device__ inline void sample_heavy(BucketLds<B>& L, uint32_t S, uint32_t ntiles, const uint4* __restrict__ pt) {
+__device__ inline void sample_heavy(BucketLds<B>& L, uint32_t S, uint32_t ntiles, const uint2* __restrict__ pt) {
   constexpr uint32_t R = BK_SAMPLES_PER_LANE, NS = 64 * R;
   const uint32_t lane = threadIdx.x & 63;
   if ((threadIdx.x >> 6) == 0) {
@@ -1791,7 +1815,7 @@
 }
 
 __global__ __launch_bounds__(BkSmall::THREADS, 4) void k_bucket(
-    const uint4* __restrict__ pt,
+    const uint2* __restrict__ pt, const uint32_t* __restrict__ hin,
     const uint32_t* __restrict__ info, uint32_t ntiles, uint32_t* __restrict__ sk, uint32_t* __restrict__ sv,
     uint32_t* __restrict__ sh, uint32_t* __restrict__ segsum, uint32_t* __restrict__ rid,
     uint32_t* __restrict__ run_start, uint32_t* __restrict__ run_end, unsigned long long* num_runs,
@@ -1801,7 +1825,13 @@
   using B = BkSmall;
   __shared__ BucketLds<B> L;
   if (*err) return;
-  const uint32_t tid = threadIdx.x, lane = tid & 63, wave = tid >> 6, d = blockIdx.x;
+  const uint32_t tid = threadIdx.x, lane = tid & 63, wave = tid >> 6;
+#if RL_XCD_BUCKETS
+  static_assert(PART_DIGITS % 8 == 0, "buckets per XCD");
+  const uint32_t d = (blockIdx.x % 8) * (PART_DIGITS / 8) + blockIdx.x / 8;
+#else
+  const uint32_t d = blockIdx.x;
+#endif
   BK_STAMP(d, 0);
   bucket_setup(L, info, ntiles, d);
   const uint32_t S = L.S;
@@ -1841,10 +1871,9 @@
   bucket_src(ntiles, pp, jj);
 #pragma unroll
   for (uint32_t i = 0; i < B::ITEMS; i++) {
-    const uint4 e = pt[jj[i]];
+    const uint2 e = pt[jj[i]];
     kk[i] = e.x;
     vv[i] = e.y;
-    hh[i] = e.z;
   }
   BK_STAMP(d, 2);
   uint32_t* ht = L.v;
@@ -1907,19 +1936,23 @@
   for (uint32_t i = 0; i < B::ITEMS; i++) {
     if (!((dmask >> i) & 1u)) continue;
     const uint32_t c = wpre + cidx[i];
-    L.k[c] = kk[i];
-    L.v[c] = vv[i];
-    L.h[c] = hh[i];
+    uint32_t k, x, y;
+    tile_rec(make_uint2(kk[i], vv[i]), hin, k, x, y);
+    L.k[c] = k;
+    L.v[c] = x;
+    L.h[c] = y;
   }
   if (tid == 0) {
     if (M) L.base_pos = atomicAdd(sorted_n, M);
     L.ub = M < S ? atomicAdd(uniq_n, S - M) : 0u;
   }
   __syncthreads();
-  const uint32_t ub = L.ub + spre;
-#pragma unroll
-  for (uint32_t i = 0; i < B::ITEMS; i++)
-    if ((smask >> i) & 1u) uniq[ub + sidx[i]] = make_uint2(vv[i], kk[i]);
+  if (uniq) {
+    const uint32_t ub = L.ub + spre;
+#pragma unroll
+    for (uint32_t i = 0; i < B::ITEMS; i++)
+      if ((smask >> i) & 1u) uniq[ub + sidx[i]] = make_uint2(vv[i] & ((1u << TILE_IDX_BITS) - 1u), kk[i]);
+  }
   if (!M) return;
   const uint32_t base = L.base_pos;
   if (M <= 64) {
@@ -1960,7 +1993,7 @@
 
 template <typename B>
 __device__ inline bool bucket_peel(BucketLds<B>& L, uint32_t d, uint32_t S, uint32_t base, uint32_t ntiles,
-                                   const uint4* __restrict__ pt,
+                                   const uint2* __restrict__ pt, const uint32_t* __restrict__ hin,
                                    uint32_t* __restrict__ sk,
                                    uint32_t* __restrict__ sv, uint32_t* __restrict__ sh) {
   constexpr uint32_t IT = B::ITEMS;
@@ -2003,13 +2036,11 @@
 #pragma unroll
     for (uint32_t i = 0; i < IT; i++) pp[i] = min(strip0 + i * 64 + lane, S - 1);
     bucket_src(ntiles, pp, jj);
-#pragma unroll
-    for (uint32_t i = 0; i < IT; i++) {
-      const uint4 e = pt[jj[i]];
-      kk[i] = e.x;
-      vv[i] = e.y;
-      hh[i] = e.z;
-    }
+    uint2 e[IT];
+#pragma unroll
+    for (uint32_t i = 0; i < IT; i++) e[i] = pt[jj[i]];
+#pragma unroll
+    for (uint32_t i = 0; i < IT; i++) tile_rec(e[i], hin, kk[i], vv[i], hh[i]);
     uint32_t wl = 0, lr[IT];
     uint32_t wc[BK_HEAVY];
 #pragma unroll
@@ -2114,13 +2145,11 @@
 #pragma unroll
     for (uint32_t i = 0; i < IT; i++) pp[i] = min(s0 + i * 64 + lane, S - 1);
     bucket_src(ntiles, pp, jj);
-#pragma unroll
-    for (uint32_t i = 0; i < IT; i++) {
-      const uint4 e = pt[jj[i]];
-      kk[i] = e.x;
-      vv[i] = e.y;
-      hh[i] = e.z;
-    }
+    uint2 e[IT];
+#pragma unroll
+    for (uint32_t i = 0; i < IT; i++) e[i] = pt[jj[i]];
+#pragma unroll
+    for (uint32_t i = 0; i < IT; i++) tile_rec(e[i], hin, kk[i], vv[i], hh[i]);
     uint32_t hr[IT], wc[BK_HEAVY];
 #pragma unroll
     for (uint32_t c = 0; c < BK_HEAVY; c++) wc[c] = 0;
@@ -2172,7 +2201,7 @@
 
 template <typename B>
 __device__ inline void bucket_lsd(BucketLds<B>& L, uint32_t S, uint32_t base, uint32_t ntiles,
-                                  const uint4* __restrict__ pt,
+                                  const uint2* __restrict__ pt, const uint32_t* __restrict__ hin,
                                   uint32_t* __restrict__ sk,
                                   uint32_t* __restrict__ sv, uint32_t* __restrict__ sh, uint32_t* __restrict__ ht,
                                   uint32_t* __restrict__ segsum, uint32_t* __restrict__ rid) {
@@ -2223,13 +2252,11 @@
         for (uint32_t i = 0; i < IT; i++) jj[i] = pp[i];
       }
       if (pass == 0) {
-#pragma unroll
-        for (uint32_t i = 0; i < IT; i++) {
-          const uint4 e = pt[jj[i]];
-          kk[i] = e.x;
-          vv[i] = e.y;
-          hh[i] = e.z;
-        }
+        uint2 e[IT];
+#pragma unroll
+        for (uint32_t i = 0; i < IT; i++) e[i] = pt[jj[i]];
+#pragma unroll
+        for (uint32_t i = 0; i < IT; i++) tile_rec(e[i], hin, kk[i], vv[i], hh[i]);
       } else {
 #pragma unroll
         for (uint32_t i = 0; i < IT; i++) {
@@ -2287,7 +2314,8 @@
   return x;
 }
 
-__device__ inline void big_chunk_load(const BigMeta& M, uint32_t j, uint32_t ntiles, const uint4* __restrict__ pt,
+__device__ inline void big_chunk_load(const BigMeta& M, uint32_t j, uint32_t ntiles, const uint2* __restrict__ pt,
+                                      const uint32_t* __restrict__ hin,
                                       uint32_t (&kk)[BkSmall::ITEMS], uint32_t (&vv)[BkSmall::ITEMS],
                                       uint32_t (&hh)[BkSmall::ITEMS], uint32_t (&cls)[BkSmall::ITEMS], bool values) {
   using B = BkSmall;
@@ -2296,12 +2324,13 @@
 #pragma unroll
   for (uint32_t i = 0; i < B::ITEMS; i++) pp[i] = min(s0 + i * 64 + lane, M.S - 1);
   bucket_src(ntiles, pp, jj);
+  uint2 e[B::ITEMS];
+#pragma unroll
+  for (uint32_t i = 0; i < B::ITEMS; i++) e[i] = pt[jj[i]];
 #pragma unroll
   for (uint32_t i = 0; i < B::ITEMS; i++) {
-    const uint4 e = pt[jj[i]];
-    kk[i] = e.x;
-    hh[i] = e.z;
-    vv[i] = values ? e.y : 0u;
+    tile_rec(e[i], hin, kk[i], vv[i], hh[i]);
+    if (!values) vv[i] = 0u;
   }
 #pragma unroll
   for (uint32_t i = 0; i < B::ITEMS; i++) {
@@ -2312,7 +2341,8 @@
   }
 }
 
-__global__ __launch_bounds__(BkSmall::THREADS) void k_big_count(const uint4* __restrict__ pt,
+__global__ __launch_bounds__(BkSmall::THREADS) void k_big_count(const uint2* __restrict__ pt,
+                                                                const uint32_t* __restrict__ hin,
                                                                 const uint32_t* __restrict__ info, uint32_t ntiles,
                                                                 const BigMeta* __restrict__ meta,
                                                                 const uint32_t* __restrict__ work,
@@ -2327,7 +2357,7 @@
     const BigMeta M = meta[w >> 16];
     bucket_setup(L, info, ntiles, M.d);
     uint32_t kk[B::ITEMS], vv[B::ITEMS], hh[B::ITEMS], cls[B::ITEMS];
-    big_chunk_load(M, w & 0xFFFFu, ntiles, pt, kk, vv, hh, cls, false);
+    big_chunk_load(M, w & 0xFFFFu, ntiles, pt, hin, kk, vv, hh, cls, false);
     uint32_t nl = 0, nc[BK_HEAVY], hs[BK_HEAVY];
 #pragma unroll
     for (uint32_t c = 0; c < BK_HEAVY; c++) nc[c] = hs[c] = 0;
@@ -2367,7 +2397,7 @@
 }
 
 __global__ __launch_bounds__(BkSmall::THREADS) void k_big_place(
-    const uint4* __restrict__ pt,
+    const uint2* __restrict__ pt, const uint32_t* __restrict__ hin,
     const uint32_t* __restrict__ info, uint32_t ntiles, const BigMeta* __restrict__ meta,
     const uint32_t* __restrict__ work, const uint32_t* work_n, const uint32_t* __restrict__ cnt,
     uint32_t* __restrict__ sk, uint32_t* __restrict__ sv, uint32_t* __restrict__ sh, uint32_t* __restrict__ segsum,
@@ -2413,7 +2443,7 @@
       drun[M.db_heavy + tid] = M.rb_heavy + tid;
     }
     uint32_t kk[B::ITEMS], vv[B::ITEMS], hh[B::ITEMS], cls[B::ITEMS];
-    big_chunk_load(M, j, ntiles, pt, kk, vv, hh, cls, true);
+    big_chunk_load(M, j, ntiles, pt, hin, kk, vv, hh, cls, true);
     uint32_t rk[B::ITEMS], hp[B::ITEMS], wl = 0, wc[BK_HEAVY], wh[BK_HEAVY];
 #pragma unroll
     for (uint32_t c = 0; c < BK_HEAVY; c++) wc[c] = wh[c] = 0;
@@ -2490,7 +2520,7 @@
 }
 
 __global__ __launch_bounds__(BkBig::THREADS) void k_bucket_big(
-    const uint4* __restrict__ pt,
+    const uint2* __restrict__ pt, const uint32_t* __restrict__ hin,
     const uint32_t* __restrict__ info, uint32_t ntiles, uint32_t* __restrict__ sk, uint32_t* __restrict__ sv,
     uint32_t* __restrict__ sh, uint32_t* __restrict__ ht, uint32_t* __restrict__ segsum, uint32_t* __restrict__ rid,
     uint32_t* __restrict__ run_start, uint32_t* __restrict__ run_end, unsigned long long* num_runs,
@@ -2537,8 +2567,8 @@
       if (tid < M.r) run_start[M.rb_heavy + tid] = run_end[M.rb_heavy + tid] = 0;
       bucket_setup(L, info, ntiles, d);
       BK_STAMP(d, 1);
-      if (!bucket_peel(L, d, S, base, ntiles, pt, sk, sv, sh))
-        bucket_lsd(L, S, base, ntiles, pt, sk, sv, sh, ht, segsum, rid);
+      if (!bucket_peel(L, d, S, base, ntiles, pt, hin, sk, sv, sh))
+        bucket_lsd(L, S, base, ntiles, pt, hin, sk, sv, sh, ht, segsum, rid);
       bucket_segment<B, false>(L, d, S, base, sk, sh, segsum, rid, run_start, run_end, num_runs, drun);
     }
     BK_STAMP(d, 7);
@@ -2602,7 +2632,7 @@
     uint32_t at = 0;
     if (lane == leader) at = atomicAdd(uniq_n, (uint32_t)__popcll(m));
     at = __shfl(at, leader, 64) + (uint32_t)__popcll(m & ((1ull << lane) - 1));
-    if (one) uniq[at] = make_uint2(rec_s.sv[q], k);
+    if (one && uniq) uniq[at] = make_uint2(rec_s.sv[q], k);
   }
   const uint32_t lo = max(blockIdx.x * RC_CHUNK, 1u), hi = min(blockIdx.x * RC_CHUNK + RC_CHUNK, sn);
   if (lo >= hi) return;
@@ -2622,8 +2652,10 @@
     if (!same_stem && !skip && q == p + 1 && run_end[r] == q + 1) {
       run_end[r] = p;
       const uint32_t at = atomicAdd(uniq_n, 2u);
-      uniq[at] = make_uint2(ep, skeys[q]);
-      uniq[at + 1] = make_uint2(eq, skeys[q]);
+      if (uniq) {
+        uniq[at] = make_uint2(ep, skeys[q]);
+        uniq[at + 1] = make_uint2(eq, skeys[q]);
+      }
       continue;
     }
     keys0[eq] = KEY_DUP;
@@ -2765,7 +2797,8 @@
   __device__ inline void single(uint32_t e, uint32_t p) const {
     const uint32_t k = skeys[p];
     keys0[e] = k;
-    list[atomicAdd(n, 1u)] = make_uint2(e, k);
+    const uint32_t at = atomicAdd(n, 1u);
+    if (list) list[at] = make_uint2(e, k);
   }
 };
 
@@ -3382,15 +3415,17 @@
                                                 unsigned long long* __restrict__ res,
                                                 uint32_t* __restrict__ defer1, uint32_t* defer1_n,
                                                 unsigned long long* stats, unsigned long long* stripes, uint32_t* err,
-                                                uint32_t* errs, int restore, const uint32_t* errb_prev) {
+                                                uint32_t* errs, int restore, const uint32_t* errb_prev,
+                                                int list_valid, uint32_t* uniq_hint) {
   __shared__ uint32_t s_err, s_nu, s_cnt, s_list[256];
   if (threadIdx.x == 0) {
     s_err = __hip_atomic_load(err, __ATOMIC_RELAXED, __HIP_MEMORY_SCOPE_AGENT) | (errb_prev ? *errb_prev : 0u);
     s_nu = *uniq_n;
+    if (blk == 0 && uniq_hint && (uint64_t)s_nu * 4 < (uint64_t)b.n * RL_UNIQ_DENSE) *uniq_hint = 1u;
   }
   __syncthreads();
   const uint32_t nu = s_nu;
-  const bool by_list = (uint64_t)nu * 4 < (uint64_t)b.n * RL_UNIQ_DENSE;
+  const bool by_list = list_valid && (uint64_t)nu * 4 < (uint64_t)b.n * RL_UNIQ_DENSE;
   const uint32_t lo = blk * 256, hi = min(lo + 256, by_list ? nu : b.n);
   if (s_err || lo >= hi) return;
   refine_totals(b);
@@ -4177,7 +4212,7 @@
                                                unsigned long long* stripes, uint32_t* err, uint32_t* errs, int restore,
                                                uint32_t* __restrict__ fast_blk, const uint2* __restrict__ uniq,
                                                const uint32_t* uniq_n, unsigned long long* __restrict__ kt,
-                                               const uint32_t* errb_prev) {
+                                               const uint32_t* errb_prev, int list_valid, uint32_t* uniq_hint) {
 
   if (kt && threadIdx.x == 0) kt[2 * blockIdx.x] = wall_clock64();
   if (errb_prev && blockIdx.x == 0 && threadIdx.x == 0) {
@@ -4192,14 +4227,14 @@
               errb_prev);
   else
     unique_body(blockIdx.x, b, t, P, rec_s.rec, keys0, uniq, uniq_n, res, defer1, defer1_n, stats, stripes, err, errs,
-                restore, errb_prev);
+                restore, errb_prev, list_valid, uniq_hint);
 #else
   if (blockIdx.x < g_runs)
     runs_body(blockIdx.x, b, t, P, rec_s, skeys, svals, res, run_start, run_end, run_flags, run_state, run_alias, rid,
               run_f, num_runs, drun, defer2, defer2_n, stats, stripes, err, errs, restore, fast_blk, errb_prev);
   else
     unique_body(blockIdx.x - g_runs, b, t, P, rec_s.rec, keys0, uniq, uniq_n, res, defer1, defer1_n, stats, stripes,
-                err, errs, restore, errb_prev);
+                err, errs, restore, errb_prev, list_valid, uniq_hint);
 #endif
   if (kt && threadIdx.x == 0) kt[2 * blockIdx.x + 1] = wall_clock64();
 }
@@ -4464,7 +4499,8 @@
 static inline uint32_t cdiv(uint64_t a, uint64_t b) { return (uint32_t)((a + b - 1) / b); }
 
 void launch_stage_a(const BatchDev& b, const Scratch& s, int isolate, int per_second, hipStream_t st,
-                    hipEvent_t* ev, uint32_t* long_hint, bool long_kernel, uint32_t* big_hint, bool big_full) {
+                    hipEvent_t* ev, uint32_t* long_hint, bool long_kernel, uint32_t* big_hint, bool big_full,
+                    bool uniq_list) {
   const uint32_t g0 = cdiv(b.n > b.n_req ? b.n : b.n_req, 256);
   if (ev) (void)hipEventRecord(ev[0], st);
   if (g0)
@@ -4472,37 +4508,38 @@
                                   s.work_n, s.run_flags, s.runs64, s.hit_a, s.res, s.sorted_n, s.uniq_n);
   if (ev) (void)hipEventRecord(ev[1], st);
   const uint32_t ptiles = cdiv(b.n, PART_TILE);
-  if (b.n)
-    k_part<<<ptiles, 256, 0, st>>>(s.keys[0], b.wire ? s.hit_a : b.hits, s.tile, b.n, ptiles, s.part_info, s.err);
+  const uint32_t* hin = b.wire ? s.hit_a : b.hits;
+  if (b.n) k_part<<<ptiles, 256, 0, st>>>(s.keys[0], hin, s.tile, b.n, ptiles, s.part_info, s.err);
   if (ev) (void)hipEventRecord(ev[2], st);
   if (b.n) {
     const size_t seg_lds = (2ull * ptiles + 1) * 4;
-    k_bucket<<<PART_DIGITS, BkSmall::THREADS, seg_lds, st>>>(s.tile, s.part_info, ptiles,
+    uint2* const ulist = uniq_list ? s.uniq : nullptr;
+    k_bucket<<<PART_DIGITS, BkSmall::THREADS, seg_lds, st>>>(s.tile, hin, s.part_info, ptiles,
                                                              s.keys[1], s.vals[0], s.hits_s, s.segsum, s.rid,
                                                              s.run_start, s.run_end, s.runs64, s.drun, s.big_meta, s.big_n,
-                                                             s.big_work, s.work_n, s.sorted_n, s.uniq, s.uniq_n,
+                                                             s.big_work, s.work_n, s.sorted_n, ulist, s.uniq_n,
                                                              s.err, big_hint);
 #ifndef RL_EXP_NO_BIG
     const uint32_t gi = big_full ? BIG_ITEM_BLOCKS : 1u, gb = big_full ? BIG_BLOCKS : 1u;
-    k_big_count<<<gi, BkSmall::THREADS, seg_lds, st>>>(s.tile, s.part_info, ptiles,
+    k_big_count<<<gi, BkSmall::THREADS, seg_lds, st>>>(s.tile, hin, s.part_info, ptiles,
                                                                     s.big_meta, s.big_work, s.work_n, s.big_cnt,
                                                                     s.err);
     k_big_place<<<gi, BkSmall::THREADS, seg_lds, st>>>(
-        s.tile, s.part_info, ptiles, s.big_meta, s.big_work, s.work_n, s.big_cnt, s.keys[1],
+        s.tile, hin, s.part_info, ptiles, s.big_meta, s.big_work, s.work_n, s.big_cnt, s.keys[1],
         s.vals[0], s.hits_s, s.segsum, s.rid, s.run_start, s.run_end, s.drun, s.err);
-    k_bucket_big<<<gb, BkBig::THREADS, seg_lds, st>>>(s.tile, s.part_info, ptiles,
+    k_bucket_big<<<gb, BkBig::THREADS, seg_lds, st>>>(s.tile, hin, s.part_info, ptiles,
                                                               s.keys[1], s.vals[0], s.hits_s, s.hit_t, s.segsum,
                                                               s.rid, s.run_start, s.run_end, s.runs64, s.drun, s.big_meta,
                                                               s.big_n, s.big_cnt, s.err);
 #endif
     k_run_check<<<cdiv(b.n, RC_CHUNK), 256, 0, st>>>(b, SRec{s.rec, s.vals[0]}, s.keys[1], s.rid, s.run_start,
                                                 s.run_end, s.run_flags, s.defer, s.defer_n, s.err, s.runs64, s.split,
-                                                s.sorted_n, s.grp, s.hit_t, s.uniq, s.uniq_n, s.long_runs, s.keys[0]);
+                                                s.sorted_n, s.grp, s.hit_t, ulist, s.uniq_n, s.long_runs, s.keys[0]);
 #ifndef RL_EXP_NO_SPLIT
     k_split<<<SPLIT_BLOCKS, SPLIT_THREADS, 0, st>>>(b, SRec{s.rec, s.vals[0]}, s.vals[0], s.segsum, s.rid, s.run_start,
                                           s.run_end, s.run_flags, s.defer, s.defer_n, s.runs64, s.split, s.drun,
                                           b.n / 2 + BIG_HEAVY * PART_DIGITS, s.grp, s.lead, s.hit_t, s.vals[1], s.err,
-                                          per_second, UniqList{s.uniq, s.uniq_n, s.keys[1], s.keys[0]}, s.long_runs, long_hint,
+                                          per_second, UniqList{ulist, s.uniq_n, s.keys[1], s.keys[0]}, s.long_runs, long_hint,
                                           long_kernel ? 1 : 0);
 #endif
 #if RL_SPLIT_LONG_THREADS
@@ -4510,7 +4547,7 @@
       k_split_long<<<RL_SPLIT_LONG_BLOCKS, RL_SPLIT_LONG_THREADS, 0, st>>>(
           b, SRec{s.rec, s.vals[0]}, s.vals[0], s.segsum, s.rid, s.run_start, s.run_end, s.run_flags, s.defer,
           s.runs64, s.split, s.drun, b.n / 2 + BIG_HEAVY * PART_DIGITS, s.grp, s.lead, s.hit_t, s.vals[1], s.err,
-          per_second, UniqList{s.uniq, s.uniq_n, s.keys[1], s.keys[0]}, s.long_runs);
+          per_second, UniqList{ulist, s.uniq_n, s.keys[1], s.keys[0]}, s.long_runs);
 #endif
   }
 }
@@ -4529,7 +4566,8 @@
 
 void launch_stage_b(const BatchDev& b, const OutDev& o, const TableDev& t, const Params& P, const Scratch& s,
                     int restore, hipStream_t st, hipEvent_t* ev, const uint32_t* errb_prev, hipEvent_t table_done,
-                    unsigned long long* kt_acc, bool early, uint32_t* late_hint, bool late_full) {
+                    unsigned long long* kt_acc, bool early, uint32_t* late_hint, bool late_full, bool uniq_list,
+                    uint32_t* uniq_hint) {
   const uint32_t m = restore ? 0u : b.n_rules * RL_NUM_STATS;
   const uint32_t gb = m ? (cdiv(m, 256) < 64 ? cdiv(m, 256) : 64) : 1;
   if (!early)
@@ -4549,7 +4587,7 @@
                                          s.defer2, s.defer2_n,
                                          s.keys[0], s.defer1, s.defer1_n, o.stats, s.stripes, s.errb, s.errs, restore,
                                          s.fast_blk, s.uniq, s.uniq_n, kt_acc ? s.kt_blk : nullptr,
-                                         early ? errb_prev : nullptr);
+                                         early ? errb_prev : nullptr, uniq_list ? 1 : 0, uniq_hint);
     if (ev) (void)hipEventRecord(ev[4], st);
     if (!restore && P.lc_en)
       k_fast_over<<<g, 256, 0, st>>>(s.sorted_n, rs, s.segsum, s.rid, s.run_flags, s.run_state, s.run_f, s.errb);
```
